# sea-with-sakura/ViT-of-Pytorch

Measured on AMD Instinct MI355X. Metric: images/sec training step, ViT-B/16 224px bf16, 1/2/4/8 MI355X, higher is better.
Workload: dtype bf16; 1 GPU; ViT-B16 @224 train step (fwd+CE+bwd+SGD-momentum/OneCycleLR); model=ViT-B16, image_size=224, per_gpu_batch=256, global_batch=256, seq_len=197, num_classes=1000, parallelism=dp1, step_launch=eager

## Files before the change

### include/vit_hip.h

```cpp
#ifndef VIT_HIP_H_
#define VIT_HIP_H_

#include <stdint.h>

#ifdef __cplusplus
extern "C" {
#endif

typedef void* vit_stream_t;

enum vit_status {
  VIT_OK = 0,
  VIT_ERR_INVALID_ARG = 1,
  VIT_ERR_HIP = 2,
  VIT_ERR_UNSUPPORTED = 3,
};

const char* vit_last_error(void);
int vit_abi_version(void);
const char* vit_build_id(void);

enum vit_layout { VIT_K_CONTIG = 0, VIT_MN_CONTIG = 1 };

typedef struct vit_dropout {
  float p;
  uint32_t site;
  uint64_t seed;
  uint64_t offset;
  int64_t row_stride;
} vit_dropout;

int vit_dropout_mask(const vit_dropout* d, int64_t row0, int64_t rows, int64_t cols, float* mult,
                     int64_t ld, vit_stream_t stream);

enum vit_epilogue {
  VIT_EPI_F32 = 0,
  VIT_EPI_BF16 = 1,
  VIT_EPI_BIAS_BF16 = 2,
  VIT_EPI_BIAS_GELU = 3,
  VIT_EPI_BIAS_RESID_F32 = 4,
  VIT_EPI_GELU_BWD = 5,
  VIT_EPI_PATCH = 6,
  VIT_EPI_SPLITK = 7,
  VIT_EPI_BIAS_GELU_DGELU = 8,
  VIT_EPI_MUL_BF16 = 9,
};

typedef struct vit_gemm_args {
  int64_t M, N, K;
  const void* A;
  int64_t lda;
  int64_t a_batch_stride;
  int32_t a_layout;
  int32_t b_layout;
  const void* B;
  int64_t ldb;
  int64_t b_batch_stride;
  void* C;
  int64_t ldc;
  int64_t c_batch_stride;
  void* C2;
  int64_t ldc2;
  const float* bias;
  int64_t bias_batch_stride;
  const void* aux;
  int64_t ldaux;
  const float* aux2;
  int64_t batch;
  int64_t split_k;
  int64_t tokens;
  float* col_partial;
  int32_t epilogue;
  int32_t tile;
  const vit_dropout* dropout;
} vit_gemm_args;

int vit_gemm_bf16(const vit_gemm_args* args, vit_stream_t stream);
int64_t vit_gemm_tile_rows(const vit_gemm_args* args);
int64_t vit_gemm_partial_rows(const vit_gemm_args* args);
int64_t vit_gemm_split_rows(const vit_gemm_args* args);
int vit_gemm_bf16_part(const vit_gemm_args* args, int32_t part, vit_stream_t stream);
int vit_gemm_splitk_group(const vit_gemm_args* args, int32_t n, vit_stream_t stream);

int vit_splitk_reduce(const float* ws, int64_t batch, int64_t split, int64_t M, int64_t N,
                      float* out, int64_t ldo, int64_t out_batch_stride, int32_t accumulate,
                      vit_stream_t stream);
#define VIT_SPLITK_GROUP_MAX 8
typedef struct vit_splitk_job {
  const float* ws;
  int64_t batch, split, M, N;
  float* out;
  int64_t ldo, out_batch_stride;
  int32_t accumulate;
  int32_t reserved;
} vit_splitk_job;
int vit_splitk_reduce_group(const vit_splitk_job* jobs, int32_t njobs, vit_stream_t stream);

int vit_layernorm_fwd(const float* x, int64_t ldx, const float* gamma, const float* beta,
                      void* y, int64_t ldy, int32_t y_f32, float* mean, float* rstd,
                      int64_t rows, int64_t D, float eps, vit_stream_t stream);
int64_t vit_layernorm_bwd_partial_rows(int64_t rows);
int64_t vit_layernorm_bwd_blocks(int64_t rows);
int vit_layernorm_bwd(const void* dy, int64_t lddy, int32_t dy_f32, const float* x, int64_t ldx,
                      const float* mean, const float* rstd, const float* gamma,
                      const float* dres, int64_t lddres, float* dx, int64_t lddx,
                      void* dx_bf16, int64_t lddxb, float* partial, float* dgamma_dbeta,
                      float* dx_colsum, int32_t accumulate_params, int64_t rows, int64_t D,
                      const vit_dropout* dx_dropout, vit_stream_t stream);

int vit_attention_fwd(const void* qkv, void* o, float* lse, int64_t B, int64_t N, int64_t H,
                      int64_t hd, float scale, vit_stream_t stream);
int vit_attention_bwd(const void* qkv, const void* o, const void* dout, const float* lse, void* dqkv,
                      float* bias_partial, int64_t B, int64_t N, int64_t H, int64_t hd, float scale,
                      vit_stream_t stream);
int vit_attention_fwd_rows(const void* qkv, void* o, float* lse, int64_t B, int64_t N, int64_t H, int64_t hd,
                           float scale, int64_t q_rows, vit_stream_t stream);
int vit_attention_bwd_rows(const void* qkv, const void* o, const void* dout, const float* lse, void* dqkv,
                           float* bias_partial, int64_t B, int64_t N, int64_t H, int64_t hd, float scale,
                           int64_t q_rows, vit_stream_t stream);
int64_t vit_attention_bias_rows(int64_t N, int64_t hd, int32_t path);
int64_t vit_attention_workspace_elems(int64_t B, int64_t N, int64_t H, int32_t path);
int vit_attention_fwd_ex(const void* qkv, void* o, float* lse, int64_t B, int64_t N, int64_t H, int64_t hd,
                         float scale, int64_t q_rows, int32_t path, vit_stream_t stream);
int vit_attention_bwd_ex(const void* qkv, const void* o, const void* dout, const float* lse, void* dqkv,
                         float* bias_partial, int64_t B, int64_t N, int64_t H, int64_t hd, float scale,
                         int64_t q_rows, int32_t path, float* workspace, vit_stream_t stream);

int vit_attention_fwd_varlen(const void* q, int64_t ldq, const void* k, int64_t ldk, const void* v, int64_t ldv,
                             void* o, int64_t ldo, const int32_t* cu_q, int64_t B, int64_t max_q, int64_t Nkv,
                             int64_t H, int64_t hd, float scale, vit_stream_t stream);

int vit_im2col(const float* x, void* out, int64_t B, int64_t img, int64_t P, int64_t Kpad,
               vit_stream_t stream);
int vit_im2col_hw(const float* x, void* out, int64_t B, int64_t H, int64_t W, int64_t Ph, int64_t Pw, int64_t Kpad,
                  vit_stream_t stream);

int vit_preprocess_u8(const uint8_t* images, int64_t B, int64_t H, int64_t W, int64_t image_stride,
                      const uint8_t* flips, int64_t out_h, int64_t out_w, const float* mean_std, float* out,
                      vit_stream_t stream);

enum vit_image_layout { VIT_IMAGES_HWC = 0, VIT_IMAGES_CHW = 1 };
int vit_preprocess_u8_gather(const uint8_t* images, int64_t n_images, int32_t layout, int64_t H, int64_t W,
                             int64_t image_stride, const int64_t* index, int64_t B, const uint8_t* flips,
                             int64_t out_h, int64_t out_w, const float* mean_std, float* out,
                             const int64_t* labels_in, int64_t* labels_out, vit_stream_t stream);

int vit_embed_grad(const float* dh0, int64_t B, int64_t N, int64_t D, float* dpos, float* dcls,
                   float* dconv_bias, const vit_dropout* dropout, vit_stream_t stream);

int64_t vit_colsum_partial_rows(int64_t rows);
int vit_colsum(const void* in, int32_t in_bf16, int64_t rows, int64_t cols, int64_t ld,
               float* partial, float* out, int32_t accumulate, vit_stream_t stream);
int vit_colsum3(const void* in, int32_t in_bf16, int64_t rows, int64_t seg, int64_t ld, float* partial,
                float* out0, float* out1, float* out2, int32_t accumulate, vit_stream_t stream);

#define VIT_COLSUM_BATCH_MAX 8
typedef struct vit_colsum_job {
  const float* in;
  int64_t rows, cols, ld, seg;
  float* out0;
  float* out1;
  float* out2;
  int32_t accumulate;
  int32_t reserved;
} vit_colsum_job;
int vit_colsum_batch(const vit_colsum_job* jobs, int32_t njobs, vit_stream_t stream);

int vit_gemm_f32(int64_t M, int64_t N, int64_t K, const float* A, int64_t lda, int32_t a_trans,
                 const float* B, int64_t ldb, int32_t b_trans, float* C, int64_t ldc,
                 const float* bias, int32_t accumulate, vit_stream_t stream);

int vit_cross_entropy(const float* logits, const int64_t* labels, int64_t B, int64_t C,
                      float* dlogits, float grad_scale, float* row_stats, vit_stream_t stream);

int vit_sgd_step(float* p, const float* g, float* buf, void* p_bf16, int64_t n, float lr,
                 float momentum, float weight_decay, int32_t first, vit_stream_t stream);
int vit_sgd_step_dev(float* p, const float* g, float* buf, void* p_bf16, int64_t n, const float* hyper,
                     float weight_decay, vit_stream_t stream);
int vit_cast_f32_bf16(const float* in, void* out, int64_t n, vit_stream_t stream);
int vit_cast_pad_rows(const float* in, int64_t rows, int64_t cols, void* out, int64_t ldo,
                      vit_stream_t stream);
#define VIT_CAST_BATCH_MAX 8
typedef struct vit_cast_job {
  const float* in;
  int64_t rows, cols, ldi;
  void* out;
  int64_t ldo, rows_pad, cols_pad;
} vit_cast_job;
int vit_cast_pad_batch(const vit_cast_job* jobs, int32_t njobs, vit_stream_t stream);
int vit_pack_cols(const float* in, int64_t zstride, int64_t ldi, int64_t rows, int64_t cols, int64_t Z,
                  void* out, int64_t ldo, int32_t out_bf16, vit_stream_t stream);
int vit_pack_cols_batched(const float* in, int64_t in_batch_stride, int64_t zstride, int64_t ldi, int64_t rows,
                          int64_t cols, int64_t Z, void* out, int64_t out_batch_stride, int64_t ldo,
                          int32_t out_bf16, int64_t batch, vit_stream_t stream);
int vit_transpose_f32_bf16(const float* in, int64_t rows, int64_t cols, int64_t ldi, void* out, int64_t ldo,
                           int64_t batch, int64_t in_batch_stride, int64_t out_batch_stride, vit_stream_t stream);
int vit_axpby(const float* x, float* y, int64_t n, float a, float b, vit_stream_t stream);

int vit_im2col_f32(const float* x, float* out, int64_t B, int64_t img, int64_t P, int64_t Kpad,
                   vit_stream_t stream);
int vit_im2col_hw_f32(const float* x, float* out, int64_t B, int64_t H, int64_t W, int64_t Ph, int64_t Pw,
                      int64_t Kpad, vit_stream_t stream);
int vit_embed_fwd_f32(float* h, int64_t B, int64_t N, int64_t D, const float* pos, const float* cls,
                      vit_stream_t stream);
int vit_gelu_f32(const float* in, float* out, int64_t n, vit_stream_t stream);
int vit_attention_fwd_f32(const float* qkv, float* o, int64_t B, int64_t N, int64_t H, int64_t hd,
                          float inv_sqrt_hd, vit_stream_t stream);

int vit_gelu_bwd_f32(const float* u, const float* dy, float* dx, int64_t n, vit_stream_t stream);
int vit_dropout_apply_f32(const vit_dropout* d, const float* in, float* out, int64_t rows, int64_t cols,
                          vit_stream_t stream);
int vit_add_bcast_f32(const float* x, const float* y, float* out, int64_t outer, int64_t inner, vit_stream_t stream);
int vit_segment_colsum(const void* in, int32_t in_bf16, int64_t ld, int64_t segs, int64_t seg_stride, int64_t row0,
                       int64_t seg_rows, int64_t cols, float scale, float* out, int64_t ldo, vit_stream_t stream);
int vit_segment_colsum_bcast(const void* in, int32_t in_bf16, int64_t ld, int64_t segs, int64_t seg_stride,
                             int64_t row0, int64_t seg_rows, int64_t cols, float scale, float* out, int64_t ldo,
                             void* bc, int64_t ldbc, int64_t bc_rows, vit_stream_t stream);
int64_t vit_router_dx_gate_partial_rows(int64_t rows_pad);
int vit_router_dx_gate(const float* dx, int64_t ldx, const float* g, int64_t ldg, float g_scale, const void* gp,
                       int64_t ldgp, int64_t T, int64_t N, int64_t reserve, int64_t cols, void* out, int64_t ldo,
                       int64_t rows_pad, int64_t cols_pad, float* col_partial, int64_t ldp, vit_stream_t stream);
int64_t vit_router_head_partials(int64_t T);
int vit_router_head_fwd(const float* logits, const float* noise, int32_t noise_mode, const float* yhard_in, int64_t T,
                        int64_t N, int32_t bs, int64_t reserve, int32_t training, float norm, float* soft, float* ysoft,
                        float* hard, float* indices, float* ent_part, float* entropy, vit_stream_t stream);
int vit_router_head_bwd(const float* soft, const float* ysoft, const float* dsoft, const float* dhard, const float* dind,
                        const float* dent, float norm, int64_t T, int64_t N, int32_t bs, int64_t reserve,
                        int32_t training, float* dlogits, vit_stream_t stream);
int vit_router_select(const float* indices, int64_t T, int32_t npos, const uint32_t* active_masks, int32_t nkeys,
                      void* active, void* sel, void* any, vit_stream_t stream);
int vit_cast_rows_masked(const float* in, int64_t ldi, int64_t rows, int64_t cols, const void* mask, void* out,
                         int64_t ldo, vit_stream_t stream);
int vit_cls_mse(const float* x, int64_t ldx, const float* t, int64_t ldt, int64_t B, int64_t D, float* e, float* part,
                float* loss, vit_stream_t stream);
int vit_cls_mse_bwd(float* dx, int64_t lddx, const float* e, int64_t B, int64_t D, const float* g,
                    vit_stream_t stream);
int vit_unpack_bf16_f32(const void* in, int64_t ldi, int64_t rows, int64_t cols, float* out, int64_t ldo,
                        vit_stream_t stream);

int vit_sqnorm_partial(const float* g, int64_t n, double* partial, int32_t nparts, vit_stream_t stream);
int vit_adamw_prep(const double* partial, int32_t nparts, const float* used, float* steps, int32_t nseg,
                   float lr, float beta1, float beta2, float max_norm, float* table, float* norm_out,
                   vit_stream_t stream);
int vit_adamw_update(float* p, float* g, float* m, float* v, void* p_bf16, const int64_t* chunks, int32_t nchunks,
                     const float* table, float decay, float beta1, float beta2, float one_minus_beta1,
                     float one_minus_beta2, float eps, int32_t write_grad, vit_stream_t stream);
int vit_adamw_chunk_elems(void);
int vit_scale_by_coef(float* g, int64_t n, const float* coef, vit_stream_t stream);
int vit_zero(void* ptr, int64_t bytes, vit_stream_t stream);
int vit_rows_select(void* dst, int64_t dld, const void* src, int64_t sld, const void* mask, int64_t rows,
                    int64_t row_bytes, vit_stream_t stream);
int vit_copy2d(void* dst, int64_t dpitch, const void* src, int64_t spitch, int64_t width, int64_t height,
               vit_stream_t stream);

#ifdef __cplusplus
}
#endif
#endif
```

### vit-of-pytorch_amd/csrc/capi.hip

```cpp
#include <stdarg.h>

#include "common.h"
#include "build_id.h"

namespace vit {
static thread_local char g_last_error[512] = "";

void set_error(const char* fmt, ...) {
  va_list ap;
  va_start(ap, fmt);
  vsnprintf(g_last_error, sizeof(g_last_error), fmt, ap);
  va_end(ap);
}

int check_hip(hipError_t e, const char* what) {
  if (e == hipSuccess) return VIT_OK;
  set_error("%s: %s", what, hipGetErrorString(e));
  return VIT_ERR_HIP;
}
}

extern "C" const char* vit_last_error(void) { return vit::g_last_error; }
extern "C" int vit_abi_version(void) { return 20; }
extern "C" const char* vit_build_id(void) { return VIT_BUILD_ID; }
```

### vit-of-pytorch_amd/csrc/elementwise.hip

```cpp
#include "common.h"

namespace {

template <typename OUT>
__global__ void im2col_kernel(const float* __restrict__ x, OUT* __restrict__ out, int B, int H, int W, int Ph, int Pw,
                              int Kpad) {
  const int gw = W / Pw;
  const int N = (H / Ph) * gw + 1;
  const long total = (long)B * N * Kpad;
  const int PP = Ph * Pw, K = 3 * PP;
  for (long i = (long)blockIdx.x * blockDim.x + threadIdx.x; i < total; i += (long)gridDim.x * blockDim.x) {
    const int col = (int)(i % Kpad);
    const long row = i / Kpad;
    const int t = (int)(row % N);
    const int b = (int)(row / N);
    float v = 0.f;
    if (t > 0 && col < K) {
      const int patch = t - 1, py = patch / gw, px = patch % gw;
      const int c = col / PP, rem = col % PP, ky = rem / Pw, kx = rem % Pw;
      v = x[(((long)b * 3 + c) * H + (py * Ph + ky)) * W + (px * Pw + kx)];
    }
    if constexpr (sizeof(OUT) == 2)
      out[i] = f2bf(v);
    else
      out[i] = v;
  }
}

__global__ void pos_grad_kernel(const float* __restrict__ dh0, int B, int N, int D, float* __restrict__ dpos,
                                DropDev drop) {
  const int n = blockIdx.y;
  const int d = blockIdx.x * blockDim.x + threadIdx.x;
  if (d >= D) return;
  float s = 0.f;
  if (drop.thr) {
    for (int b = 0; b < B; ++b) s += dh0[((long)b * N + n) * D + d] * drop_mult1(drop, (long)b * N + n, d);
  } else {
    for (int b = 0; b < B; ++b) s += dh0[((long)b * N + n) * D + d];
  }
  dpos[(long)n * D + d] = s;
}

__global__ void dropout_mask_kernel(DropDev drop, long row0, long rows, int cols, float* __restrict__ out, long ld) {
  const long r = blockIdx.y;
  const int c = blockIdx.x * blockDim.x + threadIdx.x;
  if (r >= rows || c >= cols) return;
  out[r * ld + c] = drop.thr ? drop_mult1(drop, row0 + r, c) : 1.0f;
}

template <typename OUT>
__global__ void im2col8_kernel(const float* __restrict__ x, OUT* __restrict__ out, int B, int H, int W, int Ph,
                               int Pw) {
  const int gw = W / Pw, N = (H / Ph) * gw + 1, PP = Ph * Pw, K8 = 3 * PP / 8;
  const long total = (long)B * N * K8;
  for (long i = (long)blockIdx.x * blockDim.x + threadIdx.x; i < total; i += (long)gridDim.x * blockDim.x) {
    const int c8 = (int)(i % K8);
    const long row = i / K8;
    const int t = (int)(row % N), b = (int)(row / N);
    float4 lo = make_float4(0.f, 0.f, 0.f, 0.f), hi = lo;
    if (t > 0) {
      const int patch = t - 1, py = patch / gw, px = patch % gw;
      const int col = c8 * 8, c = col / PP, rem = col % PP, ky = rem / Pw, kx = rem % Pw;
      const float4* src =
          reinterpret_cast<const float4*>(x + (((long)b * 3 + c) * H + (py * Ph + ky)) * W + (px * Pw + kx));
      lo = src[0];
      hi = src[1];
    }
    if constexpr (sizeof(OUT) == 2) {
      uint4 v;
      v.x = (uint32_t)f2bf(lo.x) | ((uint32_t)f2bf(lo.y) << 16);
      v.y = (uint32_t)f2bf(lo.z) | ((uint32_t)f2bf(lo.w) << 16);
      v.z = (uint32_t)f2bf(hi.x) | ((uint32_t)f2bf(hi.y) << 16);
      v.w = (uint32_t)f2bf(hi.z) | ((uint32_t)f2bf(hi.w) << 16);
      reinterpret_cast<uint4*>(out)[i] = v;
    } else {
      reinterpret_cast<float4*>(out)[2 * i] = lo;
      reinterpret_cast<float4*>(out)[2 * i + 1] = hi;
    }
  }
}

__global__ void __launch_bounds__(768) pos_grad4_kernel(const float* __restrict__ dh0, int B, int N, int D,
                                                        float* __restrict__ dpos, DropDev drop) {
  __shared__ float4 red[8][96];
  const int C4 = D / 4 / gridDim.y;
  const int n = blockIdx.x, c = threadIdx.x % C4, grp = threadIdx.x / C4;
  const int d = (blockIdx.y * C4 + c) * 4;
  float4 s = make_float4(0.f, 0.f, 0.f, 0.f);
  const float* base = dh0 + (long)n * D + d;
  const long bstride = (long)N * D;
#pragma unroll 4
  for (int b = grp; b < B; b += 8) {
    float4 v = *reinterpret_cast<const float4*>(base + b * bstride);
    if (drop.thr) {
      const long r = (long)b * N + n;
      v.x *= drop_mult1(drop, r, d);
      v.y *= drop_mult1(drop, r, d + 1);
      v.z *= drop_mult1(drop, r, d + 2);
      v.w *= drop_mult1(drop, r, d + 3);
    }
    s.x += v.x;
    s.y += v.y;
    s.z += v.z;
    s.w += v.w;
  }
  red[grp][c] = s;
  __syncthreads();
  if (grp == 0) {
#pragma unroll
    for (int k = 1; k < 8; ++k) {
      s.x += red[k][c].x;
      s.y += red[k][c].y;
      s.z += red[k][c].z;
      s.w += red[k][c].w;
    }
    *reinterpret_cast<float4*>(dpos + (long)n * D + d) = s;
  }
}

__global__ void __launch_bounds__(256) cls_bias_grad16_kernel(const float* __restrict__ dpos, int N, int D,
                                                              float* __restrict__ dcls, float* __restrict__ dbias) {
  __shared__ float red[16][17];
  const int c = threadIdx.x & 15, r = threadIdx.x >> 4;
  const int d = blockIdx.x * 16 + c;
  float s = 0.f;
  if (d < D)
    for (int n = 1 + r; n < N; n += 16) s += dpos[(long)n * D + d];
  red[r][c] = s;
  __syncthreads();
  if (r == 0 && d < D) {
    float t = 0.f;
#pragma unroll
    for (int k = 0; k < 16; ++k) t += red[k][c];
    dbias[d] = t;
    dcls[d] = dpos[d];
  }
}

constexpr int COLSUM_MAX_CHUNKS = 256;
constexpr int COLSUM_MIN_ROWS_PER_CHUNK = 64;

__device__ __forceinline__ float* seg_dst(float* out, float* out1, float* out2, long seg, long ch, int cols, int col) {
  if (seg <= 0) return out + ch * cols + col;
  const int k = (int)(col / seg);
  float* base = k == 0 ? out : (k == 1 ? out1 : out2);
  return base ? base + (col - k * seg) : nullptr;
}

template <bool BF16>
__global__ void __launch_bounds__(256) colsum8_kernel(const void* __restrict__ in, long rows, int cols, long ld,
                                                      int chunks, float* __restrict__ out, int accumulate,
                                                      long seg = 0, float* out1 = nullptr, float* out2 = nullptr) {
  __shared__ float red[8][32][9];
// ... 55 lines not shown
}
__global__ void colsum_final_kernel(const float* __restrict__ partial, int chunks, int cols, float* __restrict__ out,
                                    int accumulate) {
  const int c = blockIdx.x * blockDim.x + threadIdx.x;
  if (c >= cols) return;
  float s = 0.f;
  for (int k = 0; k < chunks; ++k) s += partial[(long)k * cols + c];
  out[c] = accumulate ? out[c] + s : s;
}

constexpr int GF_LD = 48;
__global__ void __launch_bounds__(256) gemm_f32_kernel(int M, int N, int K, const float* __restrict__ A, long lda,
                                                       int at, const float* __restrict__ B, long ldb, int bt,
                                                       float* __restrict__ C, long ldc, const float* __restrict__ bias,
                                                       int accumulate) {
  __shared__ float smem[4 * 2 * 16 * GF_LD];
  const int lane = threadIdx.x & 63, wave = threadIdx.x >> 6;
  const int m0 = blockIdx.y * 32, n0 = blockIdx.x * 32;
  float* As = smem + wave * 2 * 16 * GF_LD;
  float* Bs = As + 16 * GF_LD;
  v4f acc[2][2];
#pragma unroll
  for (int i = 0; i < 2; ++i)
#pragma unroll
    for (int j = 0; j < 2; ++j) acc[i][j] = v4f{0.f, 0.f, 0.f, 0.f};
  const int nkt = (K + 15) / 16;
  auto load = [&](int kt, float* av, float* bv) {
    const int k0 = kt * 16;
#pragma unroll
    for (int e = 0; e < 8; ++e) {
      const int idx = lane + e * 64;
      int m, k;
      if (at) { k = idx >> 5; m = idx & 31; } else { m = idx >> 4; k = idx & 15; }
      const int gm = m0 + m, gk = k0 + k;
      av[e] = (kt < nkt && gm < M && gk < K) ? (at ? A[(long)gk * lda + gm] : A[(long)gm * lda + gk]) : 0.f;
      int n, kb;
      if (bt) { n = idx >> 4; kb = idx & 15; } else { kb = idx >> 5; n = idx & 31; }
      const int gn = n0 + n, gkb = k0 + kb;
      bv[e] = (kt < nkt && gn < N && gkb < K) ? (bt ? B[(long)gn * ldb + gkb] : B[(long)gkb * ldb + gn]) : 0.f;
    }
  };
  float av[8], bv[8];
  load(wave, av, bv);
  for (int kt = wave; kt < nkt; kt += 4) {
#pragma unroll
    for (int e = 0; e < 8; ++e) {
      const int idx = lane + e * 64;
      if (at) As[(idx >> 5) * GF_LD + (idx & 31)] = av[e]; else As[(idx & 15) * GF_LD + (idx >> 4)] = av[e];
      if (bt) Bs[(idx & 15) * GF_LD + (idx >> 4)] = bv[e]; else Bs[(idx >> 5) * GF_LD + (idx & 31)] = bv[e];
    }
    load(kt + 4, av, bv);
    __builtin_amdgcn_wave_barrier();
    asm volatile("s_waitcnt lgkmcnt(0)" ::: "memory");
#pragma unroll
    for (int ks = 0; ks < 4; ++ks) {
      const int k = ks * 4 + (lane >> 4);
      float a[2], b[2];
#pragma unroll
      for (int t = 0; t < 2; ++t) {
        a[t] = As[k * GF_LD + t * 16 + (lane & 15)];
        b[t] = Bs[k * GF_LD + t * 16 + (lane & 15)];
      }
#pragma unroll
      for (int i = 0; i < 2; ++i)
#pragma unroll
        for (int j = 0; j < 2; ++j) acc[i][j] = __builtin_amdgcn_mfma_f32_16x16x4f32(a[i], b[j], acc[i][j], 0, 0, 0);
    }
    asm volatile("s_waitcnt lgkmcnt(0)" ::: "memory");
    __builtin_amdgcn_wave_barrier();
  }
  __syncthreads();
  float* red = smem;
#pragma unroll
  for (int i = 0; i < 2; ++i)
#pragma unroll
    for (int j = 0; j < 2; ++j)
#pragma unroll
      for (int r = 0; r < 4; ++r)
        red[wave * 32 * 33 + (i * 16 + 4 * (lane >> 4) + r) * 33 + j * 16 + (lane & 15)] = acc[i][j][r];
  __syncthreads();
#pragma unroll
  for (int e = 0; e < 4; ++e) {
    const int idx = threadIdx.x + e * 256, row = idx >> 5, col = idx & 31;
    const int m = m0 + row, n = n0 + col;
    if (m >= M || n >= N) continue;
    float v = red[row * 33 + col] + red[32 * 33 + row * 33 + col] + red[2 * 32 * 33 + row * 33 + col] +
              red[3 * 32 * 33 + row * 33 + col];
    if (bias) v += bias[n];
    float* dst = C + (long)m * ldc + n;
    *dst = accumulate ? *dst + v : v;
  }
}

__global__ void __launch_bounds__(256) ce_kernel(const float* __restrict__ logits, const int64_t* __restrict__ labels,
                                                 int C, float* __restrict__ dlogits, float grad_scale,
                                                 float* __restrict__ row_stats) {
  __shared__ float red[4];
  __shared__ float red2[4];
  const int b = blockIdx.x;
  const float* x = logits + (long)b * C;
  const int64_t y64 = labels[b];
  const bool ok = y64 >= 0 && y64 < C;
  const int y = ok ? (int)y64 : 0;
  const int lane = threadIdx.x & 63, wave = threadIdx.x >> 6;
  float mx = -INFINITY;
  for (int c = threadIdx.x; c < C; c += 256) mx = fmaxf(mx, x[c]);
  mx = wave_max(mx);
  if (lane == 0) red[wave] = mx;
  __syncthreads();
  mx = fmaxf(fmaxf(red[0], red[1]), fmaxf(red[2], red[3]));
  __syncthreads();
  const float xy = ok ? x[y] : __builtin_nanf("");
  float s = 0.f, gt = 0.f;
  for (int c = threadIdx.x; c < C; c += 256) {
    s += __expf(x[c] - mx);
    gt += x[c] > xy ? 1.f : 0.f;
  }
  s = wave_sum(s);
  gt = wave_sum(gt);
  if (lane == 0) {
    red[wave] = s;
    red2[wave] = gt;
  }
  __syncthreads();
  s = red[0] + red[1] + red[2] + red[3];
  gt = red2[0] + red2[1] + red2[2] + red2[3];
  const float lse = mx + logf(s);
  if (dlogits) {
    for (int c = threadIdx.x; c < C; c += 256) {
      const float p = __expf(x[c] - lse);
      dlogits[(long)b * C + c] = ok ? (p - (c == y ? 1.f : 0.f)) * grad_scale : __builtin_nanf("");
    }
  }
  if (threadIdx.x == 0 && row_stats) {
    row_stats[b * 3 + 0] = lse - xy;
    row_stats[b * 3 + 1] = gt < 1.f ? 1.f : 0.f;
    row_stats[b * 3 + 2] = gt < 5.f ? 1.f : 0.f;
  }
}

struct SgdHostScalars {
  float lr, mom;
  int first;
  __device__ __forceinline__ void get(float& l, float& m, bool& f) const { l = lr; m = mom; f = first != 0; }
};
struct SgdDevScalars {
  const float* hyper;
  __device__ __forceinline__ void get(float& l, float& m, bool& f) const {
    l = hyper[0];
    m = hyper[1];
    f = hyper[2] != 0.0f;
  }
};
template <class S>
__global__ void sgd_kernel(float* __restrict__ p, const float* __restrict__ g, float* __restrict__ buf,
                           bf16_t* __restrict__ pb, long n, const S sc, float wd) {
  float lr, mom;
  bool first;
  sc.get(lr, mom, first);
  const long n4 = n / 4;
  for (long i = (long)blockIdx.x * blockDim.x + threadIdx.x; i < n4; i += (long)gridDim.x * blockDim.x) {
    float4 pv = reinterpret_cast<float4*>(p)[i];
    const float4 gv = reinterpret_cast<const float4*>(g)[i];
    float4 d = make_float4(gv.x + wd * pv.x, gv.y + wd * pv.y, gv.z + wd * pv.z, gv.w + wd * pv.w);
    if (!first) {
      const float4 bv = reinterpret_cast<float4*>(buf)[i];
      d = make_float4(mom * bv.x + d.x, mom * bv.y + d.y, mom * bv.z + d.z, mom * bv.w + d.w);
    }
    reinterpret_cast<float4*>(buf)[i] = d;
    pv = make_float4(pv.x - lr * d.x, pv.y - lr * d.y, pv.z - lr * d.z, pv.w - lr * d.w);
    reinterpret_cast<float4*>(p)[i] = pv;
    if (pb) {
      uint2 u;
      u.x = pack2bf(pv.x, pv.y);
      u.y = pack2bf(pv.z, pv.w);
      reinterpret_cast<uint2*>(pb)[i] = u;
    }
  }
  const long t = n4 * 4 + (long)blockIdx.x * blockDim.x + threadIdx.x;
  if (blockIdx.x == 0 && t < n) {
    float d = g[t] + wd * p[t];
    if (!first) d = mom * buf[t] + d;
    buf[t] = d;
    p[t] -= lr * d;
    if (pb) pb[t] = f2bf(p[t]);
  }
}

__global__ void cast_kernel(const float* __restrict__ in, bf16_t* __restrict__ out, long n) {
  for (long i = (long)blockIdx.x * blockDim.x + threadIdx.x; i < n; i += (long)gridDim.x * blockDim.x) out[i] = f2bf(in[i]);
}
__global__ void cast_pad_kernel(const float* __restrict__ in, long rows, long cols, bf16_t* __restrict__ out, long ldo) {
  const long total = rows * ldo;
  for (long i = (long)blockIdx.x * blockDim.x + threadIdx.x; i < total; i += (long)gridDim.x * blockDim.x) {
    const long r = i / ldo, c = i % ldo;
    out[i] = c < cols ? f2bf(in[r * cols + c]) : (bf16_t)0;
  }
}
__global__ void axpby_kernel(const float* __restrict__ x, float* __restrict__ y, long n, float a, float b) {
  for (long i = (long)blockIdx.x * blockDim.x + threadIdx.x; i < n; i += (long)gridDim.x * blockDim.x)
    y[i] = a * x[i] + (b == 0.f ? 0.f : b * y[i]);
}

unsigned grid_for(long n, int per_thread = 1) {
  long b = (n / per_thread + 255) / 256;
  if (b < 1) b = 1;
  if (b > 8192) b = 8192;
  return (unsigned)b;
}

template <typename OUT>
void im2col_launch(const float* x, OUT* out, int64_t B, int64_t H, int64_t W, int64_t Ph, int64_t Pw, int64_t Kpad,
                   hipStream_t s) {
  const int64_t N = (H / Ph) * (W / Pw) + 1;
  if (Pw % 8 == 0 && W % 4 == 0 && Kpad == 3 * Ph * Pw && (uintptr_t)x % 16 == 0 && (uintptr_t)out % 16 == 0)
    hipLaunchKernelGGL(im2col8_kernel<OUT>, dim3(grid_for(B * N * Kpad / 8)), dim3(256), 0, s, x, out, (int)B, (int)H,
                       (int)W, (int)Ph, (int)Pw);
  else
    hipLaunchKernelGGL(im2col_kernel<OUT>, dim3(grid_for(B * N * Kpad)), dim3(256), 0, s, x, out, (int)B, (int)H,
                       (int)W, (int)Ph, (int)Pw, (int)Kpad);
}

}

extern "C" int vit_im2col_hw(const float* x, void* out, int64_t B, int64_t H, int64_t W, int64_t Ph, int64_t Pw,
                             int64_t Kpad, vit_stream_t stream) {
  VIT_CHECK_ARG(x && out && B > 0 && Ph > 0 && Pw > 0 && H >= Ph && W >= Pw && Kpad >= 3 * Ph * Pw &&
                    3 * H * W < (1L << 31) && Kpad < (1L << 31),
                "vit_im2col_hw: bad args");
  im2col_launch(x, (bf16_t*)out, B, H, W, Ph, Pw, Kpad, (hipStream_t)stream);
  VIT_LAUNCH_CHECK("vit_im2col_hw");
}

extern "C" int vit_im2col_hw_f32(const float* x, float* out, int64_t B, int64_t H, int64_t W, int64_t Ph, int64_t Pw,
                                 int64_t Kpad, vit_stream_t stream) {
  VIT_CHECK_ARG(x && out && B > 0 && Ph > 0 && Pw > 0 && H >= Ph && W >= Pw && Kpad >= 3 * Ph * Pw &&
                    3 * H * W < (1L << 31) && Kpad < (1L << 31),
                "vit_im2col_hw_f32: bad args");
  im2col_launch(x, out, B, H, W, Ph, Pw, Kpad, (hipStream_t)stream);
  VIT_LAUNCH_CHECK("vit_im2col_hw_f32");
}

extern "C" int vit_im2col(const float* x, void* out, int64_t B, int64_t img, int64_t P, int64_t Kpad,
                          vit_stream_t stream) {
  VIT_CHECK_ARG(x && out && B > 0 && P > 0 && img >= P && Kpad >= 3 * P * P, "vit_im2col: bad args");
  im2col_launch(x, (bf16_t*)out, B, img, img, P, P, Kpad, (hipStream_t)stream);
  VIT_LAUNCH_CHECK("vit_im2col");
}

extern "C" int vit_embed_grad(const float* dh0, int64_t B, int64_t N, int64_t D, float* dpos, float* dcls,
                              float* dconv_bias, const vit_dropout* dropout, vit_stream_t stream) {
  VIT_CHECK_ARG(dh0 && dpos && dcls && dconv_bias && B > 0 && N > 0 && D > 0, "vit_embed_grad: bad args");
  hipStream_t s = (hipStream_t)stream;
  int ys = 0;
  if (D % 4 == 0 && ((uintptr_t)dh0 % 16) == 0 && ((uintptr_t)dpos % 16) == 0) {
    const int d4 = (int)(D / 4);
    for (int y = (d4 + 95) / 96; y <= d4; ++y)
      if (d4 % y == 0) { ys = y; break; }
    if (ys == 1 && N < 256 && d4 % 2 == 0) ys = 2;
  }
  if (ys > 0)
    hipLaunchKernelGGL(pos_grad4_kernel, dim3((unsigned)N, (unsigned)ys), dim3((unsigned)(8 * (D / 4 / ys))), 0, s, dh0,
                       (int)B, (int)N, (int)D, dpos, make_drop(dropout));
  else
    hipLaunchKernelGGL(pos_grad_kernel, dim3((unsigned)((D + 255) / 256), (unsigned)N), dim3(256), 0, s, dh0, (int)B,
                       (int)N, (int)D, dpos, make_drop(dropout));
  hipLaunchKernelGGL(cls_bias_grad16_kernel, dim3((unsigned)((D + 15) / 16)), dim3(256), 0, s, dpos, (int)N, (int)D,
                     dcls, dconv_bias);
  VIT_LAUNCH_CHECK("vit_embed_grad");
}

extern "C" int64_t vit_colsum_partial_rows(int64_t rows) {
  int64_t c = rows / COLSUM_MIN_ROWS_PER_CHUNK;
  if (c > COLSUM_MAX_CHUNKS) c = COLSUM_MAX_CHUNKS;
  return c < 1 ? 1 : c;
}

extern "C" int vit_colsum3(const void* in, int32_t in_bf16, int64_t rows, int64_t seg, int64_t ld, float* partial,
                           float* out0, float* out1, float* out2, int32_t accumulate, vit_stream_t stream) {
  const int64_t cols = 3 * seg;
  VIT_CHECK_ARG(in && partial && seg > 0 && ld >= cols, "vit_colsum3: bad args");
  const int chunks = (int)vit_colsum_partial_rows(rows);
  const bool vec = cols % 8 == 0 && ld % 8 == 0 && ((uintptr_t)in % 32) == 0 && ((uintptr_t)partial % 16) == 0;
  VIT_CHECK_ARG(vec, "vit_colsum3: needs 8-column aligned rows");
  hipStream_t s = (hipStream_t)stream;
  const unsigned gx = (unsigned)((cols / 8 + 31) / 32);
  if (chunks == 1) {
    if (in_bf16)
      hipLaunchKernelGGL(colsum8_kernel<true>, dim3(gx, 1), dim3(256), 0, s, in, (long)rows, (int)cols, (long)ld, 1,
                         out0, (int)accumulate, (long)seg, out1, out2);
    else
      hipLaunchKernelGGL(colsum8_kernel<false>, dim3(gx, 1), dim3(256), 0, s, in, (long)rows, (int)cols, (long)ld, 1,
                         out0, (int)accumulate, (long)seg, out1, out2);
    VIT_LAUNCH_CHECK("vit_colsum3");
  }
  if (in_bf16)
    hipLaunchKernelGGL(colsum8_kernel<true>, dim3(gx, chunks), dim3(256), 0, s, in, (long)rows, (int)cols, (long)ld,
                       chunks, partial, 0, 0L, (float*)nullptr, (float*)nullptr);
  else
    hipLaunchKernelGGL(colsum8_kernel<false>, dim3(gx, chunks), dim3(256), 0, s, in, (long)rows, (int)cols, (long)ld,
                       chunks, partial, 0, 0L, (float*)nullptr, (float*)nullptr);
  hipLaunchKernelGGL(colsum8_kernel<false>, dim3(gx, 1), dim3(256), 0, s, (const void*)partial, (long)chunks,
                     (int)cols, (long)cols, 1, out0, (int)accumulate, (long)seg, out1, out2);
  VIT_LAUNCH_CHECK("vit_colsum3");
}

extern "C" int vit_colsum(const void* in, int32_t in_bf16, int64_t rows, int64_t cols, int64_t ld, float* partial,
                          float* out, int32_t accumulate, vit_stream_t stream) {
  VIT_CHECK_ARG(in && partial && out && cols > 0 && ld >= cols, "vit_colsum: bad args");
  hipStream_t s = (hipStream_t)stream;
  const int chunks = (int)vit_colsum_partial_rows(rows);
  const bool vec = cols % 8 == 0 && ld % 8 == 0 && ((uintptr_t)in % 32) == 0 && ((uintptr_t)partial % 16) == 0 &&
                   ((uintptr_t)out % 4) == 0;
  if (vec) {
    const unsigned gx = (unsigned)((cols / 8 + 31) / 32);
    float* dst1 = chunks == 1 ? out : partial;
    if (in_bf16)
      hipLaunchKernelGGL(colsum8_kernel<true>, dim3(gx, chunks), dim3(256), 0, s, in, (long)rows, (int)cols, (long)ld,
                         chunks, dst1, chunks == 1 ? (int)accumulate : 0);
    else
      hipLaunchKernelGGL(colsum8_kernel<false>, dim3(gx, chunks), dim3(256), 0, s, in, (long)rows, (int)cols,
                         (long)ld, chunks, dst1, chunks == 1 ? (int)accumulate : 0);
    if (chunks > 1)
      hipLaunchKernelGGL(colsum8_kernel<false>, dim3(gx, 1), dim3(256), 0, s, (const void*)partial, (long)chunks,
                         (int)cols, (long)cols, 1, out, (int)accumulate);
    VIT_LAUNCH_CHECK("vit_colsum");
  }
  const unsigned gx = (unsigned)((cols + 255) / 256);
  hipLaunchKernelGGL(colsum_partial_kernel, dim3(gx, chunks), dim3(256), 0, s, in, (int)in_bf16, (long)rows, (int)cols,
                     (long)ld, chunks, partial);
  hipLaunchKernelGGL(colsum_final_kernel, dim3(gx), dim3(256), 0, s, partial, chunks, (int)cols, out, (int)accumulate);
  VIT_LAUNCH_CHECK("vit_colsum");
}

namespace {
struct ColsumJobDev {
  const float* in;
  float* out[3];
  long ld;
  int rows, cols, seg, acc, blk0;
  int pad;
};
struct ColsumBatchDev {
  ColsumJobDev j[VIT_COLSUM_BATCH_MAX];
  int n;
};

__global__ void __launch_bounds__(256) colsum_batch_kernel(const ColsumBatchDev bt) {
  __shared__ float4 red[16][17];
  const int bid = blockIdx.x;
  int jx = 0;
#pragma unroll
  for (int k = 1; k < VIT_COLSUM_BATCH_MAX; ++k)
    if (k < bt.n && bid >= bt.j[k].blk0) jx = k;
  const ColsumJobDev& J = bt.j[jx];
  const int c0 = (bid - J.blk0) * 64;
  const int cg = threadIdx.x & 15, rl = threadIdx.x >> 4;
  const int c = c0 + cg * 4;
  float4 acc = {0.f, 0.f, 0.f, 0.f};
  if (J.pad && c < J.cols) {
    const float* p = J.in + c;
    const long ld = J.ld;
    int r = rl;
    for (; r + 112 < J.rows; r += 128) {
      float4 v[8];
#pragma unroll
      for (int u = 0; u < 8; ++u) v[u] = *reinterpret_cast<const float4*>(p + (long)(r + 16 * u) * ld);
#pragma unroll
      for (int u = 0; u < 8; ++u) {
        acc.x += v[u].x; acc.y += v[u].y; acc.z += v[u].z; acc.w += v[u].w;
      }
    }
    for (; r < J.rows; r += 16) {
      const float4 v = *reinterpret_cast<const float4*>(p + (long)r * ld);
      acc.x += v.x; acc.y += v.y; acc.z += v.z; acc.w += v.w;
    }
  } else if (c < J.cols) {
    const float* p = J.in + c;
    const int nc = J.cols - c < 4 ? J.cols - c : 4;
    for (int r = rl; r < J.rows; r += 16) {
      const float* q = p + (long)r * J.ld;
      acc.x += q[0];
      if (nc > 1) acc.y += q[1];
      if (nc > 2) acc.z += q[2];
      if (nc > 3) acc.w += q[3];
    }
  }
  red[rl][cg] = acc;
  __syncthreads();
  if (threadIdx.x < 64) {
    const int g = threadIdx.x >> 2, k = threadIdx.x & 3;
    const int col = c0 + threadIdx.x;
    if (col < J.cols) {
      float s = 0.f;
#pragma unroll
      for (int q = 0; q < 16; ++q) s += reinterpret_cast<const float*>(&red[q][g])[k];
      const int sg = J.seg > 0 ? col / J.seg : 0;
      float* base = J.out[sg];
      if (base) {
        float* dst = base + (col - sg * J.seg);
        *dst = J.acc ? *dst + s : s;
      }
    }
  }
}
}

extern "C" int vit_colsum_batch(const vit_colsum_job* jobs, int32_t njobs, vit_stream_t stream) {
  VIT_CHECK_ARG(jobs && njobs >= 1 && njobs <= VIT_COLSUM_BATCH_MAX, "vit_colsum_batch: njobs=%d outside [1, %d]",
                (int)njobs, VIT_COLSUM_BATCH_MAX);
  ColsumBatchDev bt{};
  int blk = 0;
  for (int k = 0; k < njobs; ++k) {
    const vit_colsum_job& s = jobs[k];
    VIT_CHECK_ARG(s.in && s.rows >= 1 && s.cols >= 1 && s.ld >= s.cols && s.rows <= 0x7fffffff &&
                      s.cols <= 0x7fffffff,
                  "vit_colsum_batch: job %d: bad shape (rows %lld, cols %lld, ld %lld)", k, (long long)s.rows,
                  (long long)s.cols, (long long)s.ld);
    VIT_CHECK_ARG(s.seg >= 0 && (s.seg == 0 || s.cols <= 3 * s.seg), "vit_colsum_batch: job %d: seg %lld", k,
                  (long long)s.seg);
    VIT_CHECK_ARG(s.out0 || s.out1 || s.out2, "vit_colsum_batch: job %d has no output", k);
    ColsumJobDev& d = bt.j[k];
    d.in = s.in;
    d.out[0] = s.out0;
    d.out[1] = s.out1;
    d.out[2] = s.out2;
    d.ld = (long)s.ld;
    d.rows = (int)s.rows;
    d.cols = (int)s.cols;
    d.seg = (int)s.seg;
    d.acc = s.accumulate ? 1 : 0;
    d.blk0 = blk;
    d.pad = (s.cols % 4 == 0 && s.ld % 4 == 0 && ((uintptr_t)s.in % 16) == 0) ? 1 : 0;
    blk += (int)((s.cols + 63) / 64);
  }
  bt.n = njobs;
  hipLaunchKernelGGL(colsum_batch_kernel, dim3(blk), dim3(256), 0, (hipStream_t)stream, bt);
  return vit::check_hip(hipGetLastError(), "vit_colsum_batch");
}

extern "C" int vit_gemm_f32(int64_t M, int64_t N, int64_t K, const float* A, int64_t lda, int32_t a_trans,
                            const float* B, int64_t ldb, int32_t b_trans, float* C, int64_t ldc, const float* bias,
                            int32_t accumulate, vit_stream_t stream) {
  VIT_CHECK_ARG(A && B && C && M >= 0 && N >= 0 && K >= 0, "vit_gemm_f32: bad args");
  if (M == 0 || N == 0) return VIT_OK;
  dim3 grid((unsigned)((N + 31) / 32), (unsigned)((M + 31) / 32)), block(256);
  hipLaunchKernelGGL(gemm_f32_kernel, grid, block, 0, (hipStream_t)stream, (int)M, (int)N, (int)K, A, (long)lda,
                     (int)a_trans, B, (long)ldb, (int)b_trans, C, (long)ldc, bias, (int)accumulate);
  VIT_LAUNCH_CHECK("vit_gemm_f32");
}

extern "C" int vit_cross_entropy(const float* logits, const int64_t* labels, int64_t B, int64_t C, float* dlogits,
                                 float grad_scale, float* row_stats, vit_stream_t stream) {
  VIT_CHECK_ARG(logits && labels && B > 0 && C > 0, "vit_cross_entropy: bad args");
  hipLaunchKernelGGL(ce_kernel, dim3((unsigned)B), dim3(256), 0, (hipStream_t)stream, logits, labels, (int)C, dlogits,
                     grad_scale, row_stats);
  VIT_LAUNCH_CHECK("vit_cross_entropy");
}

extern "C" int vit_sgd_step_dev(float* p, const float* g, float* buf, void* p_bf16, int64_t n, const float* hyper,
                                float weight_decay, vit_stream_t stream) {
  VIT_CHECK_ARG(p && g && buf && hyper && n >= 0, "vit_sgd_step_dev: bad args");
  VIT_CHECK_ARG(((uintptr_t)p | (uintptr_t)g | (uintptr_t)buf) % 16 == 0 && ((uintptr_t)p_bf16 % 8 == 0),
                "vit_sgd_step_dev: buffers must be 16-B aligned (bf16 mirror 8-B)");
  if (n == 0) return VIT_OK;
  hipLaunchKernelGGL(sgd_kernel<SgdDevScalars>, dim3(grid_for(n, 4)), dim3(256), 0, (hipStream_t)stream, p, g, buf,
                     (bf16_t*)p_bf16, (long)n, SgdDevScalars{hyper}, weight_decay);
  VIT_LAUNCH_CHECK("vit_sgd_step_dev");
}

extern "C" int vit_sgd_step(float* p, const float* g, float* buf, void* p_bf16, int64_t n, float lr, float momentum,
                            float weight_decay, int32_t first, vit_stream_t stream) {
  VIT_CHECK_ARG(p && g && buf && n >= 0, "vit_sgd_step: bad args");
  VIT_CHECK_ARG(((uintptr_t)p | (uintptr_t)g | (uintptr_t)buf) % 16 == 0 && ((uintptr_t)p_bf16 % 8 == 0),
                "vit_sgd_step: buffers must be 16-B aligned (bf16 mirror 8-B)");
  if (n == 0) return VIT_OK;
  hipLaunchKernelGGL(sgd_kernel<SgdHostScalars>, dim3(grid_for(n, 4)), dim3(256), 0, (hipStream_t)stream, p, g, buf,
                     (bf16_t*)p_bf16, (long)n, SgdHostScalars{lr, momentum, (int)first}, weight_decay);
  VIT_LAUNCH_CHECK("vit_sgd_step");
}

extern "C" int vit_cast_f32_bf16(const float* in, void* out, int64_t n, vit_stream_t stream) {
  VIT_CHECK_ARG(in && out && n >= 0, "vit_cast_f32_bf16: bad args");
  if (n == 0) return VIT_OK;
  hipLaunchKernelGGL(cast_kernel, dim3(grid_for(n)), dim3(256), 0, (hipStream_t)stream, in, (bf16_t*)out, (long)n);
  VIT_LAUNCH_CHECK("vit_cast_f32_bf16");
}

extern "C" int vit_cast_pad_rows(const float* in, int64_t rows, int64_t cols, void* out, int64_t ldo,
                                 vit_stream_t stream) {
  VIT_CHECK_ARG(in && out && ldo >= cols, "vit_cast_pad_rows: bad args");
  if (rows * ldo == 0) return VIT_OK;
  hipLaunchKernelGGL(cast_pad_kernel, dim3(grid_for(rows * ldo)), dim3(256), 0, (hipStream_t)stream, in, (long)rows,
                     (long)cols, (bf16_t*)out, (long)ldo);
  VIT_LAUNCH_CHECK("vit_cast_pad_rows");
}

namespace {
struct CastJobDev {
  const float* in;
  bf16_t* out;
  long rows, cols, ldi, ldo, rows_pad, cols_pad;
  int blk0, nb;
  int vec;
};
struct CastBatchDev {
  CastJobDev j[VIT_CAST_BATCH_MAX];
  int n;
};
__global__ void __launch_bounds__(256) cast_pad_batch_kernel(const CastBatchDev bt) {
  int jx = 0;
#pragma unroll
  for (int k = 1; k < VIT_CAST_BATCH_MAX; ++k)
    if (k < bt.n && (int)blockIdx.x >= bt.j[k].blk0) jx = k;
  const CastJobDev& J = bt.j[jx];
  if (J.vec) {
    const unsigned cq = (unsigned)(J.cols_pad >> 2), tq = (unsigned)(J.rows_pad * cq);
    for (unsigned q = (blockIdx.x - J.blk0) * 256u + threadIdx.x; q < tq; q += (unsigned)J.nb * 256u) {
      const unsigned r = q / cq, c = (q - r * cq) << 2;
      uint2 o = {0u, 0u};
      if (r < J.rows && c < J.cols) {
        const float4 v = *reinterpret_cast<const float4*>(J.in + r * J.ldi + c);
        o.x = pack2bf(v.x, v.y);
        o.y = pack2bf(v.z, v.w);
      }
      *reinterpret_cast<uint2*>(J.out + r * J.ldo + c) = o;
    }
    return;
  }
  const long total = J.rows_pad * J.cols_pad;
  for (long i = (long)(blockIdx.x - J.blk0) * 256 + threadIdx.x; i < total; i += (long)J.nb * 256) {
    const long r = i / J.cols_pad, c = i - r * J.cols_pad;
    J.out[r * J.ldo + c] = r < J.rows && c < J.cols ? f2bf(J.in[r * J.ldi + c]) : (bf16_t)0;
  }
}
}

extern "C" int vit_cast_pad_batch(const vit_cast_job* jobs, int32_t njobs, vit_stream_t stream) {
  VIT_CHECK_ARG(jobs && njobs >= 1 && njobs <= VIT_CAST_BATCH_MAX, "vit_cast_pad_batch: 1..%d jobs, got %d",
                VIT_CAST_BATCH_MAX, (int)njobs);
  CastBatchDev bt{};
  long blk = 0;
  for (int k = 0; k < njobs; ++k) {
    const vit_cast_job& j = jobs[k];
    VIT_CHECK_ARG(j.in && j.out && j.rows >= 0 && j.cols >= 0 && j.ldi >= j.cols && j.rows_pad >= j.rows &&
                      j.cols_pad >= j.cols && j.ldo >= j.cols_pad,
                  "vit_cast_pad_batch: job %d: bad shape", k);
    const int vec = (j.cols | j.cols_pad | j.ldi | j.ldo) % 4 == 0 && (uintptr_t)j.in % 16 == 0 &&
                    (uintptr_t)j.out % 8 == 0 && j.rows_pad * j.cols_pad / 4 < (1L << 31) ? 1 : 0;
    long nb = (j.rows_pad * j.cols_pad / (vec ? 4 : 1) + 255) / 256;
    if (nb > 2048) nb = 2048;
    if (nb < 1) nb = 1;
    CastJobDev& d = bt.j[k];
    d.in = j.in; d.out = (bf16_t*)j.out; d.rows = j.rows; d.cols = j.cols; d.ldi = j.ldi; d.ldo = j.ldo;
    d.rows_pad = j.rows_pad; d.cols_pad = j.cols_pad; d.blk0 = (int)blk; d.nb = (int)nb;
    d.vec = vec;
    blk += nb;
  }
  bt.n = njobs;
  hipLaunchKernelGGL(cast_pad_batch_kernel, dim3((unsigned)blk), dim3(256), 0, (hipStream_t)stream, bt);
  VIT_LAUNCH_CHECK("vit_cast_pad_batch");
}

extern "C" int vit_axpby(const float* x, float* y, int64_t n, float a, float b, vit_stream_t stream) {
  VIT_CHECK_ARG(x && y && n >= 0, "vit_axpby: bad args");
  if (n == 0) return VIT_OK;
  hipLaunchKernelGGL(axpby_kernel, dim3(grid_for(n)), dim3(256), 0, (hipStream_t)stream, x, y, (long)n, a, b);
  VIT_LAUNCH_CHECK("vit_axpby");
}

namespace {
template <bool BF16OUT>
__global__ void pack_cols_kernel(const float* __restrict__ in, long zstride, long ldi, int rows, int cols, int Z,
                                 void* __restrict__ out, long ldo, long in_bs = 0, long out_bs = 0) {
  in += (long)blockIdx.y * in_bs;
  out = (char*)out + (long)blockIdx.y * out_bs * (BF16OUT ? 2 : 4);
  const long total = (long)rows * Z * cols;
  for (long i = (long)blockIdx.x * blockDim.x + threadIdx.x; i < total; i += (long)gridDim.x * blockDim.x) {
    const long r = i / ((long)Z * cols);
    const int zc = (int)(i % ((long)Z * cols));
    const int z = zc / cols, c = zc % cols;
    const float v = in[z * zstride + r * ldi + c];
    if constexpr (BF16OUT)
      ((bf16_t*)out)[r * ldo + zc] = f2bf(v);
    else
      ((float*)out)[r * ldo + zc] = v;
  }
}
}

extern "C" int vit_pack_cols(const float* in, int64_t zstride, int64_t ldi, int64_t rows, int64_t cols, int64_t Z,
                             void* out, int64_t ldo, int32_t out_bf16, vit_stream_t stream) {
  VIT_CHECK_ARG(in && out && rows >= 0 && cols >= 0 && Z >= 1 && ldo >= Z * cols, "vit_pack_cols: bad args");
  const long total = rows * Z * cols;
  if (total == 0) return VIT_OK;
  if (out_bf16)
    hipLaunchKernelGGL(pack_cols_kernel<true>, dim3(grid_for(total)), dim3(256), 0, (hipStream_t)stream, in,
                       (long)zstride, (long)ldi, (int)rows, (int)cols, (int)Z, out, (long)ldo);
  else
    hipLaunchKernelGGL(pack_cols_kernel<false>, dim3(grid_for(total)), dim3(256), 0, (hipStream_t)stream, in,
                       (long)zstride, (long)ldi, (int)rows, (int)cols, (int)Z, out, (long)ldo);
  VIT_LAUNCH_CHECK("vit_pack_cols");
}

extern "C" int vit_pack_cols_batched(const float* in, int64_t in_batch_stride, int64_t zstride, int64_t ldi,
                                     int64_t rows, int64_t cols, int64_t Z, void* out, int64_t out_batch_stride,
                                     int64_t ldo, int32_t out_bf16, int64_t batch, vit_stream_t stream) {
  VIT_CHECK_ARG(in && out && rows >= 0 && cols >= 0 && Z >= 1 && ldo >= Z * cols && batch >= 1 && batch < 65536,
                "vit_pack_cols_batched: bad args");
  const long total = rows * Z * cols;
  if (total == 0) return VIT_OK;
  long gx = (total + 255) / 256;
  if (gx > 1024) gx = 1024;
  const dim3 grid((unsigned)gx, (unsigned)batch);
  if (out_bf16)
    hipLaunchKernelGGL(pack_cols_kernel<true>, grid, dim3(256), 0, (hipStream_t)stream, in, (long)zstride, (long)ldi,
                       (int)rows, (int)cols, (int)Z, out, (long)ldo, (long)in_batch_stride, (long)out_batch_stride);
  else
    hipLaunchKernelGGL(pack_cols_kernel<false>, grid, dim3(256), 0, (hipStream_t)stream, in, (long)zstride, (long)ldi,
                       (int)rows, (int)cols, (int)Z, out, (long)ldo, (long)in_batch_stride, (long)out_batch_stride);
  VIT_LAUNCH_CHECK("vit_pack_cols_batched");
// ... 742 lines not shown
```

### vit-of-pytorch_amd/csrc/gemm.hip

```cpp
#include "gemm_decl.h"

namespace {
using vitg::GemmDev;
using vitg::EPI_DROP;

int pick_tile(const vit_gemm_args* a) {
  if (a->tile > 0) return (int)a->tile;
  const bool ak = a->a_layout == VIT_K_CONTIG, bk = a->b_layout == VIT_K_CONTIG;
  if (a->epilogue == VIT_EPI_SPLITK && a->M >= 256 && a->N >= 256) {
    static const int env_sk = vit::knob("VIT_GEMM_SPLITK_CFG", 9);
    return env_sk == 5 || env_sk == 6 || env_sk == 7 || env_sk == 8 ? env_sk : 9;
  }
  if (a->M >= 1024 && a->N >= 256) {
    static const int env_rs = vit::knob("VIT_GEMM_RESID_PP2", 1);
    if (ak && (env_rs || !(a->epilogue == VIT_EPI_BIAS_RESID_F32 && a->K < 2048))) return 9;
    if (a->N >= 2048 && a->epilogue != VIT_EPI_GELU_BWD && a->epilogue != VIT_EPI_MUL_BF16) return 5;
    if (!bk && a->K >= 3072) return 5;
    return 3;
  }
  return 0;
}

int tile_rows_of(int cfg) {
  switch (cfg) {
    case 1: case 2: case 3: case 5: case 6: case 7: case 8: case 9: case 10: case 11: return 256;
    default: return 128;
  }
}

long wave_split_rows(const vit_gemm_args* a, int cfg) {
  if (!((cfg == 5 || cfg == 9) && a->batch == 1 && a->split_k == 1 && a->epilogue != VIT_EPI_PATCH && a->tile == 0))
    return 0;
  static const int ncu = [] {
    int dev = 0, n = 0;
    if (hipGetDevice(&dev) != hipSuccess || hipDeviceGetAttribute(&n, hipDeviceAttributeMultiprocessorCount, dev) !=
                                               hipSuccess)
      return 0;
    return n;
  }();
  if (ncu <= 0) return 0;
  const long tiles_n = (a->N + 255) / 256, tiles = ((a->M + 255) / 256) * tiles_n;
  const long full = tiles / ncu, rem = tiles - full * ncu;
  const long main_rows = (full * ncu / tiles_n) * 256;
  return full >= 1 && rem > 0 && 2 * rem <= ncu && main_rows > 0 && main_rows < a->M ? main_rows : 0;
}

int rem_config() {
  static const int rem_cfg = vit::knob("VIT_GEMM_REM_CFG", 0);
  return rem_cfg >= 0 && rem_cfg <= 9 && rem_cfg != 1 ? rem_cfg : 0;
}

}

extern "C" int64_t vit_gemm_tile_rows(const vit_gemm_args* a) {
  if (!a) return 0;
  return tile_rows_of(pick_tile(a));
}

extern "C" int64_t vit_gemm_partial_rows(const vit_gemm_args* a) {
  if (!a) return 0;
  const int cfg = pick_tile(a);
  const long main_rows = wave_split_rows(a, cfg);
  if (main_rows > 0) {
    const long rr = tile_rows_of(rem_config());
    return main_rows / 256 + (a->M - main_rows + rr - 1) / rr;
  }
  const long tr = tile_rows_of(cfg);
  return (a->M + tr - 1) / tr;
}

extern "C" int64_t vit_gemm_split_rows(const vit_gemm_args* a) {
  if (!a) return 0;
  return wave_split_rows(a, pick_tile(a));
}

#ifdef VIT_PP2_STAMPS
static unsigned long long* g_pp2_stamp_buf = nullptr;
extern "C" int vit_gemm_set_stamps(void* dev_buf) {
  g_pp2_stamp_buf = (unsigned long long*)dev_buf;
  return 0;
}
#endif

namespace {
int make_dev(const vit_gemm_args* a, GemmDev& d, bool& empty) {
  empty = false;
  VIT_CHECK_ARG(a != nullptr, "vit_gemm_bf16: null args");
  VIT_CHECK_ARG(a->M >= 0 && a->N >= 0 && a->K >= 0, "vit_gemm_bf16: negative size");
  VIT_CHECK_ARG(a->K % 64 == 0, "vit_gemm_bf16: K=%lld must be a multiple of 64", (long long)a->K);
  VIT_CHECK_ARG(a->M < (1 << 30) && a->N < (1 << 30), "vit_gemm_bf16: M/N too large");
  VIT_CHECK_ARG(a->A && a->B && a->C, "vit_gemm_bf16: null operand");
  VIT_CHECK_ARG(a->batch >= 1 && a->split_k >= 1, "vit_gemm_bf16: batch/split_k must be >= 1");
  VIT_CHECK_ARG(a->split_k == 1 || a->epilogue == VIT_EPI_SPLITK, "vit_gemm_bf16: split_k>1 needs VIT_EPI_SPLITK");
  VIT_CHECK_ARG(a->a_layout == VIT_K_CONTIG || a->a_layout == VIT_MN_CONTIG, "vit_gemm_bf16: bad a_layout");
  VIT_CHECK_ARG(a->b_layout == VIT_K_CONTIG || a->b_layout == VIT_MN_CONTIG, "vit_gemm_bf16: bad b_layout");
  if (a->M == 0 || a->N == 0) {
    empty = true;
    return VIT_OK;
  }
  const bool ak = a->a_layout == VIT_K_CONTIG, bk = a->b_layout == VIT_K_CONTIG;
  const long a_rows = ak ? a->M : a->K, a_cols = ak ? a->K : a->M;
  const long b_rows = bk ? a->N : a->K, b_cols = bk ? a->K : a->N;
  VIT_CHECK_ARG(a->lda >= a_cols && a->ldb >= b_cols, "vit_gemm_bf16: leading dimension too small");
  VIT_CHECK_ARG(a->lda % 8 == 0 && a->ldb % 8 == 0, "vit_gemm_bf16: lda/ldb must be multiples of 8");
  VIT_CHECK_ARG(((uintptr_t)a->A | (uintptr_t)a->B) % 16 == 0 && (a->a_batch_stride | a->b_batch_stride) % 8 == 0,
                "vit_gemm_bf16: A/B must be 16-byte aligned");
  const long a_bytes = ((a_rows - 1) * a->lda + ((a_cols + 7) & ~7L)) * 2;
  const long b_bytes = ((b_rows - 1) * a->ldb + ((b_cols + 7) & ~7L)) * 2;
  VIT_CHECK_ARG(a_bytes < (1L << 31) && b_bytes < (1L << 31), "vit_gemm_bf16: operand larger than 2 GiB");
  switch (a->epilogue) {
    case VIT_EPI_BIAS_GELU: VIT_CHECK_ARG(a->C2 != nullptr, "GELU epilogue needs C2"); break;
    case VIT_EPI_BIAS_RESID_F32: VIT_CHECK_ARG(a->aux != nullptr, "RESID epilogue needs aux"); break;
    case VIT_EPI_GELU_BWD: VIT_CHECK_ARG(a->aux != nullptr, "GELU_BWD epilogue needs aux"); break;
    case VIT_EPI_MUL_BF16: VIT_CHECK_ARG(a->aux != nullptr, "MUL epilogue needs aux"); break;
    case VIT_EPI_BIAS_GELU_DGELU: VIT_CHECK_ARG(a->C2 != nullptr, "GELU_DGELU epilogue needs C2"); break;
    case VIT_EPI_PATCH:
      VIT_CHECK_ARG(a->aux && a->aux2 && a->bias && a->tokens > 0 && a->batch == 1, "PATCH epilogue args");
      break;
    default: break;
  }
  d = GemmDev{};
  d.M = (int)a->M; d.N = (int)a->N; d.K = (int)a->K;
  d.A = (const char*)a->A; d.lda = a->lda; d.a_bs = a->a_batch_stride; d.a_bytes = (uint32_t)a_bytes;
  d.B = (const char*)a->B; d.ldb = a->ldb; d.b_bs = a->b_batch_stride; d.b_bytes = (uint32_t)b_bytes;
  d.C = a->C; d.ldc = a->ldc; d.c_bs = a->c_batch_stride;
  d.C2 = a->C2; d.ldc2 = a->ldc2;
  d.bias = a->bias; d.bias_bs = a->bias_batch_stride;
  d.aux = a->aux; d.ldaux = a->ldaux; d.aux2 = a->aux2;
  d.split_k = (int)a->split_k; d.tokens = (int)a->tokens;
  {
    auto al = [](const void* q) { return ((uintptr_t)q % 32) == 0; };
    bool v = al(a->C) && a->ldc % 8 == 0 && a->c_batch_stride % 8 == 0;
    if (a->C2) v = v && al(a->C2) && a->ldc2 % 8 == 0;
    if (a->bias) v = v && al(a->bias) && a->bias_batch_stride % 8 == 0;
    if (a->aux) v = v && al(a->aux) && a->ldaux % 8 == 0;
    if (a->aux2) v = v && al(a->aux2);
    if (a->epilogue == VIT_EPI_SPLITK) v = al(a->C) && a->N % 8 == 0;
    d.vec = v ? 1 : 0;
  }
  d.col_partial = a->col_partial;
  d.drop = make_drop(a->dropout);
  VIT_CHECK_ARG(!d.drop.thr || a->epilogue == VIT_EPI_PATCH || a->epilogue == VIT_EPI_BIAS_RESID_F32 ||
                    a->epilogue == VIT_EPI_BIAS_GELU_DGELU,
                "vit_gemm_bf16: dropout is supported on the PATCH, BIAS_RESID_F32 and BIAS_GELU_DGELU epilogues");
  VIT_CHECK_ARG(!d.drop.thr || (a->a_layout == VIT_K_CONTIG &&
                                  (a->b_layout == VIT_K_CONTIG || a->epilogue == VIT_EPI_BIAS_RESID_F32)),
                "vit_gemm_bf16: dropout epilogues need a K-contiguous A (and B, except BIAS_RESID_F32)");
  {
    static const int env_gm = vit::knob("VIT_GEMM_GROUP_M", 8);
    static const int env_nt = vit::knob("VIT_GEMM_NT", 0);
    d.group_m = env_gm;
    d.nt = env_nt;
    static const int env_diag = vit::knob("VIT_GEMM_DIAG", 0);
    d.diag = env_diag;
    static const int env_sx = vit::knob("VIT_GEMM_SPLIT_XCD", 1);
    d.split_xcd = env_sx;
    static const int env_prio = vit::knob("VIT_GEMM_PRIO", 1);
    d.prio = env_prio;
    static const int env_ilv = vit::knob("VIT_GEMM_ILV", -1);
    d.ilv = env_ilv;
#ifdef VIT_PP2_STAMPS
    d.stamps = g_pp2_stamp_buf;
#endif
  }
  return VIT_OK;
}

int gemm_bf16_impl(const vit_gemm_args* a, int part, vit_stream_t stream) {
  GemmDev d;
  bool empty = false;
  if (const int rc = make_dev(a, d, empty)) return rc;
  if (empty) return VIT_OK;
  const bool ak = a->a_layout == VIT_K_CONTIG, bk = a->b_layout == VIT_K_CONTIG;
  if (a->col_partial) {
    VIT_CHECK_ARG(a->batch == 1 && a->split_k == 1 && d.vec && a->N % 8 == 0 &&
                      (a->epilogue == VIT_EPI_F32 || a->epilogue == VIT_EPI_BF16 || a->epilogue == VIT_EPI_GELU_BWD ||
                       a->epilogue == VIT_EPI_MUL_BF16 ||
                       a->epilogue == VIT_EPI_BIAS_BF16 || a->epilogue == VIT_EPI_BIAS_RESID_F32),
                  "vit_gemm_bf16: col_partial needs batch 1, split_k 1, aligned N%%8==0 operands and a plain epilogue");
  }
  hipStream_t s = (hipStream_t)stream;
  const int batch = (int)a->batch, split = (int)a->split_k;
  const int cfg = pick_tile(a);
#ifdef VIT_DIAG_KNOBS
  VIT_CHECK_ARG(cfg >= 0 && cfg <= 11, "vit_gemm_bf16: bad tile config %d", cfg);
#else
  VIT_CHECK_ARG(cfg >= 0 && cfg <= 9, "vit_gemm_bf16: bad tile config %d", cfg);
#endif
  VIT_CHECK_ARG(cfg != 1 || a->K % 32 == 0, "vit_gemm_bf16: K");
  auto run = [&](int c, const GemmDev& g) -> hipError_t {
    switch (a->epilogue) {
      case VIT_EPI_F32: return vitg::launch_layout_x<VIT_EPI_F32>(c, g, ak, bk, batch, split, s);
      case VIT_EPI_BF16: return vitg::launch_layout_x<VIT_EPI_BF16>(c, g, ak, bk, batch, split, s);
      case VIT_EPI_BIAS_BF16: return vitg::launch_layout_x<VIT_EPI_BIAS_BF16>(c, g, ak, bk, batch, split, s);
      case VIT_EPI_BIAS_GELU: return vitg::launch_layout_x<VIT_EPI_BIAS_GELU>(c, g, ak, bk, batch, split, s);
      case VIT_EPI_BIAS_RESID_F32:
        if (g.drop.thr) return vitg::launch_kk_x<VIT_EPI_BIAS_RESID_F32 | EPI_DROP>(c, g, bk, batch, split, s);
        return vitg::launch_layout_x<VIT_EPI_BIAS_RESID_F32>(c, g, ak, bk, batch, split, s);
      case VIT_EPI_GELU_BWD: return vitg::launch_layout_x<VIT_EPI_GELU_BWD>(c, g, ak, bk, batch, split, s);
      case VIT_EPI_BIAS_GELU_DGELU:
        if (g.drop.thr) return vitg::launch_kk_x<VIT_EPI_BIAS_GELU_DGELU | EPI_DROP>(c, g, bk, batch, split, s);
        return vitg::launch_layout_x<VIT_EPI_BIAS_GELU_DGELU>(c, g, ak, bk, batch, split, s);
      case VIT_EPI_MUL_BF16: return vitg::launch_layout_x<VIT_EPI_MUL_BF16>(c, g, ak, bk, batch, split, s);
      case VIT_EPI_PATCH:
        if (g.drop.thr) return vitg::launch_kk_x<VIT_EPI_PATCH | EPI_DROP>(c, g, bk, batch, split, s);
        return vitg::launch_layout_x<VIT_EPI_PATCH>(c, g, ak, bk, batch, split, s);
      case VIT_EPI_SPLITK: return vitg::launch_layout_x<VIT_EPI_SPLITK>(c, g, ak, bk, batch, split, s);
      default: return hipErrorInvalidValue;
    }
  };
  if (a->epilogue < 0 || a->epilogue > VIT_EPI_MUL_BF16) {
    vit::set_error("vit_gemm_bf16: unknown epilogue %d", a->epilogue);
    return VIT_ERR_INVALID_ARG;
  }
  if (const long main_rows = wave_split_rows(a, cfg)) {
    GemmDev g1 = d, g2 = d;
    g1.M = (int)main_rows;
    g2.M = (int)(a->M - main_rows);
    const long r0 = main_rows;
    const long a_off = ak ? r0 * a->lda * 2 : r0 * 2;
    g2.A = d.A + a_off;
    g2.a_bytes = d.a_bytes > a_off ? (uint32_t)(d.a_bytes - a_off) : 0u;
    const int csz = (a->epilogue == VIT_EPI_F32 || a->epilogue == VIT_EPI_BIAS_RESID_F32) ? 4 : 2;
    g2.C = (char*)d.C + r0 * a->ldc * csz;
    if (d.C2) g2.C2 = (char*)d.C2 + r0 * a->ldc2 * 2;
    if (d.aux) g2.aux = (const char*)d.aux + r0 * a->ldaux * (a->epilogue == VIT_EPI_BIAS_RESID_F32 ? 4 : 2);
    if (d.col_partial) g2.col_partial = d.col_partial + (main_rows / 256) * a->N;
    g2.drop.row0 = (int)r0;
    hipError_t e = hipSuccess;
    if (part != 2) e = run(cfg, g1);
    if (e == hipSuccess && part != 1) e = run(rem_config(), g2);
    return vit::check_hip(e, "vit_gemm_bf16 launch");
  }
  if (part == 2) return VIT_OK;
  return vit::check_hip(run(cfg, d), "vit_gemm_bf16 launch");
}
}

extern "C" int vit_gemm_bf16(const vit_gemm_args* a, vit_stream_t stream) { return gemm_bf16_impl(a, 0, stream); }

extern "C" int vit_gemm_bf16_part(const vit_gemm_args* a, int32_t part, vit_stream_t stream) {
  VIT_CHECK_ARG(part == 1 || part == 2, "vit_gemm_bf16_part: part %d (1 = whole-wave rows, 2 = remainder)", part);
  return gemm_bf16_impl(a, part, stream);
}

extern "C" int vit_gemm_splitk_group(const vit_gemm_args* args, int32_t n, vit_stream_t stream) {
  VIT_CHECK_ARG(args != nullptr && n >= 1 && n <= vitg::GEMM_GROUP_MAX, "vit_gemm_splitk_group: 1..%d members, got %d",
                vitg::GEMM_GROUP_MAX, n);
  vitg::GemmGroup g{};
  long total = 0;
  for (int i = 0; i < n; ++i) {
    const vit_gemm_args* a = args + i;
    VIT_CHECK_ARG(a->epilogue == VIT_EPI_SPLITK && a->a_layout == VIT_MN_CONTIG && a->b_layout == VIT_MN_CONTIG &&
                      a->tile == 0 && !a->col_partial && !a->dropout,
                  "vit_gemm_splitk_group: member %d must be a split-K weight gradient (VIT_EPI_SPLITK, both operands "
                  "M/N-contiguous, no tile / col_partial / dropout)", i);
    bool empty = false;
    if (const int rc = make_dev(a, g.g[i], empty)) return rc;
    VIT_CHECK_ARG(!empty, "vit_gemm_splitk_group: member %d is empty", i);
    g.start[i] = (int)total;
    total += ((a->M + 255) / 256) * ((a->N + 255) / 256) * a->split_k * a->batch;
    VIT_CHECK_ARG(total < (1L << 30), "vit_gemm_splitk_group: grid too large");
  }
  g.start[n] = (int)total;
  g.n = n;
  return vit::check_hip(vitg::launch_splitk_group(g, (hipStream_t)stream), "vit_gemm_splitk_group launch");
}

namespace {
__global__ void splitk_reduce_kernel(const float* __restrict__ ws, int split, long M, long N, float* __restrict__ out,
                                     long ldo, long obs, int accumulate) {
  const int z = blockIdx.y;
  const long total = M * N;
  const float* w = ws + (long)z * split * total;
  float* o = out + z * obs;
  for (long i = (long)blockIdx.x * blockDim.x + threadIdx.x; i < total; i += (long)gridDim.x * blockDim.x) {
    float s = 0.f;
    for (int k = 0; k < split; ++k) s += w[k * total + i];
    const long m = i / N, n = i - m * N;
    float* dst = o + m * ldo + n;
    *dst = accumulate ? *dst + s : s;
  }
}
__global__ void splitk_reduce4_kernel(const float* __restrict__ ws, int split, long M, long N, float* __restrict__ out,
                                      long ldo, long obs, int accumulate) {
  const int z = blockIdx.y;
  const long total = M * N, total4 = total / 4;
  const float4* w = reinterpret_cast<const float4*>(ws + (long)z * split * total);
  float* o = out + z * obs;
  for (long i = (long)blockIdx.x * blockDim.x + threadIdx.x; i < total4; i += (long)gridDim.x * blockDim.x) {
    float4 s = make_float4(0.f, 0.f, 0.f, 0.f);
    int k = 0;
    for (; k + 4 <= split; k += 4) {
      const float4 a = w[(long)k * total4 + i], b = w[(long)(k + 1) * total4 + i];
      const float4 c = w[(long)(k + 2) * total4 + i], d = w[(long)(k + 3) * total4 + i];
      s.x += (a.x + b.x) + (c.x + d.x);
      s.y += (a.y + b.y) + (c.y + d.y);
      s.z += (a.z + b.z) + (c.z + d.z);
      s.w += (a.w + b.w) + (c.w + d.w);
    }
    for (; k < split; ++k) {
      const float4 a = w[(long)k * total4 + i];
      s.x += a.x; s.y += a.y; s.z += a.z; s.w += a.w;
    }
    const long e = i * 4, m = e / N, n = e - m * N;
    float4* dst = reinterpret_cast<float4*>(o + m * ldo + n);
    if (accumulate) {
      const float4 p = *dst;
      s.x += p.x; s.y += p.y; s.z += p.z; s.w += p.w;
    }
    *dst = s;
  }
}

struct SplitkJobDev {
  const float* ws;
  float* out;
  long M, N, ldo, obs;
  int split, batch, nb, blk0, acc;
};
struct SplitkGroupDev {
  SplitkJobDev j[VIT_SPLITK_GROUP_MAX];
  int n;
};
__global__ void splitk_reduce4_group_kernel(const SplitkGroupDev G) {
  int jx = 0;
#pragma unroll
  for (int k = 1; k < VIT_SPLITK_GROUP_MAX; ++k)
    if (k < G.n && (int)blockIdx.x >= G.j[k].blk0) jx = k;
  const SplitkJobDev& J = G.j[jx];
  const int local = blockIdx.x - J.blk0;
  const int z = local / J.nb, bx = local - z * J.nb;
  const long total = J.M * J.N, total4 = total / 4;
  const float4* w = reinterpret_cast<const float4*>(J.ws + (long)z * J.split * total);
  float* o = J.out + z * J.obs;
  for (long i = (long)bx * blockDim.x + threadIdx.x; i < total4; i += (long)J.nb * blockDim.x) {
// ... 80 lines not shown
```

### vit-of-pytorch_amd/csrc/gemm_decl.h

```cpp
#pragma once
#include "common.h"
#include <stdlib.h>

namespace vitg {

struct GemmDev {
  int M, N, K;
  const char* A;
  long lda;
  long a_bs;
  uint32_t a_bytes;
  const char* B;
  long ldb;
  long b_bs;
  uint32_t b_bytes;
  void* C;
  long ldc;
  long c_bs;
  void* C2;
  long ldc2;
  const float* bias;
  long bias_bs;
  const void* aux;
  long ldaux;
  const float* aux2;
  int split_k;
  int tokens;
  int vec;
  float* col_partial;
  int group_m;
  int nt;
  DropDev drop;
  int diag;
  int split_xcd;
  int prio;
  int ilv;
#ifdef VIT_PP2_STAMPS
  unsigned long long* stamps;
#endif
};

constexpr int GEMM_GROUP_MAX = 4;
struct GemmGroup {
  GemmDev g[GEMM_GROUP_MAX];
  int start[GEMM_GROUP_MAX + 1];
  int n;
};
hipError_t launch_splitk_group(const GemmGroup& g, hipStream_t s);

constexpr int EPI_DROP = 16;

template <int EPI>
hipError_t launch_layout_x(int cfg, const GemmDev& d, bool ak, bool bk, int batch, int split, hipStream_t s);
template <int EPI>
hipError_t launch_kk_x(int cfg, const GemmDev& d, bool bk, int batch, int split, hipStream_t s);
template <> hipError_t launch_layout_x<0>(int, const GemmDev&, bool, bool, int, int, hipStream_t);
template <> hipError_t launch_layout_x<1>(int, const GemmDev&, bool, bool, int, int, hipStream_t);
template <> hipError_t launch_layout_x<2>(int, const GemmDev&, bool, bool, int, int, hipStream_t);
template <> hipError_t launch_layout_x<3>(int, const GemmDev&, bool, bool, int, int, hipStream_t);
template <> hipError_t launch_layout_x<4>(int, const GemmDev&, bool, bool, int, int, hipStream_t);
template <> hipError_t launch_layout_x<5>(int, const GemmDev&, bool, bool, int, int, hipStream_t);
template <> hipError_t launch_layout_x<6>(int, const GemmDev&, bool, bool, int, int, hipStream_t);
template <> hipError_t launch_layout_x<7>(int, const GemmDev&, bool, bool, int, int, hipStream_t);
template <> hipError_t launch_layout_x<8>(int, const GemmDev&, bool, bool, int, int, hipStream_t);
template <> hipError_t launch_layout_x<9>(int, const GemmDev&, bool, bool, int, int, hipStream_t);
template <> hipError_t launch_kk_x<20>(int, const GemmDev&, bool, int, int, hipStream_t);
template <> hipError_t launch_kk_x<22>(int, const GemmDev&, bool, int, int, hipStream_t);
template <> hipError_t launch_kk_x<24>(int, const GemmDev&, bool, int, int, hipStream_t);
}
```

### vit-of-pytorch_amd/vitmi/_lib.py

```python
from __future__ import annotations

import ctypes
import os

_HERE = os.path.dirname(os.path.abspath(__file__))
LIB_PATH = os.environ.get("VITMI_LIB") or os.path.join(_HERE, "libvit_hip.so")

c_i64 = ctypes.c_int64
c_i32 = ctypes.c_int32
c_f32 = ctypes.c_float
c_vp = ctypes.c_void_p

ABI_VERSION = 20

K_CONTIG, MN_CONTIG = 0, 1
(EPI_F32, EPI_BF16, EPI_BIAS_BF16, EPI_BIAS_GELU, EPI_BIAS_RESID_F32, EPI_GELU_BWD, EPI_PATCH, EPI_SPLITK,
 EPI_BIAS_GELU_DGELU, EPI_MUL_BF16) = range(10)


class Dropout(ctypes.Structure):
    _fields_ = [("p", c_f32), ("site", ctypes.c_uint32), ("seed", ctypes.c_uint64), ("offset", ctypes.c_uint64),
                ("row_stride", c_i64)]


class GemmArgs(ctypes.Structure):
    _fields_ = [
        ("M", c_i64), ("N", c_i64), ("K", c_i64),
        ("A", c_vp), ("lda", c_i64), ("a_batch_stride", c_i64),
        ("a_layout", c_i32), ("b_layout", c_i32),
        ("B", c_vp), ("ldb", c_i64), ("b_batch_stride", c_i64),
        ("C", c_vp), ("ldc", c_i64), ("c_batch_stride", c_i64),
        ("C2", c_vp), ("ldc2", c_i64),
        ("bias", c_vp), ("bias_batch_stride", c_i64),
        ("aux", c_vp), ("ldaux", c_i64), ("aux2", c_vp),
        ("batch", c_i64), ("split_k", c_i64), ("tokens", c_i64), ("col_partial", c_vp),
        ("epilogue", c_i32), ("tile", c_i32), ("dropout", ctypes.POINTER(Dropout)),
    ]


class ColsumJob(ctypes.Structure):
    _fields_ = [("inp", c_vp), ("rows", c_i64), ("cols", c_i64), ("ld", c_i64), ("seg", c_i64),
                ("out0", c_vp), ("out1", c_vp), ("out2", c_vp), ("accumulate", c_i32), ("reserved", c_i32)]


COLSUM_BATCH_MAX = 8


class SplitkJob(ctypes.Structure):
    _fields_ = [("ws", c_vp), ("batch", c_i64), ("split", c_i64), ("M", c_i64), ("N", c_i64), ("out", c_vp),
                ("ldo", c_i64), ("out_batch_stride", c_i64), ("accumulate", c_i32), ("reserved", c_i32)]


SPLITK_GROUP_MAX = 8


class CastJob(ctypes.Structure):
    _fields_ = [("inp", c_vp), ("rows", c_i64), ("cols", c_i64), ("ldi", c_i64), ("out", c_vp), ("ldo", c_i64),
                ("rows_pad", c_i64), ("cols_pad", c_i64)]


CAST_BATCH_MAX = 8

_SIGS = {
    "vit_last_error": (ctypes.c_char_p, []),
    "vit_abi_version": (c_i32, []),
    "vit_gemm_bf16": (c_i32, [ctypes.POINTER(GemmArgs), c_vp]),
    "vit_gemm_tile_rows": (c_i64, [ctypes.POINTER(GemmArgs)]),
    "vit_gemm_partial_rows": (c_i64, [ctypes.POINTER(GemmArgs)]),
    "vit_gemm_split_rows": (c_i64, [ctypes.POINTER(GemmArgs)]),
    "vit_gemm_bf16_part": (c_i32, [ctypes.POINTER(GemmArgs), c_i32, c_vp]),
    "vit_gemm_splitk_group": (c_i32, [ctypes.POINTER(GemmArgs), c_i32, c_vp]),
    "vit_segment_colsum": (c_i32, [c_vp, c_i32, c_i64, c_i64, c_i64, c_i64, c_i64, c_i64, c_f32, c_vp, c_i64, c_vp]),
    "vit_segment_colsum_bcast": (c_i32, [c_vp, c_i32, c_i64, c_i64, c_i64, c_i64, c_i64, c_i64, c_f32, c_vp, c_i64,
                                         c_vp, c_i64, c_i64, c_vp]),
    "vit_router_dx_gate_partial_rows": (c_i64, [c_i64]),
    "vit_router_dx_gate": (c_i32, [c_vp, c_i64, c_vp, c_i64, c_f32, c_vp, c_i64, c_i64, c_i64, c_i64, c_i64, c_vp,
                                   c_i64, c_i64, c_i64, c_vp, c_i64, c_vp]),
    "vit_splitk_reduce_group": (c_i32, [ctypes.POINTER(SplitkJob), c_i32, c_vp]),
    "vit_cast_pad_batch": (c_i32, [ctypes.POINTER(CastJob), c_i32, c_vp]),
    "vit_router_head_partials": (c_i64, [c_i64]),
    "vit_cast_rows_masked": (c_i32, [c_vp, c_i64, c_i64, c_i64, c_vp, c_vp, c_i64, c_vp]),
    "vit_router_select": (c_i32, [c_vp, c_i64, c_i32, ctypes.POINTER(ctypes.c_uint32), c_i32, c_vp, c_vp, c_vp, c_vp]),
    "vit_cls_mse": (c_i32, [c_vp, c_i64, c_vp, c_i64, c_i64, c_i64, c_vp, c_vp, c_vp, c_vp]),
    "vit_cls_mse_bwd": (c_i32, [c_vp, c_i64, c_vp, c_i64, c_i64, c_vp, c_vp]),
    "vit_router_head_fwd": (c_i32, [c_vp, c_vp, c_i32, c_vp, c_i64, c_i64, c_i32, c_i64, c_i32, c_f32, c_vp, c_vp, c_vp,
                                    c_vp, c_vp, c_vp, c_vp]),
    "vit_router_head_bwd": (c_i32, [c_vp, c_vp, c_vp, c_vp, c_vp, c_vp, c_f32, c_i64, c_i64, c_i32, c_i64, c_i32, c_vp,
                                    c_vp]),
    "vit_splitk_reduce": (c_i32, [c_vp, c_i64, c_i64, c_i64, c_i64, c_vp, c_i64, c_i64, c_i32, c_vp]),
    "vit_layernorm_fwd": (c_i32, [c_vp, c_i64, c_vp, c_vp, c_vp, c_i64, c_i32, c_vp, c_vp, c_i64, c_i64, c_f32, c_vp]),
    "vit_layernorm_bwd_partial_rows": (c_i64, [c_i64]),
    "vit_layernorm_bwd_blocks": (c_i64, [c_i64]),
    "vit_layernorm_bwd": (c_i32, [c_vp, c_i64, c_i32, c_vp, c_i64, c_vp, c_vp, c_vp, c_vp, c_i64, c_vp, c_i64,
                                  c_vp, c_i64, c_vp, c_vp, c_vp, c_i32, c_i64, c_i64, ctypes.POINTER(Dropout),
                                  c_vp]),
    "vit_attention_fwd": (c_i32, [c_vp, c_vp, c_vp, c_i64, c_i64, c_i64, c_i64, c_f32, c_vp]),
    "vit_attention_bwd": (c_i32, [c_vp, c_vp, c_vp, c_vp, c_vp, c_vp, c_i64, c_i64, c_i64, c_i64, c_f32, c_vp]),
    "vit_attention_fwd_rows": (c_i32, [c_vp, c_vp, c_vp, c_i64, c_i64, c_i64, c_i64, c_f32, c_i64, c_vp]),
    "vit_attention_bwd_rows": (c_i32, [c_vp, c_vp, c_vp, c_vp, c_vp, c_vp, c_i64, c_i64, c_i64, c_i64, c_f32, c_i64,
                                       c_vp]),
    "vit_attention_bias_rows": (c_i64, [c_i64, c_i64, c_i32]),
    "vit_attention_workspace_elems": (c_i64, [c_i64, c_i64, c_i64, c_i32]),
    "vit_attention_fwd_ex": (c_i32, [c_vp, c_vp, c_vp, c_i64, c_i64, c_i64, c_i64, c_f32, c_i64, c_i32, c_vp]),
    "vit_attention_bwd_ex": (c_i32, [c_vp, c_vp, c_vp, c_vp, c_vp, c_vp, c_i64, c_i64, c_i64, c_i64, c_f32, c_i64,
                                     c_i32, c_vp, c_vp]),
    "vit_im2col": (c_i32, [c_vp, c_vp, c_i64, c_i64, c_i64, c_i64, c_vp]),
    "vit_im2col_hw": (c_i32, [c_vp, c_vp, c_i64, c_i64, c_i64, c_i64, c_i64, c_i64, c_vp]),
    "vit_preprocess_u8": (c_i32, [c_vp, c_i64, c_i64, c_i64, c_i64, c_vp, c_i64, c_i64, c_vp, c_vp, c_vp]),
    "vit_preprocess_u8_gather": (c_i32, [c_vp, c_i64, c_i32, c_i64, c_i64, c_i64, c_vp, c_i64, c_vp, c_i64, c_i64, c_vp,
                                         c_vp, c_vp, c_vp, c_vp]),
    "vit_embed_grad": (c_i32, [c_vp, c_i64, c_i64, c_i64, c_vp, c_vp, c_vp, ctypes.POINTER(Dropout), c_vp]),
    "vit_dropout_mask": (c_i32, [ctypes.POINTER(Dropout), c_i64, c_i64, c_i64, c_vp, c_i64, c_vp]),
    "vit_colsum_partial_rows": (c_i64, [c_i64]),
    "vit_colsum": (c_i32, [c_vp, c_i32, c_i64, c_i64, c_i64, c_vp, c_vp, c_i32, c_vp]),
    "vit_gemm_f32": (c_i32, [c_i64, c_i64, c_i64, c_vp, c_i64, c_i32, c_vp, c_i64, c_i32, c_vp, c_i64, c_vp, c_i32,
                             c_vp]),
    "vit_cross_entropy": (c_i32, [c_vp, c_vp, c_i64, c_i64, c_vp, c_f32, c_vp, c_vp]),
    "vit_sgd_step": (c_i32, [c_vp, c_vp, c_vp, c_vp, c_i64, c_f32, c_f32, c_f32, c_i32, c_vp]),
    "vit_cast_f32_bf16": (c_i32, [c_vp, c_vp, c_i64, c_vp]),
    "vit_cast_pad_rows": (c_i32, [c_vp, c_i64, c_i64, c_vp, c_i64, c_vp]),
    "vit_axpby": (c_i32, [c_vp, c_vp, c_i64, c_f32, c_f32, c_vp]),
    "vit_pack_cols": (c_i32, [c_vp, c_i64, c_i64, c_i64, c_i64, c_i64, c_vp, c_i64, c_i32, c_vp]),
    "vit_pack_cols_batched": (c_i32, [c_vp, c_i64, c_i64, c_i64, c_i64, c_i64, c_i64, c_vp, c_i64, c_i64, c_i32, c_i64,
                                      c_vp]),
    "vit_transpose_f32_bf16": (c_i32, [c_vp, c_i64, c_i64, c_i64, c_vp, c_i64, c_i64, c_i64, c_i64, c_vp]),
    "vit_colsum_batch": (c_i32, [ctypes.POINTER(ColsumJob), c_i32, c_vp]),
    "vit_colsum3": (c_i32, [c_vp, c_i32, c_i64, c_i64, c_i64, c_vp, c_vp, c_vp, c_vp, c_i32, c_vp]),
    "vit_im2col_f32": (c_i32, [c_vp, c_vp, c_i64, c_i64, c_i64, c_i64, c_vp]),
    "vit_im2col_hw_f32": (c_i32, [c_vp, c_vp, c_i64, c_i64, c_i64, c_i64, c_i64, c_i64, c_vp]),
    "vit_embed_fwd_f32": (c_i32, [c_vp, c_i64, c_i64, c_i64, c_vp, c_vp, c_vp]),
    "vit_gelu_f32": (c_i32, [c_vp, c_vp, c_i64, c_vp]),
    "vit_attention_fwd_f32": (c_i32, [c_vp, c_vp, c_i64, c_i64, c_i64, c_i64, c_f32, c_vp]),
    "vit_gelu_bwd_f32": (c_i32, [c_vp, c_vp, c_vp, c_i64, c_vp]),
    "vit_dropout_apply_f32": (c_i32, [ctypes.POINTER(Dropout), c_vp, c_vp, c_i64, c_i64, c_vp]),
    "vit_add_bcast_f32": (c_i32, [c_vp, c_vp, c_vp, c_i64, c_i64, c_vp]),
    "vit_unpack_bf16_f32": (c_i32, [c_vp, c_i64, c_i64, c_i64, c_vp, c_i64, c_vp]),
    "vit_attention_fwd_varlen": (c_i32, [c_vp, c_i64, c_vp, c_i64, c_vp, c_i64, c_vp, c_i64, c_vp, c_i64, c_i64, c_i64,
                                         c_i64, c_i64, c_f32, c_vp]),
    "vit_sqnorm_partial": (c_i32, [c_vp, c_i64, c_vp, c_i32, c_vp]),
    "vit_adamw_prep": (c_i32, [c_vp, c_i32, c_vp, c_vp, c_i32, c_f32, c_f32, c_f32, c_f32, c_vp, c_vp, c_vp]),
    "vit_adamw_update": (c_i32, [c_vp, c_vp, c_vp, c_vp, c_vp, c_vp, c_i32, c_vp, c_f32, c_f32, c_f32, c_f32, c_f32,
                                 c_f32, c_i32, c_vp]),
    "vit_adamw_chunk_elems": (c_i32, []),
    "vit_scale_by_coef": (c_i32, [c_vp, c_i64, c_vp, c_vp]),
    "vit_zero": (c_i32, [c_vp, c_i64, c_vp]),
    "vit_copy2d": (c_i32, [c_vp, c_i64, c_vp, c_i64, c_i64, c_i64, c_vp]),
    "vit_rows_select": (c_i32, [c_vp, c_i64, c_vp, c_i64, c_vp, c_i64, c_i64, c_vp]),
    "vit_sgd_step_dev": (c_i32, [c_vp, c_vp, c_vp, c_vp, c_i64, c_vp, c_f32, c_vp]),
    "vit_build_id": (ctypes.c_char_p, []),
}

EXPORTED = tuple(_SIGS)

_lib = None


class VitHipError(RuntimeError):
    pass


def load(path: str | None = None):
    global _lib
    if _lib is not None:
        return _lib
    p = path or LIB_PATH
    if not os.path.exists(p):
        raise VitHipError(f"libvit_hip.so not built ({p}); run `make -C vit-of-pytorch_amd` or __graft_entry__.build()")
    lib = ctypes.CDLL(p)
    for name, (res, args) in _SIGS.items():
        fn = getattr(lib, name)
        fn.restype = res
        fn.argtypes = args
    if lib.vit_abi_version() != ABI_VERSION:
        raise VitHipError(f"{p} has ABI {lib.vit_abi_version()}, the bindings expect {ABI_VERSION}: rebuild it "
                          "(make -C vit-of-pytorch_amd)")
    check_build_id(lib, p)
    _lib = lib
    return lib


def check_build_id(lib, path: str, expected: str | None = None):
    from . import buildid
    if expected is None:
        if not buildid.have_sources():
            return
        expected = buildid.tree_id()
    got = lib.vit_build_id().decode()
    if got != expected:
        raise VitHipError(f"{path} was built from other sources (build id {got}, this tree {expected}): rebuild it "
                          "(make -C vit-of-pytorch_amd)")


def check(status: int, what: str):
    if status != 0:
        msg = _lib.vit_last_error().decode(errors="replace") if _lib is not None else "?"
        raise VitHipError(f"{what} failed (status {status}): {msg}")
```

### vit-of-pytorch_amd/vitmi/engine.py

```python
from __future__ import annotations

import math
import os
from collections import OrderedDict
from dataclasses import dataclass

import torch

from . import ops
from ._lib import (EPI_BF16, EPI_BIAS_BF16, EPI_BIAS_GELU_DGELU, EPI_BIAS_RESID_F32, EPI_MUL_BF16, EPI_PATCH,
                   EPI_SPLITK, K_CONTIG, MN_CONTIG)

ALIGN = 64


def _rup(x, m):
    return (x + m - 1) // m * m


_NBUF = 2

_WGRAD_TARGET = int(os.environ.get("VIT_WGRAD_TARGET", "256"))


def _hw(v):
    if isinstance(v, int):
        return v, v
    h, w = v
    return int(h), int(w)


@dataclass(frozen=True)
class ArchConfig:
    image_size: int | tuple = 224
    patch_size: int | tuple = 16
    emb_dim: int = 768
    mlp_dim: int = 3072
    num_heads: int = 12
    num_layers: int = 12
    num_classes: int = 1000

    def __post_init__(self):
        for f in ("image_size", "patch_size"):
            v = getattr(self, f)
            if not isinstance(v, int):
                object.__setattr__(self, f, _hw(v))

    @property
    def image_hw(self):
        return _hw(self.image_size)

    @property
    def patch_hw(self):
        return _hw(self.patch_size)

    @property
    def grid_hw(self):
        (h, w), (fh, fw) = self.image_hw, self.patch_hw
        return h // fh, w // fw

    @property
    def grid(self):
        gh, gw = self.grid_hw
        if gh != gw:
            raise ValueError(f"ArchConfig.grid is the side of a square patch grid; this one is {gh}x{gw} (use grid_hw)")
        return gh

    @property
    def tokens(self):
        gh, gw = self.grid_hw
        return gh * gw + 1

    @property
    def head_dim(self):
        return self.emb_dim // self.num_heads

    @property
    def patch_k(self):
        fh, fw = self.patch_hw
        return 3 * fh * fw


def layer_param_specs(cfg: ArchConfig, i: int):
    D, M, H = cfg.emb_dim, cfg.mlp_dim, cfg.num_heads
    hd = D // H
    p = f"transformer.encoder_layers.{i}."
    out = [(p + "norm1.weight", (D,)), (p + "norm1.bias", (D,))]
    for w in ("query", "key", "value"):
        out += [(p + f"attn.{w}.weight", (D, H, hd)), (p + f"attn.{w}.bias", (H, hd))]
    out += [(p + "attn.out.weight", (H, hd, D)), (p + "attn.out.bias", (D,))]
    out += [(p + "norm2.weight", (D,)), (p + "norm2.bias", (D,))]
    out += [(p + "mlp.fc1.weight", (M, D)), (p + "mlp.fc1.bias", (M,))]
    out += [(p + "mlp.fc2.weight", (D, M)), (p + "mlp.fc2.bias", (D,))]
    return out


def flat_param_specs(cfg: ArchConfig):
    D, C = cfg.emb_dim, cfg.num_classes
    specs = [("classifier.weight", (C, D)), ("classifier.bias", (C,)),
             ("transformer.norm.weight", (D,)), ("transformer.norm.bias", (D,))]
    for i in reversed(range(cfg.num_layers)):
        specs += layer_param_specs(cfg, i)
    specs += [("embedding.weight", (D, 3, *cfg.patch_hw)), ("embedding.bias", (D,)),
              ("transformer.pos_embedding.pos_embedding", (1, cfg.tokens, D)), ("cls_token", (1, 1, D))]
    return specs


class FlatLayout:
    def __init__(self, cfg: ArchConfig):
        self.cfg = cfg
        self.offsets = OrderedDict()
        self.shapes = OrderedDict()
        off = 0
        self.layer_ranges = {}
        for name, shape in flat_param_specs(cfg):
            n = math.prod(shape)
            self.offsets[name] = off
            self.shapes[name] = shape
            off = _rup(off + n, ALIGN)
        self.numel = off
        L = cfg.num_layers
        self.buckets = []
        self.buckets.append(("head", 0, self.offsets[self._lname(L - 1, "norm1.weight")]))
        for i in reversed(range(L)):
            start = self.offsets[self._lname(i, "norm1.weight")]
            end = self.offsets[self._lname(i - 1, "norm1.weight")] if i > 0 else self.offsets["embedding.weight"]
            self.buckets.append((f"layer{i}", start, end))
        self.buckets.append(("embed", self.offsets["embedding.weight"], self.numel))

    @staticmethod
    def _lname(i, s):
        return f"transformer.encoder_layers.{i}.{s}"

    def view(self, buf, name):
        o = self.offsets[name]
        shape = self.shapes[name]
        return buf[o:o + math.prod(shape)].view(shape)


class _Acts:

    def __init__(self, cfg: ArchConfig, b: int, dev):
        D, M, H, L, N = cfg.emb_dim, cfg.mlp_dim, cfg.num_heads, cfg.num_layers, cfg.tokens
        T = b * N
        Tp = _rup(T, 64)
        self.b, self.T, self.Tp = b, T, Tp
        z = lambda *s, dt=torch.bfloat16: torch.zeros(*s, device=dev, dtype=dt)
        f = torch.float32
        self.kpad = _rup(cfg.patch_k, 64)
        self.patches = z(Tp, self.kpad)
        self.h = [z(Tp, D, dt=f) for _ in range(L + 1)]
        self.hm = [z(Tp, D, dt=f) for _ in range(L)]
        self.ln1 = [z(Tp, D) for _ in range(L)]
        self.ln2 = [z(Tp, D) for _ in range(L)]
        self.mu1 = [z(T, dt=f) for _ in range(L)]
        self.rs1 = [z(T, dt=f) for _ in range(L)]
        self.mu2 = [z(T, dt=f) for _ in range(L)]
        self.rs2 = [z(T, dt=f) for _ in range(L)]
        self.qkv = [z(Tp, 3 * D) for _ in range(L)]
        self.o = [z(Tp, D) for _ in range(L)]
        self.lse = [z(b, H, N, dt=f) for _ in range(L)]
        self.gp = [z(Tp, M) for _ in range(L)]
        self.g = [z(Tp, M) for _ in range(L)]
        self.lncls = z(b, D, dt=f)
        self.muf = z(b, dt=f)
        self.rsf = z(b, dt=f)
        self.logits = z(b, cfg.num_classes, dt=f)
        self.dh = z(Tp, D, dt=f)
        self.dhb = [z(Tp, D), z(Tp, D)]
        self.dg = [z(Tp, M), z(Tp, M)]
        self.dyln = z(Tp, D)
        self.dO = z(Tp, D)
        self.dqkv = [z(Tp, 3 * D), z(Tp, 3 * D)]
        self.dlncls = z(b, D, dt=f)
        self.dlogits = z(b, cfg.num_classes, dt=f)
        self.row_stats = z(b, 3, dt=f)
        self.lnparts = [z(ops.layernorm_bwd_blocks(T), 3 * D, dt=f) for _ in range(_NBUF)]
        self.gelu_parts = [z(-(-T // 128), M, dt=f) for _ in range(_NBUF)]
        self.attn_bias_rows = ops.attention_bias_rows(N, D // H)
        self.qkv_bparts = [z(b * self.attn_bias_rows, 3 * D, dt=f) for _ in range(_NBUF)]
        nws = ops.attention_workspace_elems(b, N, H)
        self.attn_ws = z(nws, dt=f) if nws else None
        bp = _rup(b, 64)
        self.bp = bp
        self.c_o, self.c_ln2, self.c_dh, self.c_dh2, self.c_dyln = (z(bp, D) for _ in range(5))
        self.c_g, self.c_gp, self.c_dg = (z(bp, M) for _ in range(3))
        self.c_mu2, self.c_rs2 = z(b, dt=f), z(b, dt=f)


class _BiasReducer:

    def __init__(self, eng, a):
        self.eng = eng
        self.a = a
        self.D = eng.cfg.emb_dim
        self.nxt = {}
        self.queued = {}
        self.jobs = []

    def buf(self, kind, bufs):
        n = self.queued.get(kind, 0)
        if n == len(bufs):
            self.flush()
            n = 0
        self.queued[kind] = n + 1
        i = self.nxt.get(kind, 0)
        self.nxt[kind] = (i + 1) % len(bufs)
        return bufs[i]

    def reduce(self, part, rows, cols, ld, outs, seg=0):
        self.jobs.append((part, rows, cols, ld, seg, outs, False))
        if len(self.jobs) == ops.COLSUM_BATCH_MAX:
            self.flush()

    def flush(self):
        if self.jobs:
            ops.colsum_batch(self.jobs)
            self.jobs = []
        self.queued.clear()

    def ln_bwd(self, dy, lddy, x, ldx, mean, rstd, gamma, dx, lddx, rows, dgamma_dbeta, dx_colsum, **kw):
        part = self.buf("ln", self.a.lnparts)
        D = self.D
        ops.layernorm_bwd(dy, lddy, x, ldx, mean, rstd, gamma, dx, lddx, part, rows, D, **kw)
        self.reduce(part, ops.layernorm_bwd_blocks(rows), 3 * D, 3 * D, (dgamma_dbeta, dgamma_dbeta[D:], dx_colsum),
                    seg=D)


class ViTEngine:

    def __init__(self, cfg: ArchConfig, device="cuda", flat: torch.Tensor | None = None):
        if cfg.emb_dim % cfg.num_heads:
            raise ValueError("emb_dim must be divisible by num_heads")
        if cfg.head_dim % 16 or cfg.head_dim > 96:
            raise NotImplementedError(f"head_dim {cfg.head_dim} not supported by the HIP attention kernel "
                                      "(multiples of 16 up to 96)")
        if cfg.emb_dim % 64 or cfg.mlp_dim % 64:
            raise NotImplementedError("emb_dim and mlp_dim must be multiples of 64")
        self.cfg = cfg
        self.dev = torch.device(device)
        self.attn_fwd_path = ops.ATTN_AUTO
        self.layout = FlatLayout(cfg)
        n = self.layout.numel
        self.flat = flat if flat is not None else torch.zeros(n, device=self.dev)
        self.grad = torch.zeros(n, device=self.dev)
        self.mirror = torch.zeros(n, device=self.dev, dtype=torch.bfloat16)
        D, L = cfg.emb_dim, cfg.num_layers
        M = cfg.mlp_dim
        bf = torch.bfloat16
        self.wqkv = torch.zeros(L, D, 3 * D, device=self.dev, dtype=bf)
        self.bqkv = torch.zeros(L, 3 * D, device=self.dev)
        kp = _rup(cfg.patch_k, 64)
        self.wconv = torch.zeros(D, kp, device=self.dev, dtype=torch.bfloat16) if kp != cfg.patch_k else None
        self._acts = {}
        self._mirror_sig = None
        o = [self.off(self.lname(i, "norm1.weight")) for i in range(L)]
        self.layer_stride = o[0] - o[1] if L > 1 else 0
        assert all(o[i] == o[0] - i * self.layer_stride for i in range(L))
        self._ws = None
        self.step_id = 0
        self.grad_ready_hook = None
        self.grad_ready_finish = None
        self.overlap_wgrad = os.environ.get("VITMI_OVERLAP", "0") == "1"
        self.group_wgrad = os.environ.get("VITMI_GROUP_WGRAD", "1") != "0"
        self.prune_last = os.environ.get("VITMI_PRUNE_LAST", "1") != "0"
        self._pruned = False
        self._side = None
        self._ev_pool, self._ev_next = [], 0
        self.probe = None
        self.probe_wgrad = None
        self.drop_seed = (torch.initial_seed() * 0x9E3779B97F4A7C15 + 0x632BE59BD9B4E019) & (2**64 - 1)
        self._drop_offset = 0
        self._drop = None

    def _event(self):
        if self._ev_next == len(self._ev_pool):
            self._ev_pool.append(torch.cuda.Event())
        ev = self._ev_pool[self._ev_next]
        self._ev_next += 1
        return ev

    def pv(self, name, buf=None):
        return self.layout.view(self.flat if buf is None else buf, name)

    def off(self, name):
        return self.layout.offsets[name]

    def lname(self, i, s):
        return f"transformer.encoder_layers.{i}.{s}"

    def load_params(self, params):
        for k, v in params.items():
            self.pv(k).copy_(v.to(self.dev, torch.float32).reshape(self.layout.shapes[k]))
        self.invalidate_mirror()

    def state(self):
        return OrderedDict((k, self.pv(k)) for k in self.layout.offsets)

    def invalidate_mirror(self):
        self._mirror_sig = None

    def refresh_mirror(self, full=True):
        cfg = self.cfg
        D = cfg.emb_dim
        if full:
            ops.cast_bf16(self.flat, self.mirror, self.layout.numel)
        M, L = cfg.mlp_dim, cfg.num_layers
        lst = self.layer_stride
        o0 = lambda s: self.off(self.lname(0, s))
        zs = self.off(self.lname(0, "attn.key.weight")) - o0("attn.query.weight")
        ops.pack_cols_batched(self.flat[o0("attn.query.weight"):], -lst, zs, D, D, D, 3, self.wqkv, D * 3 * D, 3 * D, L)
        ops.pack_cols_batched(self.flat[o0("attn.query.bias"):], -lst, zs, D, 1, D, 3, self.bqkv, 3 * D, 3 * D, L)
        if self.wconv is not None:
            w = self.off("embedding.weight")
            ops.cast_pad_rows(self.flat[w:], D, cfg.patch_k, self.wconv, self.wconv.shape[1])

    def mark_mirror_fresh(self, sig):
        self._mirror_sig = sig

    def acts(self, b):
        a = self._acts.get(b)
        if a is None:
            if len(self._acts) >= 2:
                self._acts.pop(next(iter(self._acts)))
            a = _Acts(self.cfg, b, self.dev)
            self._acts[b] = a
        return a

    def _splitk(self, M, N, K, z=1):
        return ops.splitk_factor(M, N, K, z, _WGRAD_TARGET)

    def _workspace(self, numel):
        if self._ws is None or self._ws.numel() < numel:
            self._ws = torch.empty(numel, device=self.dev)
        return self._ws

    def _wgrad(self, A, lda, B, ldb, M, N, K, out, ldo, batch=1, b_bs=0, out_bs=0):
        s = self._splitk(M, N, K, batch)
        ws = self._workspace(batch * s * M * N)
        if self.probe_wgrad is not None:
            ev0 = torch.cuda.Event(enable_timing=True)
            ev0.record()
        ops.gemm(A, B, ws, M, N, K, a_layout=MN_CONTIG, b_layout=MN_CONTIG, lda=lda, ldb=ldb, ldc=N,
                 epilogue=EPI_SPLITK, batch=batch, b_bs=b_bs, split_k=s)
        if self.probe_wgrad is not None:
            ev1 = torch.cuda.Event(enable_timing=True)
            ev1.record()
            self.probe_wgrad.append((ev0, ev1, 2.0 * M * N * K * batch, K, False))
        ops.splitk_reduce(ws, batch, s, M, N, out, ldo, out_bs)

    def _wgrad_group(self, specs):
        K = specs[0][6]
        assert all(sp[6] == K for sp in specs)
        s = ops.splitk_factor_group([(sp[4], sp[5], sp[9]) for sp in specs], K, _WGRAD_TARGET)
        sizes = [sp[9] * s * sp[4] * sp[5] for sp in specs]
        ws = self._workspace(sum(sizes))
        members, views, o = [], [], 0
        for sp, n in zip(specs, sizes):
            A, lda, B, ldb, M, N, _, _, _, batch, b_bs, _ = sp
            w = ws[o:o + n]
            o += n
            views.append(w)
            members.append((A, B, w, M, N, K, dict(a_layout=MN_CONTIG, b_layout=MN_CONTIG, lda=lda, ldb=ldb, ldc=N,
                                                    epilogue=EPI_SPLITK, batch=batch, b_bs=b_bs, split_k=s)))
        if self.probe_wgrad is not None:
            ev0 = torch.cuda.Event(enable_timing=True)
            ev0.record()
        ops.gemm_splitk_group(members)
        if self.probe_wgrad is not None:
            ev1 = torch.cuda.Event(enable_timing=True)
            ev1.record()
            self.probe_wgrad.append((ev0, ev1, sum(2.0 * sp[4] * sp[5] * K * sp[9] for sp in specs), K, True))
        ops.splitk_reduce_group([(w, sp[9], s, sp[4], sp[5], sp[7], sp[8], sp[11], False) for sp, w in zip(specs, views)])

    def _dd(self, site, row_stride=1):
        if self._drop is None:
            return None
        p, seed, off = self._drop
        return ops.dropout_desc(p, site, seed, off, row_stride)

    def forward(self, x: torch.Tensor, dropout_p: float = 0.0):
        cfg = self.cfg
        if x.dim() != 4 or x.shape[1] != 3 or tuple(x.shape[2:]) != cfg.image_hw:
            raise ValueError(f"expected input [b, 3, {cfg.image_hw[0]}, {cfg.image_hw[1]}], got {tuple(x.shape)}")
        x = x.to(self.dev, torch.float32).contiguous()
        b = x.shape[0]
        a = self.acts(b)
        D, M, H, N, L = cfg.emb_dim, cfg.mlp_dim, cfg.num_heads, cfg.tokens, cfg.num_layers
        hd = D // H
        T = a.T
        mv = self.mirror
        f = self.flat
        if dropout_p and dropout_p > 0.0:
            if not dropout_p < 1.0:
                raise ValueError(f"dropout probability has to be in [0, 1), got {dropout_p}")
            self._drop_offset += 1
            self._drop = (float(dropout_p), self.drop_seed, self._drop_offset)
        else:
            self._drop = None
        dd = self._dd
        ops.im2col_hw(x, a.patches, b, *cfg.image_hw, *cfg.patch_hw, a.kpad)
        wconv = self.wconv if self.wconv is not None else mv[self.off("embedding.weight"):]
        ops.gemm(a.patches, wconv, a.h[0], T, D, a.kpad, a_layout=K_CONTIG, b_layout=K_CONTIG, lda=a.kpad,
                 ldb=a.kpad, ldc=D, epilogue=EPI_PATCH, bias=f[self.off("embedding.bias"):],
                 aux=f[self.off("transformer.pos_embedding.pos_embedding"):], ldaux=D,
                 aux2=f[self.off("cls_token"):], tokens=N, dropout=dd(0))
        scale = 1.0 / math.sqrt(hd)
        self._pruned = self.prune_last and self._drop is None
        for i in range(L):
            ln = lambda s: self.off(self.lname(i, s))
            ops.layernorm_fwd(a.h[i], D, f[ln("norm1.weight"):], f[ln("norm1.bias"):], a.ln1[i], D, a.mu1[i],
                              a.rs1[i], T, D)
            ops.gemm(a.ln1[i], self.wqkv[i], a.qkv[i], T, 3 * D, D, a_layout=K_CONTIG, b_layout=MN_CONTIG, lda=D,
                     ldb=3 * D, ldc=3 * D, epilogue=EPI_BIAS_BF16, bias=self.bqkv[i])
            last = self._pruned and i == L - 1
            ops.attention_fwd(a.qkv[i], a.o[i], a.lse[i], b, N, H, hd, scale, q_rows=1 if last else None,
                              path=self.attn_fwd_path)
            if last:
                self._forward_last_cls(a, i, b)
                break
            ops.gemm(a.o[i], mv[ln("attn.out.weight"):], a.hm[i], T, D, D, a_layout=K_CONTIG, b_layout=MN_CONTIG,
                     lda=D, ldb=D, ldc=D, epilogue=EPI_BIAS_RESID_F32, bias=f[ln("attn.out.bias"):], aux=a.h[i],
                     ldaux=D, dropout=dd(1 + 3 * i))
            ops.layernorm_fwd(a.hm[i], D, f[ln("norm2.weight"):], f[ln("norm2.bias"):], a.ln2[i], D, a.mu2[i],
                              a.rs2[i], T, D)
            if self.probe is not None:
                ev0 = torch.cuda.Event(enable_timing=True)
                ev0.record()
            ops.gemm(a.ln2[i], mv[ln("mlp.fc1.weight"):], a.gp[i], T, M, D, a_layout=K_CONTIG, b_layout=K_CONTIG,
                     lda=D, ldb=D, ldc=M, epilogue=EPI_BIAS_GELU_DGELU, bias=f[ln("mlp.fc1.bias"):], C2=a.g[i],
                     ldc2=M, dropout=dd(2 + 3 * i))
            if self.probe is not None:
                ev1 = torch.cuda.Event(enable_timing=True)
                ev1.record()
                self.probe.append((ev0, ev1))
            ops.gemm(a.g[i], mv[ln("mlp.fc2.weight"):], a.h[i + 1], T, D, M, a_layout=K_CONTIG, b_layout=K_CONTIG,
                     lda=M, ldb=M, ldc=D, epilogue=EPI_BIAS_RESID_F32, bias=f[ln("mlp.fc2.bias"):], aux=a.hm[i],
                     ldaux=D, dropout=dd(3 + 3 * i))
        ops.layernorm_fwd(a.h[L], N * D, f[self.off("transformer.norm.weight"):], f[self.off("transformer.norm.bias"):],
                          a.lncls, D, a.muf, a.rsf, b, D)
        C = cfg.num_classes
        ops.gemm_f32(b, C, D, a.lncls, D, False, f[self.off("classifier.weight"):], D, True, a.logits, C,
                     bias=f[self.off("classifier.bias"):])
        self.step_id += 1
        self._last_b = b
        return a.logits

    def _forward_last_cls(self, a, i, b):
        cfg = self.cfg
        D, M, N = cfg.emb_dim, cfg.mlp_dim, cfg.tokens
        f, mv = self.flat, self.mirror
        ln = lambda s: self.off(self.lname(i, s))
        S = N * D
        ops.gemm(a.o[i], mv[ln("attn.out.weight"):], a.hm[i], b, D, D, a_layout=K_CONTIG, b_layout=MN_CONTIG, lda=S,
                 ldb=D, ldc=S, epilogue=EPI_BIAS_RESID_F32, bias=f[ln("attn.out.bias"):], aux=a.h[i], ldaux=S)
        ops.copy2d(a.c_o, D * 2, a.o[i], S * 2, D * 2, b)
        ops.layernorm_fwd(a.hm[i], S, f[ln("norm2.weight"):], f[ln("norm2.bias"):], a.c_ln2, D, a.c_mu2, a.c_rs2,
                          b, D)
        ops.gemm(a.c_ln2, mv[ln("mlp.fc1.weight"):], a.c_gp, b, M, D, a_layout=K_CONTIG, b_layout=K_CONTIG, lda=D,
                 ldb=D, ldc=M, epilogue=EPI_BIAS_GELU_DGELU, bias=f[ln("mlp.fc1.bias"):], C2=a.c_g, ldc2=M)
        ops.gemm(a.c_g, mv[ln("mlp.fc2.weight"):], a.h[i + 1], b, D, M, a_layout=K_CONTIG, b_layout=K_CONTIG,
                 lda=M, ldb=M, ldc=S, epilogue=EPI_BIAS_RESID_F32, bias=f[ln("mlp.fc2.bias"):], aux=a.hm[i], ldaux=S)

    def _backward_last_cls(self, a, i, b, g, on_side, bias):
        cfg = self.cfg
        D, M, N = cfg.emb_dim, cfg.mlp_dim, cfg.tokens
        S = N * D
        f, mv = self.flat, self.mirror
        gv = lambda name: g[self.off(self.lname(i, name)):]
        bp = a.bp
        on_side(lambda: self._wgrad(a.c_dh, D, a.c_g, M, D, M, bp, gv("mlp.fc2.weight"), M))
        gpart = bias.buf("gelu", a.gelu_parts)
        w2 = mv[self.off(self.lname(i, "mlp.fc2.weight")):]
        kw = dict(a_layout=K_CONTIG, b_layout=MN_CONTIG, lda=D, ldb=M, ldc=M, epilogue=EPI_MUL_BF16, aux=a.c_gp,
                  ldaux=M, col_partial=gpart)
        ops.gemm(a.c_dh, w2, a.c_dg, b, M, D, **kw)
        tiles_m = ops.gemm_partial_rows(a.c_dh, w2, a.c_dg, b, M, D, **kw)
        bias.reduce(gpart, tiles_m, M, M, (gv("mlp.fc1.bias"),))
        on_side(lambda: self._wgrad(a.c_dg, M, a.c_ln2, D, M, D, bp, gv("mlp.fc1.weight"), D))
        ops.gemm(a.c_dg, mv[self.off(self.lname(i, "mlp.fc1.weight")):], a.c_dyln, b, D, M, a_layout=K_CONTIG,
                 b_layout=MN_CONTIG, lda=M, ldb=D, ldc=D, epilogue=EPI_BF16)
        bias.ln_bwd(a.c_dyln, D, a.hm[i], S, a.c_mu2, a.c_rs2, f[self.off(self.lname(i, "norm2.weight")):], a.dh, S, b,
                    gv("norm2.weight"), gv("attn.out.bias"), dres=a.dh, lddres=S, dx_bf16=a.c_dh2, lddxb=D)
        on_side(lambda: self._wgrad(a.c_o, D, a.c_dh2, D, D, D, bp, gv("attn.out.weight"), D))
        ops.zero_(a.dO)
        ops.gemm(a.c_dh2, mv[self.off(self.lname(i, "attn.out.weight")):], a.dO, b, D, D, a_layout=K_CONTIG,
                 b_layout=K_CONTIG, lda=D, ldb=D, ldc=S, epilogue=EPI_BF16)

    def forward_exact(self, x: torch.Tensor):
        cfg = self.cfg
        if x.dim() != 4 or x.shape[1] != 3 or tuple(x.shape[2:]) != cfg.image_hw:
            raise ValueError(f"expected input [b, 3, {cfg.image_hw[0]}, {cfg.image_hw[1]}], got {tuple(x.shape)}")
        x = x.to(self.dev, torch.float32).contiguous()
        b = x.shape[0]
        D, M, H, N, L, C = cfg.emb_dim, cfg.mlp_dim, cfg.num_heads, cfg.tokens, cfg.num_layers, cfg.num_classes
        hd = D // H
        T, kp = b * N, cfg.patch_k
        f = self.flat
        e = lambda *shape: torch.empty(*shape, device=self.dev)
        fv = lambda name: f[self.off(name):]
        patches = e(T, kp)
        ops.im2col_hw_f32(x, patches, b, *cfg.image_hw, *cfg.patch_hw, kp)
        h = e(T, D)
        ops.gemm_f32(T, D, kp, patches, kp, False, fv("embedding.weight"), kp, True, h, D, bias=fv("embedding.bias"))
        ops.embed_fwd_f32(h, b, N, D, fv("transformer.pos_embedding.pos_embedding"), fv("cls_token"))
        y, qkv, o, u = e(T, D), e(T, 3 * D), e(T, D), e(T, M)
        mu, rs = e(T), e(T)
        for i in range(L):
            ln = lambda s: fv(self.lname(i, s))
            ops.layernorm_fwd(h, D, ln("norm1.weight"), ln("norm1.bias"), y, D, mu, rs, T, D)
            for z, w in enumerate(("query", "key", "value")):
                ops.gemm_f32(T, D, D, y, D, False, ln(f"attn.{w}.weight"), D, False, qkv[:, z * D:], 3 * D,
                             bias=ln(f"attn.{w}.bias"))
            ops.attention_fwd_f32(qkv, o, b, N, H, hd, 1.0 / math.sqrt(hd))
            ops.gemm_f32(T, D, D, o, D, False, ln("attn.out.weight"), D, False, h, D, bias=ln("attn.out.bias"),
                         accumulate=True)
            ops.layernorm_fwd(h, D, ln("norm2.weight"), ln("norm2.bias"), y, D, mu, rs, T, D)
            ops.gemm_f32(T, M, D, y, D, False, ln("mlp.fc1.weight"), D, True, u, M, bias=ln("mlp.fc1.bias"))
            ops.gelu_f32(u, u, T * M)
            ops.gemm_f32(T, D, M, u, M, False, ln("mlp.fc2.weight"), M, True, h, D, bias=ln("mlp.fc2.bias"),
                         accumulate=True)
        lncls = e(b, D)
        ops.layernorm_fwd(h, N * D, fv("transformer.norm.weight"), fv("transformer.norm.bias"), lncls, D, mu, rs, b, D)
        logits = e(b, C)
        ops.gemm_f32(b, C, D, lncls, D, False, fv("classifier.weight"), D, True, logits, C, bias=fv("classifier.bias"))
        return logits

    def cross_entropy(self, labels: torch.Tensor, grad_scale: float | None = None):
        a = self.acts(self._last_b)
        gs = 1.0 / a.b if grad_scale is None else grad_scale
        ops.cross_entropy(a.logits, labels.to(self.dev, torch.int64).contiguous(), a.dlogits, gs, a.row_stats)
        return a.dlogits, a.row_stats

    def backward(self, dlogits: torch.Tensor, grad: torch.Tensor | None = None):
        cfg = self.cfg
        b = self._last_b
        a = self.acts(b)
        g = self.grad if grad is None else grad
        D, M, H, N, L, C = cfg.emb_dim, cfg.mlp_dim, cfg.num_heads, cfg.tokens, cfg.num_layers, cfg.num_classes
        hd = D // H
        T = a.T
        f = self.flat
        mv = self.mirror
        gv = lambda name: g[self.off(name):]
        dl = dlogits.to(self.dev, torch.float32).contiguous()
        hook = self.grad_ready_hook
        dd = self._dd
        main = torch.cuda.current_stream(self.dev)
        overlap = self.overlap_wgrad
        if overlap and self._side is None:
            self._side = torch.cuda.Stream(device=self.dev)
        side = self._side if overlap else main
        free_ev = {}

        def on_side(fn):
            if not overlap:
                fn()
                return
            ev = self._event()
            ev.record(main)
            side.wait_event(ev)
            with torch.cuda.stream(side):
                fn()

        def release(kind, idx):
            if overlap:
                ev = self._event()
                ev.record(side)
                free_ev[(kind, idx)] = ev

        def acquire(kind, idx):
            ev = free_ev.pop((kind, idx), None)
            if ev is not None:
                main.wait_event(ev)

        def fire(bucket):
            bias.flush()
            if not hook:
                return
            evs = []
            for st in ((main, side) if overlap else (main,)):
                ev = self._event()
                ev.record(st)
                evs.append(ev)
            hook(g, *bucket, evs)

        self._ev_next = 0
        group = self.group_wgrad and D >= 256
        out_wb = None
        bias = _BiasReducer(self, a)
        ops.gemm_f32(C, D, b, dl, C, True, a.lncls, D, False, gv("classifier.weight"), D)
        bias.reduce(dl, b, C, C, (gv("classifier.bias"),))
        ops.gemm_f32(b, D, C, dl, C, False, f[self.off("classifier.weight"):], D, False, a.dlncls, D)
        wb = 0
        pruned = self._pruned
        ops.zero_(a.dh)
        if not pruned:
            ops.zero_(a.dhb[wb])
        bias.ln_bwd(a.dlncls, D, a.h[L], N * D, a.muf, a.rsf, f[self.off("transformer.norm.weight"):], a.dh, N * D, b,
                    gv("transformer.norm.weight"), gv(self.lname(L - 1, "mlp.fc2.bias")),
                    dx_bf16=a.c_dh if pruned else a.dhb[wb], lddxb=D if pruned else N * D,
                    dx_dropout=dd(3 + 3 * (L - 1), N))
        fire(self.layout.buckets[0])
        scale = 1.0 / math.sqrt(hd)
        for i in reversed(range(L)):
            ln = lambda s: self.off(self.lname(i, s))
            li = i & 1
            if pruned and i == L - 1:
                self._backward_last_cls(a, i, b, g, on_side, bias)
                wb ^= 1
            else:
                dhb = a.dhb[wb]
                on_side(lambda: self._wgrad(dhb, D, a.g[i], M, D, M, a.Tp, gv(self.lname(i, "mlp.fc2.weight")), M))
                release("dhb", wb)
                dg = a.dg[li]
                acquire("dg", li)
                gpart = bias.buf("gelu", a.gelu_parts)
                w2 = mv[ln("mlp.fc2.weight"):]
                kw = dict(a_layout=K_CONTIG, b_layout=MN_CONTIG, lda=D, ldb=M, ldc=M, epilogue=EPI_MUL_BF16, aux=a.gp[i],
                          ldaux=M, col_partial=gpart)
                ops.gemm(dhb, w2, dg, T, M, D, **kw)
                tiles_m = ops.gemm_partial_rows(dhb, w2, dg, T, M, D, **kw)
                bias.reduce(gpart, tiles_m, M, M, (gv(self.lname(i, "mlp.fc1.bias")),))
                on_side(lambda: self._wgrad(dg, M, a.ln2[i], D, M, D, a.Tp, gv(self.lname(i, "mlp.fc1.weight")), D))
                release("dg", li)
                ops.gemm(dg, mv[ln("mlp.fc1.weight"):], a.dyln, T, D, M, a_layout=K_CONTIG, b_layout=MN_CONTIG, lda=M,
                         ldb=D, ldc=D, epilogue=EPI_BF16)
                wb ^= 1
                acquire("dhb", wb)
                dhb = a.dhb[wb]
                bias.ln_bwd(a.dyln, D, a.hm[i], D, a.mu2[i], a.rs2[i], f[ln("norm2.weight"):], a.dh, D, T,
                            gv(self.lname(i, "norm2.weight")), gv(self.lname(i, "attn.out.bias")),
                            dres=a.dh, lddres=D, dx_bf16=dhb, lddxb=D, dx_dropout=dd(1 + 3 * i))
                out_spec = (a.o[i], D, dhb, D, D, D, a.Tp, gv(self.lname(i, "attn.out.weight")), D, 1, 0, 0)
                if group:
                    out_wb = wb
                else:
                    on_side(lambda: self._wgrad(*out_spec[:9]))
                    release("dhb", wb)
                ops.gemm(dhb, mv[ln("attn.out.weight"):], a.dO, T, D, D, a_layout=K_CONTIG, b_layout=K_CONTIG, lda=D,
# ... 39 lines not shown
```

### vit-of-pytorch_amd/vitmi/ops.py

```python
from __future__ import annotations

import ctypes

import torch

from . import _lib
from ._lib import COLSUM_BATCH_MAX, Dropout, GemmArgs, check

BF16 = torch.bfloat16
F32 = torch.float32


def lib():
    return _lib.load()


def _stream():
    return ctypes.c_void_p(torch.cuda.current_stream().cuda_stream)


def _p(t):
    return ctypes.c_void_p(0 if t is None else t.data_ptr())


def _chk(t, dtype, name):
    if t is None:
        return
    if not t.is_cuda:
        raise ValueError(f"{name} must be a GPU tensor")
    if t.dtype != dtype:
        raise TypeError(f"{name} must be {dtype}, got {t.dtype}")


def _gemm_args(A, B, C, M, N, K, *, a_layout, b_layout, lda, ldb, ldc, epilogue, bias=None, aux=None, ldaux=0,
               C2=None, ldc2=0, aux2=None, batch=1, a_bs=0, b_bs=0, c_bs=0, bias_bs=0, split_k=1, tokens=0, tile=0,
               col_partial=None, dropout=None):
    a = GemmArgs()
    a.M, a.N, a.K = M, N, K
    a.A, a.lda, a.a_batch_stride, a.a_layout = A.data_ptr(), lda, a_bs, a_layout
    a.B, a.ldb, a.b_batch_stride, a.b_layout = B.data_ptr(), ldb, b_bs, b_layout
    a.C, a.ldc, a.c_batch_stride = C.data_ptr(), ldc, c_bs
    a.C2, a.ldc2 = (C2.data_ptr() if C2 is not None else None), ldc2
    a.bias, a.bias_batch_stride = (bias.data_ptr() if bias is not None else None), bias_bs
    a.aux, a.ldaux = (aux.data_ptr() if aux is not None else None), ldaux
    a.aux2 = aux2.data_ptr() if aux2 is not None else None
    a.batch, a.split_k, a.tokens = batch, split_k, tokens
    a.col_partial = col_partial.data_ptr() if col_partial is not None else None
    a.epilogue, a.tile = epilogue, tile
    a.dropout = ctypes.pointer(dropout) if dropout is not None else None
    return a


def dropout_desc(p, site, seed, offset, row_stride=1):
    if not p:
        return None
    return Dropout(float(p), int(site), int(seed) & (2**64 - 1), int(offset) & (2**64 - 1), int(row_stride))


def _dp(d):
    return ctypes.pointer(d) if d is not None else None


def dropout_mask(d, row0, rows, cols, out, ld):
    _chk(out, F32, "out")
    check(lib().vit_dropout_mask(_dp(d), row0, rows, cols, _p(out), ld, _stream()), "vit_dropout_mask")


GEMM_PROBE = None
GEMM_PROBE_MIN_M = 0


def gemm(A, B, C, M, N, K, part=0, **kw):
    _chk(A, BF16, "A")
    _chk(B, BF16, "B")
    a = _gemm_args(A, B, C, M, N, K, **kw)
    if part:
        check(lib().vit_gemm_bf16_part(ctypes.byref(a), int(part), _stream()), "vit_gemm_bf16_part")
        return
    probe = GEMM_PROBE is not None and M >= GEMM_PROBE_MIN_M and a.split_k == 1 and a.epilogue != _lib.EPI_SPLITK
    if probe:
        ev0 = torch.cuda.Event(enable_timing=True)
        ev0.record()
    check(lib().vit_gemm_bf16(ctypes.byref(a), _stream()), "vit_gemm_bf16")
    if probe:
        ev1 = torch.cuda.Event(enable_timing=True)
        ev1.record()
        GEMM_PROBE.append((ev0, ev1, 2.0 * M * N * K * a.batch, int(a.epilogue)))


def gemm_tile_rows(A, B, C, M, N, K, **kw):
    return int(lib().vit_gemm_tile_rows(ctypes.byref(_gemm_args(A, B, C, M, N, K, **kw))))


def gemm_split_rows(A, B, C, M, N, K, **kw):
    return int(lib().vit_gemm_split_rows(ctypes.byref(_gemm_args(A, B, C, M, N, K, **kw))))


def gemm_partial_rows(A, B, C, M, N, K, **kw):
    return int(lib().vit_gemm_partial_rows(ctypes.byref(_gemm_args(A, B, C, M, N, K, **kw))))


def splitk_reduce(ws, batch, split, M, N, out, ldo, out_bs=0, accumulate=False):
    _chk(ws, F32, "ws")
    _chk(out, F32, "out")
    check(lib().vit_splitk_reduce(_p(ws), batch, split, M, N, _p(out), ldo, out_bs, int(accumulate), _stream()),
          "vit_splitk_reduce")


def splitk_reduce_group(jobs):
    for k in range(0, len(jobs), _lib.SPLITK_GROUP_MAX):
        part = jobs[k:k + _lib.SPLITK_GROUP_MAX]
        arr = (_lib.SplitkJob * len(part))()
        for i, (ws, batch, split, M, N, out, ldo, out_bs, acc) in enumerate(part):
            _chk(ws, F32, "ws")
            _chk(out, F32, "out")
            arr[i] = _lib.SplitkJob(_p(ws), batch, split, M, N, _p(out), ldo, out_bs, int(acc), 0)
        check(lib().vit_splitk_reduce_group(arr, len(part), _stream()), "vit_splitk_reduce_group")


def layernorm_fwd(x, ldx, gamma, beta, y, ldy, mean, rstd, rows, D, eps=1e-5):
    _chk(x, F32, "x")
    check(lib().vit_layernorm_fwd(_p(x), ldx, _p(gamma), _p(beta), _p(y), ldy, int(y.dtype == F32), _p(mean),
                                  _p(rstd), rows, D, eps, _stream()), "vit_layernorm_fwd")


def layernorm_bwd_partial_rows(rows):
    return int(lib().vit_layernorm_bwd_partial_rows(rows))


def layernorm_bwd_blocks(rows):
    return int(lib().vit_layernorm_bwd_blocks(rows))


def layernorm_bwd(dy, lddy, x, ldx, mean, rstd, gamma, dx, lddx, partial, rows, D, *, dres=None, lddres=0,
                  dx_bf16=None, lddxb=0, dgamma_dbeta=None, dx_colsum=None, accumulate=False, dx_dropout=None):
    check(lib().vit_layernorm_bwd(_p(dy), lddy, int(dy.dtype == F32), _p(x), ldx, _p(mean), _p(rstd), _p(gamma),
                                  _p(dres), lddres, _p(dx), lddx, _p(dx_bf16), lddxb, _p(partial), _p(dgamma_dbeta),
                                  _p(dx_colsum), int(accumulate), rows, D, _dp(dx_dropout), _stream()),
          "vit_layernorm_bwd")


ATTN_AUTO, ATTN_RESIDENT, ATTN_TILED, ATTN_ONESHOT = 0, 1, 2, 3


def attention_bias_rows(N, hd, path=ATTN_AUTO):
    return int(lib().vit_attention_bias_rows(N, hd, path))


def attention_workspace_elems(B, N, H, path=ATTN_AUTO):
    return int(lib().vit_attention_workspace_elems(B, N, H, path))


def attention_fwd(qkv, o, lse, B, N, H, hd, scale, q_rows=None, path=ATTN_AUTO):
    _chk(qkv, BF16, "qkv")
    _chk(o, BF16, "o")
    _chk(lse, F32, "lse")
    check(lib().vit_attention_fwd_ex(_p(qkv), _p(o), _p(lse), B, N, H, hd, scale, N if q_rows is None else q_rows,
                                     path, _stream()), "vit_attention_fwd")


def attention_bwd(qkv, o, dout, lse, dqkv, B, N, H, hd, scale, bias_partial=None, q_rows=None, path=ATTN_AUTO,
                  workspace=None):
    _chk(workspace, F32, "workspace")
    need = attention_workspace_elems(B, N, H, path)
    if need and (workspace is None or workspace.numel() < need):
        if workspace is not None:
            raise ValueError(f"attention workspace has {workspace.numel()} floats, needs {need}")
        workspace = torch.empty(need, device=qkv.device, dtype=F32)
    check(lib().vit_attention_bwd_ex(_p(qkv), _p(o), _p(dout), _p(lse), _p(dqkv), _p(bias_partial), B, N, H, hd,
                                     scale, N if q_rows is None else q_rows, path, _p(workspace if need else None),
                                     _stream()), "vit_attention_bwd")


def im2col(x, out, B, img, P, Kpad):
    _chk(x, F32, "x")
    _chk(out, BF16, "out")
    check(lib().vit_im2col(_p(x), _p(out), B, img, P, Kpad, _stream()), "vit_im2col")


def im2col_hw(x, out, B, H, W, Ph, Pw, Kpad):
    _chk(x, F32, "x")
    _chk(out, BF16, "out")
    check(lib().vit_im2col_hw(_p(x), _p(out), B, H, W, Ph, Pw, Kpad, _stream()), "vit_im2col_hw")


def preprocess_u8(images, out, flips=None, mean=(0.5, 0.5, 0.5), std=(0.5, 0.5, 0.5)):
    _chk(images, torch.uint8, "images")
    _chk(out, F32, "out")
    _chk(flips, torch.uint8, "flips")
    if images.dim() != 4 or images.shape[3] != 3 or out.dim() != 4 or out.shape[1] != 3:
        raise ValueError(f"preprocess_u8: images [B,H,W,3] -> out [B,3,h,w], got {tuple(images.shape)} -> "
                         f"{tuple(out.shape)}")
    B, H, W, _ = images.shape
    if out.shape[0] != B or (flips is not None and flips.numel() != B):
        raise ValueError("preprocess_u8: batch mismatch")
    if images[0].stride() != (W * 3, 3, 1) or not out.is_contiguous():
        raise ValueError("preprocess_u8: images must have contiguous [H, W, 3] rows and out must be contiguous")
    ms = (ctypes.c_float * 6)(*[float(v) for v in mean], *[float(v) for v in std])
    check(lib().vit_preprocess_u8(_p(images), B, H, W, images.stride(0) if B > 1 else H * W * 3, _p(flips),
                                  out.shape[2], out.shape[3], ms, _p(out), _stream()), "vit_preprocess_u8")


IMAGES_HWC, IMAGES_CHW = 0, 1


def preprocess_u8_gather(images, index, out, flips=None, mean=(0.5, 0.5, 0.5), std=(0.5, 0.5, 0.5), layout=IMAGES_HWC,
                         labels_in=None, labels_out=None, image_stride=None):
    _chk(images, torch.uint8, "images")
    _chk(index, torch.int64, "index")
    _chk(out, F32, "out")
    _chk(flips, torch.uint8, "flips")
    _chk(labels_in, torch.int64, "labels_in")
    _chk(labels_out, torch.int64, "labels_out")
    chw = layout == IMAGES_CHW
    if images.dim() != 4 or images.shape[1 if chw else 3] != 3 or out.dim() != 4 or out.shape[1] != 3:
        raise ValueError(f"preprocess_u8_gather: images {'[n,3,H,W]' if chw else '[n,H,W,3]'} -> out [B,3,h,w], got "
                         f"{tuple(images.shape)} -> {tuple(out.shape)}")
    n = images.shape[0]
    H, W = (images.shape[2], images.shape[3]) if chw else (images.shape[1], images.shape[2])
    B = out.shape[0]
    if index.dim() != 1 or index.numel() != B or (flips is not None and flips.numel() != B) or \
            (labels_out is not None and labels_out.numel() != B) or (labels_in is not None and labels_in.numel() != n):
        raise ValueError("preprocess_u8_gather: batch mismatch")
    if n and images[0].stride() != ((H * W, W, 1) if chw else (W * 3, 3, 1)) or not out.is_contiguous():
        raise ValueError("preprocess_u8_gather: every image must be contiguous and out must be contiguous")
    for name, t in (("index", index), ("flips", flips), ("labels_in", labels_in), ("labels_out", labels_out)):
        if t is not None and not t.is_contiguous():
            raise ValueError(f"preprocess_u8_gather: {name} must be contiguous")
    if image_stride is None:
        image_stride = images.stride(0) if n > 1 else H * W * 3
    ms = (ctypes.c_float * 6)(*[float(v) for v in mean], *[float(v) for v in std])
    check(lib().vit_preprocess_u8_gather(_p(images), n, int(layout), H, W, int(image_stride), _p(index), B, _p(flips),
                                         out.shape[2], out.shape[3], ms, _p(out), _p(labels_in), _p(labels_out),
                                         _stream()), "vit_preprocess_u8_gather")


def embed_grad(dh0, B, N, D, dpos, dcls, dconv_bias, dropout=None):
    check(lib().vit_embed_grad(_p(dh0), B, N, D, _p(dpos), _p(dcls), _p(dconv_bias), _dp(dropout), _stream()),
          "vit_embed_grad")


def colsum_partial_rows(rows):
    return int(lib().vit_colsum_partial_rows(rows))


def colsum(inp, rows, cols, ld, partial, out, accumulate=False):
    check(lib().vit_colsum(_p(inp), int(inp.dtype == BF16), rows, cols, ld, _p(partial), _p(out), int(accumulate),
                           _stream()), "vit_colsum")


def colsum_batch(jobs):
    arr = (_lib.ColsumJob * len(jobs))()
# ... 175 lines not shown
    part = torch.empty(B, device=x.device, dtype=F32)
    loss = torch.empty((), device=x.device, dtype=F32)
    check(lib().vit_cls_mse(_p(x), ldx, _p(t), ldt, B, D, _p(e), _p(part), _p(loss), _stream()), "vit_cls_mse")
    return loss, e


def cls_mse_bwd(dx, lddx, e, g):
    _chk(dx, F32, "dx")
    _chk(e, F32, "e")
    _chk(g, F32, "g")
    check(lib().vit_cls_mse_bwd(_p(dx), lddx, _p(e), e.shape[0], e.shape[1], _p(g), _stream()), "vit_cls_mse_bwd")


def router_select(indices, active_sets, nkeys):
    _chk(indices, F32, "indices")
    if not indices.is_contiguous():
        raise ValueError("router_select: indices must be contiguous")
    T, dev = indices.numel(), indices.device
    masks = []
    for st in active_sets:
        m = 0
        for v in st:
            if not 0 <= int(v) < 32:
                raise ValueError(f"router_select: index value {v} outside [0, 32)")
            m |= 1 << int(v)
        masks.append(m)
    active = torch.empty(len(masks), T, device=dev, dtype=torch.bool)
    sel = torch.empty(nkeys, T, device=dev, dtype=torch.bool)
    anyf = torch.empty(nkeys, device=dev, dtype=torch.bool)
    arr = (ctypes.c_uint32 * max(len(masks), 1))(*masks)
    check(lib().vit_router_select(_p(indices), T, len(masks), arr, nkeys, _p(active), _p(sel), _p(anyf), _stream()),
          "vit_router_select")
    return active, sel, anyf


def cast_rows_masked(inp, ldi, rows, cols, mask, out, ldo):
    _chk(inp, F32, "inp")
    _chk(out, BF16, "out")
    if mask is not None and (mask.dtype != torch.bool or not mask.is_contiguous() or mask.numel() != rows):
        raise ValueError("cast_rows_masked: mask must be a contiguous bool tensor of `rows` elements")
    check(lib().vit_cast_rows_masked(_p(inp), ldi, rows, cols, _p(mask), _p(out), ldo, _stream()),
          "vit_cast_rows_masked")


def unpack_bf16_f32(inp, ldi, rows, cols, out, ldo):
    _chk(inp, BF16, "inp")
    _chk(out, F32, "out")
    check(lib().vit_unpack_bf16_f32(_p(inp), ldi, rows, cols, _p(out), ldo, _stream()), "vit_unpack_bf16_f32")


def attention_fwd_varlen(q, ldq, k, ldk, v, ldv, o, ldo, cu_q, B, max_q, Nkv, H, hd, scale):
    for t, n in ((q, "q"), (k, "k"), (v, "v"), (o, "o")):
        _chk(t, BF16, n)
    _chk(cu_q, torch.int32, "cu_q")
    check(lib().vit_attention_fwd_varlen(_p(q), ldq, _p(k), ldk, _p(v), ldv, _p(o), ldo, _p(cu_q), B, max_q, Nkv, H,
                                         hd, scale, _stream()), "vit_attention_fwd_varlen")


def sqnorm_partial(g, n, partial):
    _chk(g, F32, "g")
    _chk(partial, torch.float64, "partial")
    check(lib().vit_sqnorm_partial(_p(g), n, _p(partial), partial.numel(), _stream()), "vit_sqnorm_partial")


def adamw_prep(partial, used, steps, lr, beta1, beta2, max_norm, table, norm_out):
    nseg = 0 if steps is None else steps.numel()
    check(lib().vit_adamw_prep(_p(partial), 0 if partial is None else partial.numel(), _p(used), _p(steps), nseg,
                               lr, beta1, beta2, max_norm, _p(table), _p(norm_out), _stream()), "vit_adamw_prep")


def adamw_update(p, g, m, v, p_bf16, chunks, table, lr, beta1, beta2, eps, wd, write_grad):
    check(lib().vit_adamw_update(_p(p), _p(g), _p(m), _p(v), _p(p_bf16), _p(chunks), chunks.numel() // 3, _p(table),
                                 1.0 - lr * wd, beta1, beta2, 1.0 - beta1, 1.0 - beta2, eps, int(write_grad),
                                 _stream()), "vit_adamw_update")


def adamw_chunk_elems():
    return lib().vit_adamw_chunk_elems()


def scale_by_coef(g, n, coef):
    check(lib().vit_scale_by_coef(_p(g), n, _p(coef), _stream()), "vit_scale_by_coef")


def zero_(t):
    if not t.is_contiguous():
        raise ValueError("zero_: contiguous tensor expected")
    check(lib().vit_zero(_p(t), t.numel() * t.element_size(), _stream()), "vit_zero")


def splitk_factor_group(shapes, K, cus=256):
    tiles = sum(-(-M // 256) * -(-N // 256) * b for M, N, b in shapes)
    smax = max(1, min((K // 64) // 8, 32))
    t_tile = 2.0 * 256 * 256 * K / 4.0e12
    slab = sum(2.0 * M * N * 4 * b for M, N, b in shapes) / 5.0e12
    best, best_t = 1, None
    for s in range(1, smax + 1):
        t = -(-tiles * s // cus) * t_tile / s + s * slab
        if best_t is None or t < best_t * (1 - 1e-9):
            best, best_t = s, t
    return best


def gemm_splitk_group(members):
    if not 1 <= len(members) <= 4:
        raise ValueError("gemm_splitk_group: 1 to 4 members")
    arr = (GemmArgs * len(members))()
    for i, (A, B, C, M, N, K, kw) in enumerate(members):
        _chk(A, BF16, "A")
        _chk(B, BF16, "B")
        arr[i] = _gemm_args(A, B, C, M, N, K, **kw)
    check(lib().vit_gemm_splitk_group(arr, len(members), _stream()), "vit_gemm_splitk_group")


def splitk_factor(M, N, K, batch=1, cus=256):
    tile = 256 if M >= 256 and N >= 256 else 128
    slots = cus if tile == 256 else 2 * cus
    tiles = -(-M // tile) * -(-N // tile) * batch
    smax = max(1, min((K // 64) // 8, 32))
    t_tile = 2.0 * tile * tile * K / 4.0e12
    slab = 2.0 * M * N * 4 * batch / 5.0e12
    best, best_t = 1, None
    for s in range(1, smax + 1):
        t = -(-tiles * s // slots) * t_tile / s + s * slab
        if best_t is None or t < best_t * (1 - 1e-9):
            best, best_t = s, t
    return best


def wgrad(A, lda, B, ldb, M, N, K, out, ldo, accumulate=False, batch=1, a_bs=0, b_bs=0, out_bs=0, target=256):
    from ._lib import EPI_SPLITK, MN_CONTIG
    s = splitk_factor(M, N, K, batch, target)
    ws = torch.empty(batch * s * M * N, device=out.device, dtype=F32)
    gemm(A, B, ws, M, N, K, a_layout=MN_CONTIG, b_layout=MN_CONTIG, lda=lda, ldb=ldb, ldc=N, epilogue=EPI_SPLITK,
         batch=batch, a_bs=a_bs, b_bs=b_bs, split_k=s)
    splitk_reduce(ws, batch, s, M, N, out, ldo, out_bs, accumulate)


def rows_select(dst, mask, src=None):
    if mask.dtype != torch.bool or not mask.is_contiguous() or mask.numel() != dst.shape[0]:
        raise ValueError("rows_select: mask must be a contiguous bool tensor of dst.shape[0] elements")
    rb = dst.shape[1] * dst.element_size()
    if src is not None and (src.dtype != dst.dtype or src.shape[1] != dst.shape[1]):
        raise ValueError("rows_select: src must match dst's dtype and row width")
    check(lib().vit_rows_select(_p(dst), dst.stride(0) * dst.element_size(), _p(src),
                                0 if src is None else src.stride(0) * src.element_size(), _p(mask), dst.shape[0], rb,
                                _stream()), "vit_rows_select")


def copy2d(dst, dpitch, src, spitch, width, height):
    check(lib().vit_copy2d(_p(dst), dpitch, _p(src), spitch, width, height, _stream()), "vit_copy2d")


def sgd_step_dev(p, g, buf, p_bf16, n, hyper, wd):
    _chk(hyper, F32, "hyper")
    check(lib().vit_sgd_step_dev(_p(p), _p(g), _p(buf), _p(p_bf16), n, _p(hyper), wd, _stream()), "vit_sgd_step_dev")
```

Baseline: 7670 images/sec.

## Add skinny split-K GEMM for CLS-token layer and fuse QKV packing into SGD

Adds a new split-K GEMM kernel (256x64 tiles with an fp32 workspace) for small-M GEMMs, used by the last-layer CLS-token forward and backward matmuls, where the regular 256-row tiles leave most CUs idle. Separately, the SGD step kernel gains a variant that writes the packed bf16 QKV weights and fp32 QKV biases directly while updating parameters. This lets the mirror refresh skip its separate QKV pack pass. The cost is extra workspace, a reduction step, per-element index arithmetic in the optimizer, and more complex state tracking for when the pack is valid.

After: 7707 images/sec, median of 6. No clear change (+0.5%).

```diff
diff --git a/include/vit_hip.h b/include/vit_hip.h
--- a/include/vit_hip.h
+++ b/include/vit_hip.h
@@ -73,11 +73,14 @@
   int32_t epilogue;
   int32_t tile;
   const vit_dropout* dropout;
+  void* ws;
+  int64_t ws_bytes;
 } vit_gemm_args;
 
 int vit_gemm_bf16(const vit_gemm_args* args, vit_stream_t stream);
 int64_t vit_gemm_tile_rows(const vit_gemm_args* args);
 int64_t vit_gemm_partial_rows(const vit_gemm_args* args);
+int64_t vit_gemm_workspace_bytes(const vit_gemm_args* args);
 int64_t vit_gemm_split_rows(const vit_gemm_args* args);
 int vit_gemm_bf16_part(const vit_gemm_args* args, int32_t part, vit_stream_t stream);
 int vit_gemm_splitk_group(const vit_gemm_args* args, int32_t n, vit_stream_t stream);
@@ -177,6 +180,13 @@
                  float momentum, float weight_decay, int32_t first, vit_stream_t stream);
 int vit_sgd_step_dev(float* p, const float* g, float* buf, void* p_bf16, int64_t n, const float* hyper,
                      float weight_decay, vit_stream_t stream);
+typedef struct vit_qkv_pack {
+  int64_t weight_off, bias_off, layer_stride, qkv_stride, emb_dim, layers;
+  void* wqkv;
+  float* bqkv;
+} vit_qkv_pack;
+int vit_sgd_step_dev_pack(float* p, const float* g, float* buf, void* p_bf16, int64_t n, const float* hyper,
+                          float weight_decay, const vit_qkv_pack* qkv, vit_stream_t stream);
 int vit_cast_f32_bf16(const float* in, void* out, int64_t n, vit_stream_t stream);
 int vit_cast_pad_rows(const float* in, int64_t rows, int64_t cols, void* out, int64_t ldo,
                       vit_stream_t stream);
diff --git a/vit-of-pytorch_amd/csrc/capi.hip b/vit-of-pytorch_amd/csrc/capi.hip
--- a/vit-of-pytorch_amd/csrc/capi.hip
+++ b/vit-of-pytorch_amd/csrc/capi.hip
@@ -21,5 +21,5 @@
 }
 
 extern "C" const char* vit_last_error(void) { return vit::g_last_error; }
-extern "C" int vit_abi_version(void) { return 20; }
+extern "C" int vit_abi_version(void) { return 21; }
 extern "C" const char* vit_build_id(void) { return VIT_BUILD_ID; }
diff --git a/vit-of-pytorch_amd/csrc/elementwise.hip b/vit-of-pytorch_amd/csrc/elementwise.hip
--- a/vit-of-pytorch_amd/csrc/elementwise.hip
+++ b/vit-of-pytorch_amd/csrc/elementwise.hip
@@ -1,4 +1,5 @@
 #include "common.h"
+#include <type_traits>
 
 namespace {
 
@@ -360,9 +361,17 @@
     f = hyper[2] != 0.0f;
   }
 };
-template <class S>
+struct QkvPackDev {
+  unsigned wlo, wspan, blo, bspan;
+  unsigned ls, zs, D, L;
+  int lrev, zrev;
+  bf16_t* wqkv;
+  float* bqkv;
+};
+struct NoPack {};
+template <class S, class P = NoPack>
 __global__ void sgd_kernel(float* __restrict__ p, const float* __restrict__ g, float* __restrict__ buf,
-                           bf16_t* __restrict__ pb, long n, const S sc, float wd) {
+                           bf16_t* __restrict__ pb, long n, const S sc, float wd, const P pk = P{}) {
   float lr, mom;
   bool first;
   sc.get(lr, mom, first);
@@ -383,6 +392,30 @@
       u.x = pack2bf(pv.x, pv.y);
       u.y = pack2bf(pv.z, pv.w);
       reinterpret_cast<uint2*>(pb)[i] = u;
+    }
+    if constexpr (!std::is_same<P, NoPack>::value) {
+      const unsigned e = (unsigned)i * 4u;
+      const unsigned rw = e - pk.wlo, rb = e - pk.blo;
+      if (rw < pk.wspan) {
+        const unsigned li = rw / pk.ls, w = rw - li * pk.ls;
+        const unsigned zi = w / pk.zs, wz = w - zi * pk.zs;
+        if (zi < 3u && wz < pk.D * pk.D) {
+          const unsigned r = wz / pk.D, c = wz - r * pk.D;
+          const unsigned layer = pk.lrev ? pk.L - 1u - li : li, z = pk.zrev ? 2u - zi : zi;
+          uint2 u;
+          u.x = pack2bf(pv.x, pv.y);
+          u.y = pack2bf(pv.z, pv.w);
+          *reinterpret_cast<uint2*>(pk.wqkv + ((size_t)(layer * pk.D + r) * 3u + z) * pk.D + c) = u;
+        }
+      }
+      if (rb < pk.bspan) {
+        const unsigned li = rb / pk.ls, w = rb - li * pk.ls;
+        const unsigned zi = w / pk.zs, wz = w - zi * pk.zs;
+        if (zi < 3u && wz < pk.D) {
+          const unsigned layer = pk.lrev ? pk.L - 1u - li : li, z = pk.zrev ? 2u - zi : zi;
+          *reinterpret_cast<float4*>(pk.bqkv + (size_t)(layer * 3u + z) * pk.D + wz) = pv;
+        }
+      }
     }
   }
   const long t = n4 * 4 + (long)blockIdx.x * blockDim.x + threadIdx.x;
@@ -675,6 +708,35 @@
   hipLaunchKernelGGL(sgd_kernel<SgdDevScalars>, dim3(grid_for(n, 4)), dim3(256), 0, (hipStream_t)stream, p, g, buf,
                      (bf16_t*)p_bf16, (long)n, SgdDevScalars{hyper}, weight_decay);
   VIT_LAUNCH_CHECK("vit_sgd_step_dev");
+}
+
+extern "C" int vit_sgd_step_dev_pack(float* p, const float* g, float* buf, void* p_bf16, int64_t n, const float* hyper,
+                                     float weight_decay, const vit_qkv_pack* q, vit_stream_t stream) {
+  VIT_CHECK_ARG(p && g && buf && hyper && n >= 0 && q, "vit_sgd_step_dev_pack: bad args");
+  VIT_CHECK_ARG(((uintptr_t)p | (uintptr_t)g | (uintptr_t)buf) % 16 == 0 && ((uintptr_t)p_bf16 % 8 == 0),
+                "vit_sgd_step_dev_pack: buffers must be 16-B aligned (bf16 mirror 8-B)");
+  const int64_t D = q->emb_dim, L = q->layers;
+  const int64_t ls = q->layer_stride < 0 ? -q->layer_stride : q->layer_stride;
+  const int64_t zs = q->qkv_stride < 0 ? -q->qkv_stride : q->qkv_stride;
+  const int64_t down = (q->layer_stride < 0 ? (L - 1) * q->layer_stride : 0) + (q->qkv_stride < 0 ? 2 * q->qkv_stride : 0);
+  const int64_t wlo = q->weight_off + down, blo = q->bias_off + down;
+  const int64_t wspan = (L - 1) * ls + 2 * zs + D * D, bspan = (L - 1) * ls + 2 * zs + D;
+  VIT_CHECK_ARG(q->wqkv && q->bqkv && D >= 4 && L >= 1 && zs >= D * D && (L == 1 || ls >= 3 * zs) &&
+                    (D | ls | zs | q->weight_off | q->bias_off) % 4 == 0 && wlo >= 0 && blo >= 0 &&
+                    wlo + wspan <= n && blo + bspan <= n && n < (1LL << 32) && (uintptr_t)q->wqkv % 8 == 0 &&
+                    (uintptr_t)q->bqkv % 16 == 0,
+                "vit_sgd_step_dev_pack: the q|k|v weights [D][D] and biases [D] must sit inside p at constant, "
+                "non-overlapping strides (multiples of 4 elements), n < 2^32");
+  if (n == 0) return VIT_OK;
+  QkvPackDev d;
+  d.wlo = (unsigned)wlo; d.wspan = (unsigned)wspan; d.blo = (unsigned)blo; d.bspan = (unsigned)bspan;
+  d.ls = L == 1 ? 0xffffffffu : (unsigned)ls;
+  d.zs = (unsigned)zs; d.D = (unsigned)D; d.L = (unsigned)L;
+  d.lrev = q->layer_stride < 0; d.zrev = q->qkv_stride < 0;
+  d.wqkv = (bf16_t*)q->wqkv; d.bqkv = q->bqkv;
+  hipLaunchKernelGGL((sgd_kernel<SgdDevScalars, QkvPackDev>), dim3(grid_for(n, 4)), dim3(256), 0, (hipStream_t)stream, p,
+                     g, buf, (bf16_t*)p_bf16, (long)n, SgdDevScalars{hyper}, weight_decay, d);
+  VIT_LAUNCH_CHECK("vit_sgd_step_dev_pack");
 }
 
 extern "C" int vit_sgd_step(float* p, const float* g, float* buf, void* p_bf16, int64_t n, float lr, float momentum,
diff --git a/vit-of-pytorch_amd/csrc/gemm.hip b/vit-of-pytorch_amd/csrc/gemm.hip
--- a/vit-of-pytorch_amd/csrc/gemm.hip
+++ b/vit-of-pytorch_amd/csrc/gemm.hip
@@ -4,33 +4,7 @@
 using vitg::GemmDev;
 using vitg::EPI_DROP;
 
-int pick_tile(const vit_gemm_args* a) {
-  if (a->tile > 0) return (int)a->tile;
-  const bool ak = a->a_layout == VIT_K_CONTIG, bk = a->b_layout == VIT_K_CONTIG;
-  if (a->epilogue == VIT_EPI_SPLITK && a->M >= 256 && a->N >= 256) {
-    static const int env_sk = vit::knob("VIT_GEMM_SPLITK_CFG", 9);
-    return env_sk == 5 || env_sk == 6 || env_sk == 7 || env_sk == 8 ? env_sk : 9;
-  }
-  if (a->M >= 1024 && a->N >= 256) {
-    static const int env_rs = vit::knob("VIT_GEMM_RESID_PP2", 1);
-    if (ak && (env_rs || !(a->epilogue == VIT_EPI_BIAS_RESID_F32 && a->K < 2048))) return 9;
-    if (a->N >= 2048 && a->epilogue != VIT_EPI_GELU_BWD && a->epilogue != VIT_EPI_MUL_BF16) return 5;
-    if (!bk && a->K >= 3072) return 5;
-    return 3;
-  }
-  return 0;
-}
-
-int tile_rows_of(int cfg) {
-  switch (cfg) {
-    case 1: case 2: case 3: case 5: case 6: case 7: case 8: case 9: case 10: case 11: return 256;
-    default: return 128;
-  }
-}
-
-long wave_split_rows(const vit_gemm_args* a, int cfg) {
-  if (!((cfg == 5 || cfg == 9) && a->batch == 1 && a->split_k == 1 && a->epilogue != VIT_EPI_PATCH && a->tile == 0))
-    return 0;
+int num_cus() {
   static const int ncu = [] {
     int dev = 0, n = 0;
     if (hipGetDevice(&dev) != hipSuccess || hipDeviceGetAttribute(&n, hipDeviceAttributeMultiprocessorCount, dev) !=
@@ -38,6 +12,90 @@
       return 0;
     return n;
   }();
+  return ncu;
+}
+
+bool vec_aligned(const vit_gemm_args* a) {
+  auto al = [](const void* q) { return ((uintptr_t)q % 32) == 0; };
+  bool v = al(a->C) && a->ldc % 8 == 0 && a->c_batch_stride % 8 == 0;
+  if (a->C2) v = v && al(a->C2) && a->ldc2 % 8 == 0;
+  if (a->bias) v = v && al(a->bias) && a->bias_batch_stride % 8 == 0;
+  if (a->aux) v = v && al(a->aux) && a->ldaux % 8 == 0;
+  if (a->aux2) v = v && al(a->aux2);
+  if (a->epilogue == VIT_EPI_SPLITK) v = al(a->C) && a->N % 8 == 0;
+  return v;
+}
+
+constexpr int CFG_SKINNY = 12;
+constexpr int TILE_SKINNY_SPLIT = 1200;
+
+bool skinny_forced(const vit_gemm_args* a) { return a->tile == CFG_SKINNY || a->tile >= TILE_SKINNY_SPLIT; }
+
+bool skinny_able(const vit_gemm_args* a) {
+  const int e = a->epilogue;
+  return a->M >= 1 && a->M <= 256 && a->N >= 8 && a->N % 8 == 0 && a->K >= 64 && a->K % 64 == 0 && a->batch == 1 &&
+         a->split_k == 1 && !(a->dropout && a->dropout->p > 0.0f) && a->a_layout == VIT_K_CONTIG &&
+         (e == VIT_EPI_BF16 || e == VIT_EPI_BIAS_BF16 || e == VIT_EPI_BIAS_RESID_F32 || e == VIT_EPI_GELU_BWD ||
+          e == VIT_EPI_BIAS_GELU_DGELU || e == VIT_EPI_MUL_BF16) &&
+         a->C && vec_aligned(a);
+}
+
+int skinny_split(const vit_gemm_args* a) {
+  const int nkt = (int)(a->K / 64);
+  if (a->tile > TILE_SKINNY_SPLIT) {
+    const int s = a->tile - TILE_SKINNY_SPLIT;
+    return s < nkt ? s : nkt;
+  }
+  const int ncu = num_cus() > 0 ? num_cus() : 256;
+  const int tiles = (int)((a->N + 63) / 64);
+  int s = (ncu + tiles) / (2 * tiles);
+  if (s > nkt / 2) s = nkt / 2;
+  return s < 1 ? 1 : s;
+}
+
+bool skinny_gains(const vit_gemm_args* a) {
+  const int ncu = num_cus() > 0 ? num_cus() : 256;
+  const long tiles128 = ((a->M + 127) / 128) * ((a->N + 127) / 128);
+  return a->K >= 512 && 4 * tiles128 <= ncu;
+}
+
+long skinny_ws_bytes(const vit_gemm_args* a) { return (long)skinny_split(a) * a->M * a->N * 4; }
+
+bool skinny_ws_ok(const vit_gemm_args* a) {
+  return a->ws && ((uintptr_t)a->ws % 32) == 0 && a->ws_bytes >= skinny_ws_bytes(a);
+}
+
+int pick_tile(const vit_gemm_args* a) {
+  if (skinny_forced(a)) return CFG_SKINNY;
+  if (a->tile > 0) return (int)a->tile;
+  if (a->M <= 256 && skinny_able(a) && skinny_gains(a) && skinny_ws_ok(a)) return CFG_SKINNY;
+  const bool ak = a->a_layout == VIT_K_CONTIG, bk = a->b_layout == VIT_K_CONTIG;
+  if (a->epilogue == VIT_EPI_SPLITK && a->M >= 256 && a->N >= 256) {
+    static const int env_sk = vit::knob("VIT_GEMM_SPLITK_CFG", 9);
+    return env_sk == 5 || env_sk == 6 || env_sk == 7 || env_sk == 8 ? env_sk : 9;
+  }
+  if (a->M >= 1024 && a->N >= 256) {
+    static const int env_rs = vit::knob("VIT_GEMM_RESID_PP2", 1);
+    if (ak && (env_rs || !(a->epilogue == VIT_EPI_BIAS_RESID_F32 && a->K < 2048))) return 9;
+    if (a->N >= 2048 && a->epilogue != VIT_EPI_GELU_BWD && a->epilogue != VIT_EPI_MUL_BF16) return 5;
+    if (!bk && a->K >= 3072) return 5;
+    return 3;
+  }
+  return 0;
+}
+
+int tile_rows_of(int cfg) {
+  switch (cfg) {
+    case 1: case 2: case 3: case 5: case 6: case 7: case 8: case 9: case 10: case 11: return 256;
+    case CFG_SKINNY: return vitg::SKINNY_PART_ROWS;
+    default: return 128;
+  }
+}
+
+long wave_split_rows(const vit_gemm_args* a, int cfg) {
+  if (!((cfg == 5 || cfg == 9) && a->batch == 1 && a->split_k == 1 && a->epilogue != VIT_EPI_PATCH && a->tile == 0))
+    return 0;
+  const int ncu = num_cus();
   if (ncu <= 0) return 0;
   const long tiles_n = (a->N + 255) / 256, tiles = ((a->M + 255) / 256) * tiles_n;
   const long full = tiles / ncu, rem = tiles - full * ncu;
@@ -67,6 +125,11 @@
   }
   const long tr = tile_rows_of(cfg);
   return (a->M + tr - 1) / tr;
+}
+
+extern "C" int64_t vit_gemm_workspace_bytes(const vit_gemm_args* a) {
+  if (!a || !skinny_able(a) || !(skinny_forced(a) || (a->tile == 0 && skinny_gains(a)))) return 0;
+  return skinny_ws_bytes(a);
 }
 
 extern "C" int64_t vit_gemm_split_rows(const vit_gemm_args* a) {
@@ -128,16 +191,7 @@
   d.bias = a->bias; d.bias_bs = a->bias_batch_stride;
   d.aux = a->aux; d.ldaux = a->ldaux; d.aux2 = a->aux2;
   d.split_k = (int)a->split_k; d.tokens = (int)a->tokens;
-  {
-    auto al = [](const void* q) { return ((uintptr_t)q % 32) == 0; };
-    bool v = al(a->C) && a->ldc % 8 == 0 && a->c_batch_stride % 8 == 0;
-    if (a->C2) v = v && al(a->C2) && a->ldc2 % 8 == 0;
-    if (a->bias) v = v && al(a->bias) && a->bias_batch_stride % 8 == 0;
-    if (a->aux) v = v && al(a->aux) && a->ldaux % 8 == 0;
-    if (a->aux2) v = v && al(a->aux2);
-    if (a->epilogue == VIT_EPI_SPLITK) v = al(a->C) && a->N % 8 == 0;
-    d.vec = v ? 1 : 0;
-  }
+  d.vec = vec_aligned(a) ? 1 : 0;
   d.col_partial = a->col_partial;
   d.drop = make_drop(a->dropout);
   VIT_CHECK_ARG(!d.drop.thr || a->epilogue == VIT_EPI_PATCH || a->epilogue == VIT_EPI_BIAS_RESID_F32 ||
@@ -182,6 +236,16 @@
   hipStream_t s = (hipStream_t)stream;
   const int batch = (int)a->batch, split = (int)a->split_k;
   const int cfg = pick_tile(a);
+  if (cfg == CFG_SKINNY) {
+    VIT_CHECK_ARG(skinny_able(a), "vit_gemm_bf16: the skinny path needs M <= 256, N %% 8 == 0, batch 1, split_k 1, no "
+                                  "dropout, a K-contiguous A, aligned operands and a BF16 / BIAS_BF16 / BIAS_RESID_F32 / "
+                                  "GELU_BWD / BIAS_GELU_DGELU / MUL_BF16 epilogue");
+    VIT_CHECK_ARG(skinny_ws_ok(a), "vit_gemm_bf16: the skinny path needs a 32-byte aligned ws of %ld bytes",
+                  skinny_ws_bytes(a));
+    if (part == 2) return VIT_OK;
+    return vit::check_hip(vitg::launch_skinny(a->epilogue, d, bk, skinny_split(a), (float*)a->ws, s),
+                          "vit_gemm_bf16 skinny launch");
+  }
 #ifdef VIT_DIAG_KNOBS
   VIT_CHECK_ARG(cfg >= 0 && cfg <= 11, "vit_gemm_bf16: bad tile config %d", cfg);
 #else
diff --git a/vit-of-pytorch_amd/csrc/gemm_decl.h b/vit-of-pytorch_amd/csrc/gemm_decl.h
--- a/vit-of-pytorch_amd/csrc/gemm_decl.h
+++ b/vit-of-pytorch_amd/csrc/gemm_decl.h
@@ -48,6 +48,9 @@
 };
 hipError_t launch_splitk_group(const GemmGroup& g, hipStream_t s);
 
+constexpr int SKINNY_PART_ROWS = 32;
+hipError_t launch_skinny(int epi, const GemmDev& d, bool bk, int split, float* ws, hipStream_t s);
+
 constexpr int EPI_DROP = 16;
 
 template <int EPI>
diff --git a/vit-of-pytorch_amd/csrc/gemm_skinny.hip b/vit-of-pytorch_amd/csrc/gemm_skinny.hip
--- /dev/null
+++ b/vit-of-pytorch_amd/csrc/gemm_skinny.hip
@@ -0,0 +1,230 @@
+#include "gemm_kernels.h"
+
+namespace {
+constexpr int SK_BM = 256, SK_BN = 64, SK_BK = 64, SK_STAGES = 3, SK_NWAVE = 8;
+
+__device__ __forceinline__ int swz_mn64(int row) { return ((row & 3) ^ ((row >> 3) & 1)) & 3; }
+
+__device__ __forceinline__ void stage_b_mn64(char* smem, int lds_off, __amdgpu_buffer_rsrc_t rs, long ld, int kt,
+                                             int wave, int lane) {
+  const int c = wave * 64 + lane;
+  const int r = c >> 3, pc = c & 7;
+  const int lane_off = (int)(r * ld * 2) + ((pc * 16) ^ (swz_mn64(r) << 5));
+  const int base = __builtin_amdgcn_readfirstlane((int)((long)kt * SK_BK * ld * 2));
+  __builtin_amdgcn_raw_ptr_buffer_load_lds(rs, LDS_PTR(void, smem + lds_off + wave * 1024), 16, lane_off + base, 0, 0,
+                                           0);
+}
+__device__ __forceinline__ uint32_t frag_tr64_lane_off(int r0, int lane) {
+  const int g = lane >> 4, i = lane & 15, q = i >> 2, p = i & 3;
+  const int ra = 8 * g + q;
+  return (uint32_t)(ra * (SK_BN * 2) + (((r0 + 4 * p) * 2) ^ (swz_mn64(ra) << 5)));
+}
+
+template <bool BKC>
+__global__ void __launch_bounds__(SK_NWAVE * 64, 2) gemm_skinny_kernel(const GemmDev p, float* __restrict__ ws) {
+  constexpr int BM = SK_BM, BN = SK_BN, BK = SK_BK, STAGES = SK_STAGES, NWAVE = SK_NWAVE;
+  constexpr int NT = NWAVE * 64;
+  constexpr int FM = 2, FN = BN / 16, KK = BK / 32;
+  constexpr int A_BYTES = BM * BK * 2, B_BYTES = BN * BK * 2;
+  constexpr int STAGE = A_BYTES + B_BYTES;
+  constexpr int PIPE = STAGES * STAGE;
+  constexpr int LPS = STAGE / 1024 / NWAVE;
+  constexpr int LDC = BN + 4;
+  static_assert(BM * LDC * 4 <= PIPE && PIPE <= 160 * 1024, "LDS budget");
+  __shared__ __attribute__((aligned(16))) char smem[PIPE];
+
+  const int lane = threadIdx.x & 63;
+  const int wave = __builtin_amdgcn_readfirstlane(threadIdx.x >> 6);
+  const int n0 = blockIdx.x * BN, split_idx = blockIdx.y;
+  const int wm0 = wave * 32;
+  const bool active = wm0 < p.M;
+
+  const long b_shift = BKC ? (long)n0 * p.ldb * 2 : (long)n0 * 2;
+  const uint32_t b_rec = (long)p.b_bytes > b_shift ? (uint32_t)(p.b_bytes - b_shift) : 0u;
+  const __amdgpu_buffer_rsrc_t rsA = make_rsrc(p.A, p.a_bytes);
+  const __amdgpu_buffer_rsrc_t rsB = make_rsrc(p.B + b_shift, b_rec);
+
+  const int nkt = p.K / BK;
+  const int kt0 = (int)((long)nkt * split_idx / p.split_k);
+  const int kt1 = (int)((long)nkt * (split_idx + 1) / p.split_k);
+  const int nk = kt1 - kt0;
+
+  v4f acc[FM][FN];
+#pragma unroll
+  for (int i = 0; i < FM; ++i)
+#pragma unroll
+    for (int j = 0; j < FN; ++j) acc[i][j] = v4f{0.f, 0.f, 0.f, 0.f};
+
+  auto issue = [&](int step) {
+    const int buf = (step % STAGES) * STAGE;
+    stage_tile<BM, BK, true, NWAVE>(smem, buf, rsA, p.lda, kt0 + step, wave, lane);
+    if constexpr (BKC)
+      stage_tile<BN, BK, true, NWAVE>(smem, buf + A_BYTES, rsB, p.ldb, kt0 + step, wave, lane);
+    else
+      stage_b_mn64(smem, buf + A_BYTES, rsB, p.ldb, kt0 + step, wave, lane);
+  };
+#pragma unroll
+  for (int s = 0; s < STAGES - 1; ++s)
+    if (s < nk) issue(s);
+
+  for (int t = 0; t < nk; ++t) {
+    if (nk - 1 - t >= STAGES - 2)
+      wait_vm<LPS*(STAGES - 2)>();
+    else
+      wait_vm<0>();
+    __builtin_amdgcn_s_barrier();
+    asm volatile("" ::: "memory");
+    if (t + STAGES - 1 < nk) issue(t + STAGES - 1);
+    const int cur = (t % STAGES) * STAGE;
+    if (active) {
+      if constexpr (BKC) {
+#pragma unroll
+        for (int kk = 0; kk < KK; ++kk) {
+          v8s bfr[FN];
+#pragma unroll
+          for (int j = 0; j < FN; ++j) bfr[j] = read_frag<BN, BK, true>(smem, cur + A_BYTES, j * 16, kk, lane);
+#pragma unroll
+          for (int i = 0; i < FM; ++i) {
+            const v8s af = read_frag<BM, BK, true>(smem, cur, wm0 + i * 16, kk, lane);
+#pragma unroll
+            for (int j = 0; j < FN; ++j)
+              acc[i][j] = __builtin_amdgcn_mfma_f32_16x16x32_bf16(__builtin_bit_cast(v8bf, af),
+                                                                  __builtin_bit_cast(v8bf, bfr[j]), acc[i][j], 0, 0, 0);
+          }
+        }
+      } else {
+        const uint32_t sb = __builtin_amdgcn_readfirstlane((uint32_t)(uintptr_t)LDS_PTR(char, smem) + cur);
+#pragma unroll
+        for (int kk = 0; kk < KK; ++kk) {
+          v8s bfr[FN], af[FM];
+#pragma unroll
+          for (int j = 0; j < FN; ++j)
+            bfr[j] = kk == 0 ? read_frag_tr_asm<BN, 0>(sb + A_BYTES + frag_tr64_lane_off(j * 16, lane))
+                             : read_frag_tr_asm<BN, 1>(sb + A_BYTES + frag_tr64_lane_off(j * 16, lane));
+#pragma unroll
+          for (int i = 0; i < FM; ++i) af[i] = read_frag<BM, BK, true>(smem, cur, wm0 + i * 16, kk, lane);
+          asm volatile("s_waitcnt lgkmcnt(0)" ::: "memory");
+          __builtin_amdgcn_sched_barrier(0);
+#pragma unroll
+          for (int i = 0; i < FM; ++i)
+#pragma unroll
+            for (int j = 0; j < FN; ++j)
+              acc[i][j] = __builtin_amdgcn_mfma_f32_16x16x32_bf16(__builtin_bit_cast(v8bf, af[i]),
+                                                                  __builtin_bit_cast(v8bf, bfr[j]), acc[i][j], 0, 0, 0);
+        }
+      }
+    }
+    asm volatile("" ::: "memory");
+  }
+
+  const int g = lane >> 4, c = lane & 15;
+  wait_vm<0>();
+  __syncthreads();
+  float* cs = reinterpret_cast<float*>(smem);
+  if (active) {
+#pragma unroll
+    for (int i = 0; i < FM; ++i)
+#pragma unroll
+      for (int j = 0; j < FN; ++j)
+#pragma unroll
+        for (int r = 0; r < 4; ++r) cs[(wm0 + i * 16 + 4 * g + r) * LDC + j * 16 + c] = acc[i][j][r];
+  }
+  __syncthreads();
+  constexpr int CPR = BN / 8;
+  float* slab = ws + (long)split_idx * p.M * p.N;
+#pragma unroll
+  for (int it = 0; it < BM * CPR / NT; ++it) {
+    const int e = threadIdx.x + it * NT;
+    const int m = e / CPR, n = n0 + (e % CPR) * 8;
+    if (m < p.M && n < p.N) {
+      float v[8];
+      ld8f(cs + m * LDC + (e % CPR) * 8, v);
+      st8f(slab + (long)m * p.N + n, v);
+    }
+  }
+}
+
+template <int EPI>
+__global__ void __launch_bounds__(256) skinny_finish_kernel(const GemmDev p, const float* __restrict__ ws, int split) {
+  constexpr int PR = vitg::SKINNY_PART_ROWS;
+  __shared__ float red[PR][SK_BN];
+  const int ch = threadIdx.x & 7, row = threadIdx.x >> 3;
+  const int m = blockIdx.y * PR + row, n = blockIdx.x * SK_BN + ch * 8;
+  const bool ok = m < p.M && n < p.N;
+  float v[8] = {0.f, 0.f, 0.f, 0.f, 0.f, 0.f, 0.f, 0.f};
+  if (ok) {
+    constexpr int AW = AuxPre<EPI>::W > 0 ? AuxPre<EPI>::W : 1;
+    uint4 ax[AW];
+    if constexpr (AuxPre<EPI>::W > 0) AuxPre<EPI>::fetch(p, m, n, ax);
+    const long total4 = (long)p.M * p.N / 4;
+    const float4* w = reinterpret_cast<const float4*>(ws + (long)m * p.N + n);
+    float4 s0 = make_float4(0.f, 0.f, 0.f, 0.f), s1 = s0;
+    int k = 0;
+    for (; k + 4 <= split; k += 4) {
+      const float4 a0 = w[(long)k * total4], b0 = w[(long)(k + 1) * total4];
+      const float4 c0 = w[(long)(k + 2) * total4], d0 = w[(long)(k + 3) * total4];
+      const float4 a1 = w[(long)k * total4 + 1], b1 = w[(long)(k + 1) * total4 + 1];
+      const float4 c1 = w[(long)(k + 2) * total4 + 1], d1 = w[(long)(k + 3) * total4 + 1];
+      s0.x += (a0.x + b0.x) + (c0.x + d0.x);
+      s0.y += (a0.y + b0.y) + (c0.y + d0.y);
+      s0.z += (a0.z + b0.z) + (c0.z + d0.z);
+      s0.w += (a0.w + b0.w) + (c0.w + d0.w);
+      s1.x += (a1.x + b1.x) + (c1.x + d1.x);
+      s1.y += (a1.y + b1.y) + (c1.y + d1.y);
+      s1.z += (a1.z + b1.z) + (c1.z + d1.z);
+      s1.w += (a1.w + b1.w) + (c1.w + d1.w);
+    }
+    for (; k < split; ++k) {
+      const float4 a0 = w[(long)k * total4], a1 = w[(long)k * total4 + 1];
+      s0.x += a0.x; s0.y += a0.y; s0.z += a0.z; s0.w += a0.w;
+      s1.x += a1.x; s1.y += a1.y; s1.z += a1.z; s1.w += a1.w;
+    }
+    v[0] = s0.x; v[1] = s0.y; v[2] = s0.z; v[3] = s0.w;
+    v[4] = s1.x; v[5] = s1.y; v[6] = s1.z; v[7] = s1.w;
+    float u[8];
+    if constexpr (AuxPre<EPI>::W > 0) AuxPre<EPI>::unpack(ax, u);
+    epi_store8<EPI>(p, 0, 0, m, n, v, AuxPre<EPI>::W > 0 ? u : nullptr);
+  }
+  if (p.col_partial) {
+#pragma unroll
+    for (int k = 0; k < 8; ++k) red[row][ch * 8 + k] = ok ? v[k] : 0.f;
+    __syncthreads();
+    const int col = blockIdx.x * SK_BN + threadIdx.x;
+    if (threadIdx.x < SK_BN && col < p.N) {
+      float sum = 0.f;
+#pragma unroll 8
+      for (int r = 0; r < PR; ++r) sum += red[r][threadIdx.x];
+      p.col_partial[(long)blockIdx.y * p.N + col] = sum;
+    }
+  }
+}
+
+template <int EPI>
+void launch_finish(const GemmDev& d, const float* ws, int split, hipStream_t s) {
+  const dim3 grid((d.N + SK_BN - 1) / SK_BN, (d.M + vitg::SKINNY_PART_ROWS - 1) / vitg::SKINNY_PART_ROWS);
+  hipLaunchKernelGGL((skinny_finish_kernel<EPI>), grid, dim3(256), 0, s, d, ws, split);
+}
+}
+
+hipError_t vitg::launch_skinny(int epi, const GemmDev& d, bool bk, int split, float* ws, hipStream_t s) {
+  if (d.M < 1 || d.M > SK_BM || d.N % 8 != 0 || !d.vec || split < 1 || split > d.K / SK_BK || !ws)
+    return hipErrorInvalidValue;
+  GemmDev g = d;
+  g.split_k = split;
+  const dim3 grid((d.N + SK_BN - 1) / SK_BN, split);
+  if (bk)
+    hipLaunchKernelGGL((gemm_skinny_kernel<true>), grid, dim3(SK_NWAVE * 64), 0, s, g, ws);
+  else
+    hipLaunchKernelGGL((gemm_skinny_kernel<false>), grid, dim3(SK_NWAVE * 64), 0, s, g, ws);
+  if (const hipError_t e = hipGetLastError(); e != hipSuccess) return e;
+  switch (epi) {
+    case VIT_EPI_BF16: launch_finish<VIT_EPI_BF16>(d, ws, split, s); break;
+    case VIT_EPI_BIAS_BF16: launch_finish<VIT_EPI_BIAS_BF16>(d, ws, split, s); break;
+    case VIT_EPI_BIAS_RESID_F32: launch_finish<VIT_EPI_BIAS_RESID_F32>(d, ws, split, s); break;
+    case VIT_EPI_GELU_BWD: launch_finish<VIT_EPI_GELU_BWD>(d, ws, split, s); break;
+    case VIT_EPI_BIAS_GELU_DGELU: launch_finish<VIT_EPI_BIAS_GELU_DGELU>(d, ws, split, s); break;
+    case VIT_EPI_MUL_BF16: launch_finish<VIT_EPI_MUL_BF16>(d, ws, split, s); break;
+    default: return hipErrorInvalidValue;
+  }
+  return hipGetLastError();
+}
diff --git a/vit-of-pytorch_amd/vitmi/_lib.py b/vit-of-pytorch_amd/vitmi/_lib.py
--- a/vit-of-pytorch_amd/vitmi/_lib.py
+++ b/vit-of-pytorch_amd/vitmi/_lib.py
@@ -11,7 +11,7 @@
 c_f32 = ctypes.c_float
 c_vp = ctypes.c_void_p
 
-ABI_VERSION = 20
+ABI_VERSION = 21
 
 K_CONTIG, MN_CONTIG = 0, 1
 (EPI_F32, EPI_BF16, EPI_BIAS_BF16, EPI_BIAS_GELU, EPI_BIAS_RESID_F32, EPI_GELU_BWD, EPI_PATCH, EPI_SPLITK,
@@ -35,6 +35,7 @@
         ("aux", c_vp), ("ldaux", c_i64), ("aux2", c_vp),
         ("batch", c_i64), ("split_k", c_i64), ("tokens", c_i64), ("col_partial", c_vp),
         ("epilogue", c_i32), ("tile", c_i32), ("dropout", ctypes.POINTER(Dropout)),
+        ("ws", c_vp), ("ws_bytes", c_i64),
     ]
 
 
@@ -52,6 +53,11 @@
 
 
 SPLITK_GROUP_MAX = 8
+
+
+class QkvPack(ctypes.Structure):
+    _fields_ = [("weight_off", c_i64), ("bias_off", c_i64), ("layer_stride", c_i64), ("qkv_stride", c_i64),
+                ("emb_dim", c_i64), ("layers", c_i64), ("wqkv", c_vp), ("bqkv", c_vp)]
 
 
 class CastJob(ctypes.Structure):
@@ -68,6 +74,7 @@
     "vit_gemm_tile_rows": (c_i64, [ctypes.POINTER(GemmArgs)]),
     "vit_gemm_partial_rows": (c_i64, [ctypes.POINTER(GemmArgs)]),
     "vit_gemm_split_rows": (c_i64, [ctypes.POINTER(GemmArgs)]),
+    "vit_gemm_workspace_bytes": (c_i64, [ctypes.POINTER(GemmArgs)]),
     "vit_gemm_bf16_part": (c_i32, [ctypes.POINTER(GemmArgs), c_i32, c_vp]),
     "vit_gemm_splitk_group": (c_i32, [ctypes.POINTER(GemmArgs), c_i32, c_vp]),
     "vit_segment_colsum": (c_i32, [c_vp, c_i32, c_i64, c_i64, c_i64, c_i64, c_i64, c_i64, c_f32, c_vp, c_i64, c_vp]),
@@ -147,6 +154,7 @@
     "vit_copy2d": (c_i32, [c_vp, c_i64, c_vp, c_i64, c_i64, c_i64, c_vp]),
     "vit_rows_select": (c_i32, [c_vp, c_i64, c_vp, c_i64, c_vp, c_i64, c_i64, c_vp]),
     "vit_sgd_step_dev": (c_i32, [c_vp, c_vp, c_vp, c_vp, c_i64, c_vp, c_f32, c_vp]),
+    "vit_sgd_step_dev_pack": (c_i32, [c_vp, c_vp, c_vp, c_vp, c_i64, c_vp, c_f32, ctypes.POINTER(QkvPack), c_vp]),
     "vit_build_id": (ctypes.c_char_p, []),
 }
 
diff --git a/vit-of-pytorch_amd/vitmi/engine.py b/vit-of-pytorch_amd/vitmi/engine.py
--- a/vit-of-pytorch_amd/vitmi/engine.py
+++ b/vit-of-pytorch_amd/vitmi/engine.py
@@ -2,6 +2,7 @@
 
 import math
 import os
+import weakref
 from collections import OrderedDict
 from dataclasses import dataclass
 
@@ -176,7 +177,7 @@
         self.dlogits = z(b, cfg.num_classes, dt=f)
         self.row_stats = z(b, 3, dt=f)
         self.lnparts = [z(ops.layernorm_bwd_blocks(T), 3 * D, dt=f) for _ in range(_NBUF)]
-        self.gelu_parts = [z(-(-T // 128), M, dt=f) for _ in range(_NBUF)]
+        self.gelu_parts = [z(max(-(-T // 128), -(-b // 32)), M, dt=f) for _ in range(_NBUF)]
         self.attn_bias_rows = ops.attention_bias_rows(N, D // H)
         self.qkv_bparts = [z(b * self.attn_bias_rows, 3 * D, dt=f) for _ in range(_NBUF)]
         nws = ops.attention_workspace_elems(b, N, H)
@@ -257,7 +258,16 @@
         o = [self.off(self.lname(i, "norm1.weight")) for i in range(L)]
         self.layer_stride = o[0] - o[1] if L > 1 else 0
         assert all(o[i] == o[0] - i * self.layer_stride for i in range(L))
+        self._qkv_packed = False
+        if L >= 1 and n < 2**32:
+            zs = (self.off(self.lname(0, "attn.key.weight")) - self.off(self.lname(0, "attn.query.weight")))
+            me = weakref.ref(self)
+            ops.register_qkv_pack(self.flat, self.off(self.lname(0, "attn.query.weight")),
+                                  self.off(self.lname(0, "attn.query.bias")), -self.layer_stride, zs, D, L, self.wqkv,
+                                  self.bqkv, lambda: setattr(me(), "_qkv_packed", True) if me() is not None else None)
+            weakref.finalize(self, ops._QKV_PACKERS.pop, self.flat.data_ptr(), None)
         self._ws = None
+        self._cls_ws_need = {}
         self.step_id = 0
         self.grad_ready_hook = None
         self.grad_ready_finish = None
@@ -299,12 +309,19 @@
 
     def invalidate_mirror(self):
         self._mirror_sig = None
+        self._qkv_packed = False
 
     def refresh_mirror(self, full=True):
         cfg = self.cfg
         D = cfg.emb_dim
         if full:
             ops.cast_bf16(self.flat, self.mirror, self.layout.numel)
+        packed, self._qkv_packed = self._qkv_packed, False
+        if packed and not full:
+            if self.wconv is not None:
+                w = self.off("embedding.weight")
+                ops.cast_pad_rows(self.flat[w:], D, cfg.patch_k, self.wconv, self.wconv.shape[1])
+            return
         M, L = cfg.mlp_dim, cfg.num_layers
         lst = self.layer_stride
         o0 = lambda s: self.off(self.lname(0, s))
@@ -334,6 +351,17 @@
         if self._ws is None or self._ws.numel() < numel:
             self._ws = torch.empty(numel, device=self.dev)
         return self._ws
+
+    def _cls_gemm(self, A, B, C, M, N, K, ws=True, **kw):
+        if ws:
+            key = (M, N, K, kw["epilogue"], kw["b_layout"])
+            need = self._cls_ws_need.get(key)
+            if need is None:
+                need = self._cls_ws_need[key] = ops.gemm_workspace_bytes(A, B, C, M, N, K, **kw)
+            if need:
+                kw = dict(kw, ws=self._workspace(need // 4))
+        ops.gemm(A, B, C, M, N, K, **kw)
+        return kw
 
     def _wgrad(self, A, lda, B, ldb, M, N, K, out, ldo, batch=1, b_bs=0, out_bs=0):
         s = self._splitk(M, N, K, batch)
@@ -452,15 +480,16 @@
         f, mv = self.flat, self.mirror
         ln = lambda s: self.off(self.lname(i, s))
         S = N * D
-        ops.gemm(a.o[i], mv[ln("attn.out.weight"):], a.hm[i], b, D, D, a_layout=K_CONTIG, b_layout=MN_CONTIG, lda=S,
-                 ldb=D, ldc=S, epilogue=EPI_BIAS_RESID_F32, bias=f[ln("attn.out.bias"):], aux=a.h[i], ldaux=S)
+        gemm = self._cls_gemm
+        gemm(a.o[i], mv[ln("attn.out.weight"):], a.hm[i], b, D, D, a_layout=K_CONTIG, b_layout=MN_CONTIG, lda=S,
+             ldb=D, ldc=S, epilogue=EPI_BIAS_RESID_F32, bias=f[ln("attn.out.bias"):], aux=a.h[i], ldaux=S)
         ops.copy2d(a.c_o, D * 2, a.o[i], S * 2, D * 2, b)
         ops.layernorm_fwd(a.hm[i], S, f[ln("norm2.weight"):], f[ln("norm2.bias"):], a.c_ln2, D, a.c_mu2, a.c_rs2,
                           b, D)
-        ops.gemm(a.c_ln2, mv[ln("mlp.fc1.weight"):], a.c_gp, b, M, D, a_layout=K_CONTIG, b_layout=K_CONTIG, lda=D,
-                 ldb=D, ldc=M, epilogue=EPI_BIAS_GELU_DGELU, bias=f[ln("mlp.fc1.bias"):], C2=a.c_g, ldc2=M)
-        ops.gemm(a.c_g, mv[ln("mlp.fc2.weight"):], a.h[i + 1], b, D, M, a_layout=K_CONTIG, b_layout=K_CONTIG,
-                 lda=M, ldb=M, ldc=S, epilogue=EPI_BIAS_RESID_F32, bias=f[ln("mlp.fc2.bias"):], aux=a.hm[i], ldaux=S)
+        gemm(a.c_ln2, mv[ln("mlp.fc1.weight"):], a.c_gp, b, M, D, a_layout=K_CONTIG, b_layout=K_CONTIG, lda=D,
+             ldb=D, ldc=M, epilogue=EPI_BIAS_GELU_DGELU, bias=f[ln("mlp.fc1.bias"):], C2=a.c_g, ldc2=M)
+        gemm(a.c_g, mv[ln("mlp.fc2.weight"):], a.h[i + 1], b, D, M, a_layout=K_CONTIG, b_layout=K_CONTIG,
+             lda=M, ldb=M, ldc=S, epilogue=EPI_BIAS_RESID_F32, bias=f[ln("mlp.fc2.bias"):], aux=a.hm[i], ldaux=S)
 
     def _backward_last_cls(self, a, i, b, g, on_side, bias):
         cfg = self.cfg
@@ -474,18 +503,19 @@
         w2 = mv[self.off(self.lname(i, "mlp.fc2.weight")):]
         kw = dict(a_layout=K_CONTIG, b_layout=MN_CONTIG, lda=D, ldb=M, ldc=M, epilogue=EPI_MUL_BF16, aux=a.c_gp,
                   ldaux=M, col_partial=gpart)
-        ops.gemm(a.c_dh, w2, a.c_dg, b, M, D, **kw)
+        ws = not self.overlap_wgrad
+        kw = self._cls_gemm(a.c_dh, w2, a.c_dg, b, M, D, ws=ws, **kw)
         tiles_m = ops.gemm_partial_rows(a.c_dh, w2, a.c_dg, b, M, D, **kw)
         bias.reduce(gpart, tiles_m, M, M, (gv("mlp.fc1.bias"),))
         on_side(lambda: self._wgrad(a.c_dg, M, a.c_ln2, D, M, D, bp, gv("mlp.fc1.weight"), D))
-        ops.gemm(a.c_dg, mv[self.off(self.lname(i, "mlp.fc1.weight")):], a.c_dyln, b, D, M, a_layout=K_CONTIG,
-                 b_layout=MN_CONTIG, lda=M, ldb=D, ldc=D, epilogue=EPI_BF16)
+        self._cls_gemm(a.c_dg, mv[self.off(self.lname(i, "mlp.fc1.weight")):], a.c_dyln, b, D, M, ws=ws,
+                       a_layout=K_CONTIG, b_layout=MN_CONTIG, lda=M, ldb=D, ldc=D, epilogue=EPI_BF16)
         bias.ln_bwd(a.c_dyln, D, a.hm[i], S, a.c_mu2, a.c_rs2, f[self.off(self.lname(i, "norm2.weight")):], a.dh, S, b,
                     gv("norm2.weight"), gv("attn.out.bias"), dres=a.dh, lddres=S, dx_bf16=a.c_dh2, lddxb=D)
         on_side(lambda: self._wgrad(a.c_o, D, a.c_dh2, D, D, D, bp, gv("attn.out.weight"), D))
         ops.zero_(a.dO)
-        ops.gemm(a.c_dh2, mv[self.off(self.lname(i, "attn.out.weight")):], a.dO, b, D, D, a_layout=K_CONTIG,
-                 b_layout=K_CONTIG, lda=D, ldb=D, ldc=S, epilogue=EPI_BF16)
+        self._cls_gemm(a.c_dh2, mv[self.off(self.lname(i, "attn.out.weight")):], a.dO, b, D, D, ws=ws,
+                       a_layout=K_CONTIG, b_layout=K_CONTIG, lda=D, ldb=D, ldc=S, epilogue=EPI_BF16)
 
     def forward_exact(self, x: torch.Tensor):
         cfg = self.cfg
diff --git a/vit-of-pytorch_amd/vitmi/ops.py b/vit-of-pytorch_amd/vitmi/ops.py
--- a/vit-of-pytorch_amd/vitmi/ops.py
+++ b/vit-of-pytorch_amd/vitmi/ops.py
@@ -34,7 +34,7 @@
 
 def _gemm_args(A, B, C, M, N, K, *, a_layout, b_layout, lda, ldb, ldc, epilogue, bias=None, aux=None, ldaux=0,
                C2=None, ldc2=0, aux2=None, batch=1, a_bs=0, b_bs=0, c_bs=0, bias_bs=0, split_k=1, tokens=0, tile=0,
-               col_partial=None, dropout=None):
+               col_partial=None, dropout=None, ws=None):
     a = GemmArgs()
     a.M, a.N, a.K = M, N, K
     a.A, a.lda, a.a_batch_stride, a.a_layout = A.data_ptr(), lda, a_bs, a_layout
@@ -48,6 +48,9 @@
     a.col_partial = col_partial.data_ptr() if col_partial is not None else None
     a.epilogue, a.tile = epilogue, tile
     a.dropout = ctypes.pointer(dropout) if dropout is not None else None
+    if ws is not None:
+        _chk(ws, F32, "ws")
+        a.ws, a.ws_bytes = ws.data_ptr(), ws.numel() * 4
     return a
 
 
@@ -98,6 +101,10 @@
 
 def gemm_partial_rows(A, B, C, M, N, K, **kw):
     return int(lib().vit_gemm_partial_rows(ctypes.byref(_gemm_args(A, B, C, M, N, K, **kw))))
+
+
+def gemm_workspace_bytes(A, B, C, M, N, K, **kw):
+    return int(lib().vit_gemm_workspace_bytes(ctypes.byref(_gemm_args(A, B, C, M, N, K, **kw))))
 
 
 def splitk_reduce(ws, batch, split, M, N, out, ldo, out_bs=0, accumulate=False):
@@ -579,6 +586,27 @@
     check(lib().vit_copy2d(_p(dst), dpitch, _p(src), spitch, width, height, _stream()), "vit_copy2d")
 
 
+_QKV_PACKERS = {}
+
+
+def register_qkv_pack(flat, weight_off, bias_off, layer_stride, qkv_stride, emb_dim, layers, wqkv, bqkv, on_packed):
+    _chk(wqkv, BF16, "wqkv")
+    _chk(bqkv, F32, "bqkv")
+    desc = _lib.QkvPack(weight_off, bias_off, layer_stride, qkv_stride, emb_dim, layers, wqkv.data_ptr(),
+                        bqkv.data_ptr())
+    _QKV_PACKERS[flat.data_ptr()] = (flat.numel(), desc, (wqkv, bqkv), on_packed)
+
+
+def unregister_qkv_pack(flat):
+    _QKV_PACKERS.pop(flat.data_ptr(), None)
+
+
 def sgd_step_dev(p, g, buf, p_bf16, n, hyper, wd):
     _chk(hyper, F32, "hyper")
+    e = _QKV_PACKERS.get(p.data_ptr())
+    if e is not None and p_bf16 is not None and n == e[0] == p.numel():
+        check(lib().vit_sgd_step_dev_pack(_p(p), _p(g), _p(buf), _p(p_bf16), n, _p(hyper), wd, ctypes.byref(e[1]),
+                                          _stream()), "vit_sgd_step_dev_pack")
+        e[3]()
+        return
     check(lib().vit_sgd_step_dev(_p(p), _p(g), _p(buf), _p(p_bf16), n, _p(hyper), wd, _stream()), "vit_sgd_step_dev")
```
